# MadNLP/MadNLP.jl

Hardware: AMD Instinct MI355X
Metric: IP iterations/sec + ms per factorize!/solve!, condensed KKT n≈1e4 (higher is better)
Workload: dtype f64; 1 GPU; BASELINE config C3: case1354pegase-shaped sparse-condensed KKT, one instance; N=11192, m=16646, nnz(K)=68688; step = compress_J+compress_H+build_kkt+factorize (n_f=1) + inertia fetch + 2 solve_linear_system per instance; algorithm=BUNCHKAUFMAN (device: static-pivot LDL^T), outer_block=0, batch_per_gpu=1, batch_api=n/a (one instance), parallelism=1 GPU(s) x 1 independent instance(s)

## Files before the change

### include/madnlp_hip.h

```cpp
#ifndef MADNLP_HIP_H
#define MADNLP_HIP_H

#include <stdint.h>

#ifdef __cplusplus
extern "C" {
#endif

#define MNK_VERSION 100

enum { MNK_HOST = 0, MNK_DEVICE = 1 };

enum { MNK_BUNCHKAUFMAN = 1, MNK_LU = 2, MNK_QR = 3, MNK_CHOLESKY = 4, MNK_LDL = 5, MNK_EVD = 6 };

typedef struct mnk_ctx mnk_ctx;
typedef struct mnk_sc mnk_sc;
typedef struct mnk_dc mnk_dc;
typedef struct mnk_ls mnk_ls;

int mnk_version(void);
const char* mnk_last_error_string(void);
int mnk_ctx_create(int device, void* stream, mnk_ctx** out);
int mnk_ctx_destroy(mnk_ctx* ctx);
int mnk_ctx_synchronize(mnk_ctx* ctx);
// ... 156 lines not shown
                                       double* zl, double* zu);
int mnk_ipm_set_f_RR(mnk_ipm* ipm, double* f_R, const double* D_R, const double* x, const double* x_ref, double zeta);
int mnk_ipm_set_aug_rhs_RR(mnk_ipm* ipm, const double* f_R, const double* zl, const double* zu, const double* jacl,
                           const double* c, const double* y, const double* pp, const double* nn, const double* zp,
                           const double* zn, int64_t m, const double* x, const double* xl, const double* xu, double mu_R,
                           double rho, double* px, double* py, double* pzl, double* pzu);
int mnk_ipm_finish_aug_solve_RR(mnk_ipm* ipm, double* dpp, double* dnn, double* dzp, double* dzn, const double* l,
                                const double* dl, const double* pp, const double* nn, const double* zp, const double* zn,
                                int64_t m, double mu_R, double rho);
int mnk_ipm_reset_bound_dual_1(mnk_ipm* ipm, double* z, const double* x, int64_t n, double mu, double kappa_sigma);
int mnk_ipm_set_initial_bounds(mnk_ipm* ipm, double* xl, double* xu, int64_t n, double tol);
int mnk_ipm_set_initial_rhs(mnk_ipm* ipm, const double* f, const double* zl, const double* zu, double* px, double* py,
                            int64_t m, double* pzl, double* pzu);
int mnk_ipm_set_aug_rhs_ifr(mnk_ipm* ipm, const double* c, int64_t m, double* px, double* py, double* pzl, double* pzu);
int mnk_ipm_set_g_ifr(mnk_ipm* ipm, double* g, const double* f, const double* x, const double* xl, const double* xu,
                      const double* jacl, double mu);
int mnk_ipm_initialize_variables(mnk_ipm* ipm, double* x, const double* xl, const double* xu, int64_t n, double bound_push,
                                 double bound_fac);
int mnk_sc_set_aug_RR(mnk_sc* sc, const double* x, const double* xl, const double* xu, const double* zl, const double* zu,
                      const double* D_R, const double* pp, const double* zp, const double* nn, const double* zn, double zeta,
                      double primal_reg, double dual_reg);
int mnk_dc_set_aug_RR(mnk_dc* dc, const double* x, const double* xl, const double* xu, const double* zl, const double* zu,
                      const double* D_R, const double* pp, const double* zp, const double* nn, const double* zn, double zeta,
                      double primal_reg, double dual_reg);

int mnk_ipm_get_dot(mnk_ipm* ipm, const double* x, const double* y, int64_t n, double* out);
int mnk_ipm_get_sum(mnk_ipm* ipm, const double* v, int64_t n, double* out);
int mnk_ipm_get_norm2(mnk_ipm* ipm, const double* v, int64_t n, double* out);
int mnk_ipm_vec_copy(mnk_ipm* ipm, double* dst, const double* src, int64_t n);
int mnk_ipm_vec_fill(mnk_ipm* ipm, double* v, int64_t n, double value);
int mnk_ipm_vec_axpby(mnk_ipm* ipm, double* out, double a, const double* x, double b, const double* y, int64_t n);
int mnk_ipm_vec_scatter_axpy(mnk_ipm* ipm, double* y, const int64_t* idx, double a, const double* x, int64_t n);
int mnk_ipm_vec_gather(mnk_ipm* ipm, double* out, double a, const double* x, const int64_t* idx, int64_t n);
int mnk_ipm_bound_dual_axpy(mnk_ipm* ipm, double* zl, double* zu, double a, const double* dzl, const double* dzu);
int mnk_ipm_bound_dual_fill(mnk_ipm* ipm, double* zl, double* zu, double v);
int mnk_ipm_gemv(mnk_ipm* ipm, int trans, int64_t m, int64_t n, double alpha, const double* A, int64_t lda, const double* x,
                 double beta, double* y);

typedef struct mnk_opf mnk_opf;
int mnk_opf_create(mnk_ctx* ctx, int64_t nbus, int64_t ngen, int64_t nbranch, const int32_t* fr, const int32_t* to,
                   const int32_t* gen_bus, const double* arc_coef, const double* bus_data, const double* gen_cost,
                   mnk_opf** out);
int mnk_opf_destroy(mnk_opf* opf);
int mnk_opf_sizes(mnk_opf* opf, int64_t* n, int64_t* m, int64_t* nnzj, int64_t* nnzh);
int mnk_opf_obj_terms(mnk_opf* opf, const double* x, double* terms );
int mnk_opf_grad(mnk_opf* opf, const double* x, double* g);
int mnk_opf_cons(mnk_opf* opf, const double* x, double* c);
int mnk_opf_jac_coord(mnk_opf* opf, const double* x, double* jac);
int mnk_opf_hess_coord(mnk_opf* opf, const double* x, const double* y, double obj_weight, double* hess);

typedef struct mnk_schur mnk_schur;
int mnk_schur_create(mnk_ctx* ctx, int64_t ns_local, int64_t blk, int64_t nd, int algo, mnk_schur** out);
int mnk_schur_destroy(mnk_schur* h);
int mnk_schur_set_block(mnk_schur* h, int64_t k, const double* A_kk, int64_t lda, const double* C_dk, int64_t ldc,
                        int loc);
int mnk_schur_build_local(mnk_schur* h, const double* S0, int64_t lds0, int loc_s0, double* S_out, int64_t lds_out);
int mnk_schur_factorize_s(mnk_schur* h, const double* S, int64_t lds, int loc, int* info);
int mnk_schur_inertia_s(mnk_schur* h, int64_t* num_pos, int64_t* num_zero, int64_t* num_neg);
int mnk_schur_scenario_inertia(mnk_schur* h, int64_t k, int64_t* num_pos, int64_t* num_zero, int64_t* num_neg);
int mnk_schur_forward(mnk_schur* h, double* rhs_k, double* contrib_d);
int mnk_schur_solve_s(mnk_schur* h, double* rhs_d);
int mnk_schur_backward(mnk_schur* h, double* rhs_k, const double* x_d);
void* mnk_schur_s_buffer(mnk_schur* h);
int mnk_schur_set_structure(mnk_schur* h, int64_t n, int64_t m, int64_t nv, int64_t nc, int64_t nnzh, const int32_t* hess_I,
                            const int32_t* hess_J, int64_t nnzj, const int32_t* jac_I, const int32_t* jac_J, int64_t n_ineq,
                            const int64_t* ind_ineq, int64_t n_eq, const int64_t* ind_eq, int index_base, int64_t ns_global,
                            const int64_t* local_scen, int own_design);
int mnk_schur_assemble(mnk_schur* h, const double* hess, const double* jac, const double* pr_diag, const double* du_diag, int loc);
void* mnk_schur_s0_buffer(mnk_schur* h);
int mnk_schur_get_block(mnk_schur* h, int64_t k, double* A_kk, double* C_dk, double* S0);
int mnk_schur_solve(mnk_schur* h, double* rhs_k, double* rhs_d, int loc);

int mnk_ls_debug_solve_trace(mnk_ls* ls, unsigned long long* out, int64_t n);

int mnk_ls_debug_dag_state(mnk_ls* ls, int* flags, int64_t nflags, int* chain, int64_t nchain, int* have);

int mnk_debug_grid_at_launch(int cu_first, int num_cu, int first, int per_cu);
int mnk_debug_shader_clock(mnk_ctx* ctx, double* mhz);

int mnk_debug_dag_tasks(int ntile, int chunk, int band_tiles, int js2, int taper0, int* out, int cap, int* first_phase);
int mnk_debug_dag_merged_tasks(int ntile, int chunk, int band_tiles, int js2, int taper0, int fill, int ninst, int period,
                               int* out, int cap);

int mnk_debug_update(mnk_ctx* ctx, int variant, int64_t M, int64_t K, const double* A, int64_t lda,
                     double* C, double* C2, int64_t ldc, int reps, double* ms);

#ifdef __cplusplus
}
#endif
#endif
```

### madnlp.jl_amd/_lib.py

```python
from __future__ import annotations

import ctypes as C
import os
import subprocess

_HERE = os.path.dirname(os.path.abspath(__file__))
CSRC = os.path.join(_HERE, "csrc")
LIBDIR = os.path.join(_HERE, "lib")
LIBPATH = os.path.join(LIBDIR, "libmadnlp_hip.so")
_LIB_OVERRIDE = os.environ.get("MNK_LIBPATH")
SOURCES = ["gemm_f64.hip", "dag.hip", "factor.hip", "solve.hip", "ls.hip", "sparse_kkt.hip", "dense_kkt.hip", "bk.hip", "schur.hip", "ipm_vec.hip", "opf_eval.hip", "qr.hip"]
HEADERS = ["common.h", "ls.h", "kkt_vec.h", "gemm_tile.h", "leaf64.h", "gemm_macro.h", os.path.join("..", "..", "include", "madnlp_hip.h")]

MNK_HOST, MNK_DEVICE = 0, 1
MNK_BUNCHKAUFMAN, MNK_LU, MNK_QR, MNK_CHOLESKY, MNK_LDL, MNK_EVD = 1, 2, 3, 4, 5, 6
MNK_SC_JT, MNK_SC_HESS, MNK_SC_AUG, MNK_SC_DIAGBUF = 0, 1, 2, 3


def _stale() -> bool:
    if not os.path.exists(LIBPATH):
        return True
    t = os.path.getmtime(LIBPATH)
    deps = [os.path.join(CSRC, s) for s in SOURCES + HEADERS]
    return any(os.path.exists(d) and os.path.getmtime(d) > t for d in deps)
# ... 103 lines not shown
    "mnk_ipm_get_rel_search_norm": (C.c_int, [_vp, _vp, _vp, C.POINTER(C.c_double)]),
    "mnk_ipm_get_sd_sc": (C.c_int, [_vp, _vp, C.c_int64, _vp, _vp, C.c_double, C.POINTER(C.c_double)]),
    "mnk_ipm_get_norms": (C.c_int, [_vp, _vp, C.c_int64, C.POINTER(C.c_double)]),
    "mnk_ipm_set_perturbation_sets": (C.c_int, [_vp, C.c_int64, _vp, C.c_int64, _vp, C.c_int]),
    "mnk_ipm_set_aug_rhs": (C.c_int, [_vp, _vp, _vp, _vp, _vp, _vp, C.c_int64, _vp, _vp, _vp, C.c_double, _vp, _vp, _vp, _vp]),
    "mnk_ipm_dual_inf_perturbation": (C.c_int, [_vp, _vp, C.c_double, C.c_double]),
    "mnk_ipm_adjust_boundary": (C.c_int, [_vp, _vp, _vp, _vp, C.c_double]),
    "mnk_ipm_reset_bound_dual": (C.c_int, [_vp, _vp, _vp, _vp, _vp, _vp, C.c_double, C.c_double]),
    "mnk_ipm_get_obj_val_R": (C.c_int, [_vp, _vp, _vp, C.c_int64, _vp, _vp, _vp, C.c_double, C.c_double, C.POINTER(C.c_double)]),
    "mnk_ipm_get_theta_R": (C.c_int, [_vp, _vp, _vp, _vp, C.c_int64, C.POINTER(C.c_double)]),
    "mnk_ipm_get_inf_pr_R": (C.c_int, [_vp, _vp, _vp, _vp, C.c_int64, C.POINTER(C.c_double)]),
    "mnk_ipm_get_inf_du_R": (C.c_int, [_vp, _vp, _vp, _vp, _vp, _vp, _vp, _vp, C.c_int64, C.c_double, C.c_double, C.POINTER(C.c_double)]),
    "mnk_ipm_get_inf_compl_R": (C.c_int, [_vp, _vp, _vp, _vp, _vp, _vp, _vp, _vp, _vp, _vp, C.c_int64, C.c_double, C.c_double, C.POINTER(C.c_double)]),
    "mnk_ipm_get_alpha_max_R": (C.c_int, [_vp, _vp, _vp, _vp, _vp, _vp, _vp, _vp, _vp, C.c_int64, C.c_double, C.POINTER(C.c_double)]),
    "mnk_ipm_get_alpha_z_R": (C.c_int, [_vp, _vp, _vp, _vp, _vp, _vp, _vp, _vp, _vp, C.c_int64, C.c_double, C.POINTER(C.c_double)]),
    "mnk_ipm_get_varphi_R": (C.c_int, [_vp, C.c_double, _vp, _vp, _vp, _vp, _vp, C.c_int64, C.c_double, C.POINTER(C.c_double)]),
    "mnk_ipm_get_F": (C.c_int, [_vp, _vp, C.c_int64, _vp, _vp, _vp, _vp, _vp, _vp, _vp, C.c_double, C.POINTER(C.c_double)]),
    "mnk_ipm_get_varphi_d_R": (C.c_int, [_vp, _vp, _vp, _vp, _vp, _vp, _vp, _vp, _vp, _vp, C.c_int64, C.c_double, C.c_double, C.POINTER(C.c_double)]),
    "mnk_ipm_populate_RR_nn": (C.c_int, [_vp, _vp, _vp, C.c_int64, C.c_double, C.c_double]),
    "mnk_ipm_initialize_robust_restorer": (C.c_int, [_vp, _vp, _vp, C.c_int64, C.c_double, C.c_double, _vp, _vp, _vp, _vp, _vp, _vp, _vp, _vp]),
    "mnk_ipm_set_f_RR": (C.c_int, [_vp, _vp, _vp, _vp, _vp, C.c_double]),
    "mnk_ipm_set_aug_rhs_RR": (C.c_int, [_vp, _vp, _vp, _vp, _vp, _vp, _vp, _vp, _vp, _vp, _vp, C.c_int64, _vp, _vp, _vp, C.c_double, C.c_double, _vp, _vp, _vp, _vp]),
    "mnk_ipm_finish_aug_solve_RR": (C.c_int, [_vp, _vp, _vp, _vp, _vp, _vp, _vp, _vp, _vp, _vp, _vp, C.c_int64, C.c_double, C.c_double]),
    "mnk_ipm_reset_bound_dual_1": (C.c_int, [_vp, _vp, _vp, C.c_int64, C.c_double, C.c_double]),
    "mnk_ipm_set_initial_bounds": (C.c_int, [_vp, _vp, _vp, C.c_int64, C.c_double]),
    "mnk_ipm_set_initial_rhs": (C.c_int, [_vp, _vp, _vp, _vp, _vp, _vp, C.c_int64, _vp, _vp]),
    "mnk_ipm_set_aug_rhs_ifr": (C.c_int, [_vp, _vp, C.c_int64, _vp, _vp, _vp, _vp]),
    "mnk_ipm_set_g_ifr": (C.c_int, [_vp, _vp, _vp, _vp, _vp, _vp, _vp, C.c_double]),
    "mnk_ipm_initialize_variables": (C.c_int, [_vp, _vp, _vp, _vp, C.c_int64, C.c_double, C.c_double]),
    "mnk_ipm_get_dot": (C.c_int, [_vp, _vp, _vp, C.c_int64, C.POINTER(C.c_double)]),
    "mnk_ipm_get_sum": (C.c_int, [_vp, _vp, C.c_int64, C.POINTER(C.c_double)]),
    "mnk_ipm_get_norm2": (C.c_int, [_vp, _vp, C.c_int64, C.POINTER(C.c_double)]),
    "mnk_ipm_vec_copy": (C.c_int, [_vp, _vp, _vp, C.c_int64]),
    "mnk_ipm_vec_fill": (C.c_int, [_vp, _vp, C.c_int64, C.c_double]),
    "mnk_ipm_vec_axpby": (C.c_int, [_vp, _vp, C.c_double, _vp, C.c_double, _vp, C.c_int64]),
    "mnk_ipm_vec_scatter_axpy": (C.c_int, [_vp, _vp, _vp, C.c_double, _vp, C.c_int64]),
    "mnk_ipm_vec_gather": (C.c_int, [_vp, _vp, C.c_double, _vp, _vp, C.c_int64]),
    "mnk_ipm_bound_dual_axpy": (C.c_int, [_vp, _vp, _vp, C.c_double, _vp, _vp]),
    "mnk_ipm_bound_dual_fill": (C.c_int, [_vp, _vp, _vp, C.c_double]),
    "mnk_ipm_gemv": (C.c_int, [_vp, C.c_int, C.c_int64, C.c_int64, C.c_double, _vp, C.c_int64, _vp, C.c_double, _vp]),
    "mnk_opf_create": (C.c_int, [_vp, C.c_int64, C.c_int64, C.c_int64, _vp, _vp, _vp, _vp, _vp, _vp, C.POINTER(_vp)]),
    "mnk_opf_destroy": (C.c_int, [_vp]),
    "mnk_opf_sizes": (C.c_int, [_vp, _i64p, _i64p, _i64p, _i64p]),
    "mnk_opf_obj_terms": (C.c_int, [_vp, _vp, _vp]),
    "mnk_opf_grad": (C.c_int, [_vp, _vp, _vp]),
    "mnk_opf_cons": (C.c_int, [_vp, _vp, _vp]),
    "mnk_opf_jac_coord": (C.c_int, [_vp, _vp, _vp]),
    "mnk_opf_hess_coord": (C.c_int, [_vp, _vp, _vp, C.c_double, _vp]),
    "mnk_sc_set_aug_RR": (C.c_int, [_vp, _vp, _vp, _vp, _vp, _vp, _vp, _vp, _vp, _vp, _vp, C.c_double, C.c_double, C.c_double]),
    "mnk_dc_set_aug_RR": (C.c_int, [_vp, _vp, _vp, _vp, _vp, _vp, _vp, _vp, _vp, _vp, _vp, C.c_double, C.c_double, C.c_double]),
    "mnk_ls_bk_info": (C.c_int, [_vp, C.POINTER(C.c_int), C.POINTER(C.c_int), _vp, _vp]),
    "mnk_ls_get_stat": (C.c_int, [_vp, C.c_char_p, C.POINTER(C.c_double)]),
    "mnk_sc_set_bounds": (C.c_int, [_vp, C.c_int64, _vp, C.c_int64, _vp, C.c_int]),
    "mnk_sc_set_barrier_terms": (C.c_int, [_vp, _vp, _vp, _vp, _vp, _vp, C.c_int]),
    "mnk_sc_solve_kkt": (C.c_int, [_vp, _vp, _vp, C.c_int]),
    "mnk_sc_mul": (C.c_int, [_vp, _vp, _vp, C.c_double, C.c_double, C.c_int]),
    "mnk_dc_set_bounds": (C.c_int, [_vp, C.c_int64, _vp, C.c_int64, _vp, C.c_int]),
    "mnk_dc_set_barrier_terms": (C.c_int, [_vp, _vp, _vp, _vp, _vp, _vp, C.c_int]),
    "mnk_dc_solve_kkt": (C.c_int, [_vp, _vp, _vp, C.c_int]),
    "mnk_dc_mul": (C.c_int, [_vp, _vp, _vp, C.c_double, C.c_double, C.c_int]),
    "mnk_schur_create": (C.c_int, [_vp, C.c_int64, C.c_int64, C.c_int64, C.c_int, C.POINTER(_vp)]),
    "mnk_schur_destroy": (C.c_int, [_vp]),
    "mnk_schur_set_block": (C.c_int, [_vp, C.c_int64, _vp, C.c_int64, _vp, C.c_int64, C.c_int]),
    "mnk_schur_build_local": (C.c_int, [_vp, _vp, C.c_int64, C.c_int, _vp, C.c_int64]),
    "mnk_schur_factorize_s": (C.c_int, [_vp, _vp, C.c_int64, C.c_int, C.POINTER(C.c_int)]),
    "mnk_schur_inertia_s": (C.c_int, [_vp, _i64p, _i64p, _i64p]),
    "mnk_schur_scenario_inertia": (C.c_int, [_vp, C.c_int64, _i64p, _i64p, _i64p]),
    "mnk_schur_forward": (C.c_int, [_vp, _vp, _vp]),
    "mnk_schur_solve_s": (C.c_int, [_vp, _vp]),
    "mnk_schur_backward": (C.c_int, [_vp, _vp, _vp]),
    "mnk_schur_s_buffer": (C.c_void_p, [_vp]),
    "mnk_schur_set_structure": (C.c_int, [_vp, C.c_int64, C.c_int64, C.c_int64, C.c_int64, C.c_int64, _vp, _vp, C.c_int64, _vp, _vp,
                                          C.c_int64, _vp, C.c_int64, _vp, C.c_int, C.c_int64, _vp, C.c_int]),
    "mnk_schur_assemble": (C.c_int, [_vp, _vp, _vp, _vp, _vp, C.c_int]),
    "mnk_schur_s0_buffer": (_vp, [_vp]),
    "mnk_schur_get_block": (C.c_int, [_vp, C.c_int64, _vp, _vp, _vp]),
    "mnk_schur_solve": (C.c_int, [_vp, _vp, _vp, C.c_int]),
    "mnk_ls_debug_solve_trace": (C.c_int, [_vp, _vp, C.c_int64]),
    "mnk_ls_debug_dag_state": (C.c_int, [_vp, _vp, C.c_int64, _vp, C.c_int64, _vp]),
    "mnk_debug_grid_at_launch": (C.c_int, [C.c_int, C.c_int, C.c_int, C.c_int]),
    "mnk_debug_shader_clock": (C.c_int, [_vp, _vp]),
    "mnk_debug_dag_tasks": (C.c_int, [C.c_int, C.c_int, C.c_int, C.c_int, C.c_int, _vp, C.c_int, _vp]),
    "mnk_debug_dag_merged_tasks": (C.c_int, [C.c_int] * 8 + [_vp, C.c_int]),
    "mnk_factorize_batch_begin": (C.c_int, []),
    "mnk_factorize_batch_end": (C.c_int, []),
    "mnk_solve_batch_begin": (C.c_int, []),
    "mnk_solve_batch_end": (C.c_int, []),
    "mnk_release_idle_streams": (C.c_int, [C.c_int]),
    "mnk_sc_step_batch": (C.c_int, [C.c_int, _vp, _vp, _vp, _vp, _vp, _vp, C.c_int]),
    "mnk_ls_inertia_batch": (C.c_int, [C.c_int, _vp, _i64p, _i64p, _i64p]),
    "mnk_ls_solve_batch": (C.c_int, [C.c_int, _vp, _vp, C.c_int]),
    "mnk_debug_update": (C.c_int, [_vp, C.c_int, C.c_int64, C.c_int64, _vp, C.c_int64, _vp, _vp, C.c_int64, C.c_int,
                                   C.POINTER(C.c_double)]),
    "mnk_gemm_nt": (C.c_int, [_vp, C.c_int, C.c_int64, C.c_int64, C.c_int64, _vp, C.c_int64, _vp,
                              C.c_int64, _vp, C.c_int64]),
}


def lib():
    global _lib
    if _lib is not None:
        return _lib
    if not os.path.exists(LIBPATH):
        raise ImportError(
            f"{LIBPATH} is missing: run `python -c 'import __graft_entry__ as g; g.build()'` "
            "(hipcc --offload-arch=gfx950).  There is no CPU fallback for the KKT hot path.")
    try:
        import torch
    except Exception:
        pass
    l = C.CDLL(_LIB_OVERRIDE if _LIB_OVERRIDE and os.path.exists(_LIB_OVERRIDE) else LIBPATH)
    for name, (res, args) in SIGNATURES.items():
        f = getattr(l, name)
        f.restype = res
        f.argtypes = args
    _lib = l
    return l


class HipError(RuntimeError):
    pass


def check(rc: int, what: str = ""):
    if rc != 0:
        msg = lib().mnk_last_error_string()
        raise HipError(f"{what} failed (rc={rc}): {msg.decode() if msg else ''}")
```

### madnlp.jl_amd/csrc/dag.hip

```cpp
#include <algorithm>
#include <atomic>
#include <cfloat>
#include <climits>
#include <vector>

#include "gemm_tile.h"
#include "ls.h"

namespace mnk {

#ifndef MNK_DAG_DIAG_SUB
#define MNK_DAG_DIAG_SUB 1
#endif
struct DagInst {
    double* F;
    int64_t ld;
    double* V;
    const double* dinv;
    const double* dblk;
    const double* inv16;
    int* front;
    int* af;
    int* tprog;
    int* info;
    unsigned long long* vmax;
    double* zfill;
    int64_t N;
};

typedef const DagInst __attribute__((address_space(4))) * DagInstP;

struct DagArgs {
    const DagInst* insts;
    const int4* tasks;
    int ntasks;
    int ntile;
    int* qctr;
    long spin_limit;
    unsigned long long* trace;
    unsigned long long* wgstat;
    int fake_share;
};

#ifndef MNK_DIAG_BULK_DBG
#define MNK_DIAG_BULK_DBG 0
#endif
constexpr int DAG_BANDACC = 1, DAG_FINAL = 2, DAG_FIRST = 4, DAG_FILL = 8;

template <class IP>
__device__ __forceinline__ int dag_wait_front(IP a, long spin_limit, int s0, int s1, int s2, int s3, int c, int kend, int* s_val, int* d8 = nullptr) {
    if (threadIdx.x < 64) {
        const int lane = threadIdx.x;
        const int idx = lane == 0 ? s0 : (lane == 1 ? s1 : (lane == 2 ? s2 : s3));
        long spins = 0;
        int r;
        for (;;) {
            int f = lane < 4 ? __hip_atomic_load(a->front + idx, __ATOMIC_RELAXED, __HIP_MEMORY_SCOPE_AGENT) : INT_MAX;
#if MNK_DIAG_BULK_DBG
            const int f_raw = f;
#endif
            f = min(f, __shfl_xor(f, 1));
            f = min(f, __shfl_xor(f, 2));
            r = __builtin_amdgcn_readfirstlane(f);
            if (r > c) break;
            __builtin_amdgcn_s_sleep(4);
            if ((++spins & 255) == 0) {
#if MNK_DIAG_BULK_DBG
                if (d8 != nullptr && (spins & 0x3ffff) == 0) {
                    if (lane < 4) d8[8 + lane] = f_raw;
                    if (lane == 0) { d8[1] = 2; d8[2] = s0 | (s2 << 16); d8[3] = c; d8[4] = r; d8[5] = (int)(spins >> 18); }
                }
#endif
                if (__hip_atomic_load(a->info, __ATOMIC_RELAXED, __HIP_MEMORY_SCOPE_AGENT) != 0) {
#if MNK_DIAG_BULK_DBG
                    if (d8 != nullptr && lane == 0) { const unsigned long long now = wall_clock64(); d8[1] |= 16; d8[14] = (int)(unsigned)now; d8[15] = (int)(unsigned)(now >> 32); }
#endif
                    r = -1;
                    break;
                }
                if (spins > spin_limit) {
                    if (lane == 0 && atomicCAS(a->info, 0, -7) == 0) a->info[1] = 1;
                    r = -1;
                    break;
                }
            }
        }
        if (r > kend) r = kend;
        __builtin_amdgcn_fence(__ATOMIC_ACQUIRE, "agent");
        if (lane == 0) *s_val = r;
    }
    __syncthreads();
    const int r = *s_val;
    __syncthreads();
    return r;
}

template <class IP>
__device__ __forceinline__ bool dag_wait_words(IP a, long spin_limit, const int* w0, int t0, const int* w1, int t1, int* s_val, int* d8 = nullptr) {
    if (threadIdx.x < 64) {
        const int lane = threadIdx.x;
        long spins = 0;
        int ok = 1;
        for (;;) {
            const int v = lane < 2 ? __hip_atomic_load(lane == 0 ? w0 : w1, __ATOMIC_RELAXED, __HIP_MEMORY_SCOPE_AGENT) : INT_MAX;
            if (__all(v >= (lane == 0 ? t0 : (lane == 1 ? t1 : INT_MIN)))) break;
            __builtin_amdgcn_s_sleep(2);
            if ((++spins & 255) == 0) {
#if MNK_DIAG_BULK_DBG
                if (d8 != nullptr && (spins & 0x3ffff) == 0 && lane == 0) { d8[1] = 3; d8[2] = 0; d8[3] = t0; d8[4] = v; d8[5] = (int)(spins >> 18); }
#endif
// ... 82 lines not shown
                x0 = __builtin_amdgcn_mfma_f64_16x16x4f64(iv[sx], t0[sx], x0, 0, 0, 0);
                x1 = __builtin_amdgcn_mfma_f64_16x16x4f64(iv[sx], t1[sx], x1, 0, 0, 0);
            }
            X[h4 + cb][0] = x0;
            X[h4 + cb][1] = x1;
#pragma unroll
            for (int r = 0; r < 4; ++r) {
                if (LDL) vm = fmax(vm, fmax(fabs(x0[r]), fabs(x1[r])));
                const int64_t cc = (int64_t)(coff + 16 * cb + 4 * r) * ld;
                const double di = LDL ? Sd[16 * cb + 4 * r] : 1.0;
                Fs[cc] = LDL ? x0[r] * di : x0[r];
                Fs[cc + 16] = LDL ? x1[r] * di : x1[r];
                if (LDL) {
                    Vs[cc] = x0[r];
                    Vs[cc + 16] = x1[r];
                }
            }
            __builtin_amdgcn_sched_barrier(0);
        }
    };
    fill_diag(ja);
    __syncthreads();
    stamp(0);
    trsm(std::integral_constant<int, 0>(), 0);
    __syncthreads();
    stamp(1);
    {
        const double* __restrict__ Lba = F + (int64_t)64 * (ja + 1) + (int64_t)64 * ja * ld;
        for (int slot = tid; slot < 1024; slot += 256) {
            const int q = slot >> 6, i = slot & 15, k4 = (slot >> 4) & 3;
            const double* src = Lba + (16 * (q >> 2) + i) + (int64_t)(16 * (q & 3) + k4) * ld;
            v4f64 v;
#pragma unroll
            for (int sx = 0; sx < 4; ++sx) v[sx] = -src[(int64_t)(4 * sx) * ld];
            S[slot] = v;
        }
    }
    __syncthreads();
    stamp(2);
#pragma unroll
    for (int cb2 = 0; cb2 < 4; ++cb2)
#pragma unroll
        for (int ib = 0; ib < 4; ++ib) {
            const v4f64 aop = S[(cb2 * 4 + ib) * 64 + lane];
#pragma unroll
            for (int sx = 0; sx < 4; ++sx) {
                X[4 + cb2][0] = __builtin_amdgcn_mfma_f64_16x16x4f64(aop[sx], X[ib][0][sx], X[4 + cb2][0], 0, 0, 0);
                X[4 + cb2][1] = __builtin_amdgcn_mfma_f64_16x16x4f64(aop[sx], X[ib][1][sx], X[4 + cb2][1], 0, 0, 0);
            }
            if (ib == 3) __builtin_amdgcn_sched_barrier(0);
        }
    __syncthreads();
    stamp(3);
    fill_diag(ja + 1);
    __syncthreads();
    stamp(4);
    trsm(std::integral_constant<int, 1>(), 64);
    stamp(5);
    if (LDL && a->vmax != nullptr) {
        if (!(vm <= DBL_MAX)) vm = __longlong_as_double(0x7ff0000000000000LL);
        for (int off = 32; off > 0; off >>= 1) vm = fmax(vm, __shfl_xor(vm, off));
        if (lane == 0 && vm > 0.0) {
            const unsigned long long bits = (unsigned long long)__double_as_longlong(vm);
            if (bits > __hip_atomic_load(a->vmax, __ATOMIC_RELAXED, __HIP_MEMORY_SCOPE_AGENT)) atomicMax(a->vmax, bits);
        }
    }
}

__global__ void dag_gate_kernel(const int* __restrict__ word, int target, int* __restrict__ info, long spin_limit) {
    long spins = 0;
    while (__hip_atomic_load(word, __ATOMIC_RELAXED, __HIP_MEMORY_SCOPE_AGENT) < target) {
        __builtin_amdgcn_s_sleep(8);
        if ((++spins & 255) == 0) {
            if (__hip_atomic_load(info, __ATOMIC_RELAXED, __HIP_MEMORY_SCOPE_AGENT) != 0) break;
            if (spins > spin_limit) {
                if (atomicCAS(info, 0, -7) == 0) info[1] = 3;
                break;
            }
        }
    }
}

__global__ __launch_bounds__(256) void dag_reset_kernel(int* __restrict__ flags, int64_t n, int* __restrict__ info, DagInst rec,
                                                        DagInst* __restrict__ rec_dst, const SmallSysRec* __restrict__ recs = nullptr) {
    if (recs != nullptr) {
        const SmallSysRec r = recs[blockIdx.y];
        flags = r.flags; n = r.nflags; info = r.info;
    }
    if (blockIdx.x == 0 && threadIdx.x == 0 && rec_dst != nullptr) *rec_dst = rec;
    int4* f4 = reinterpret_cast<int4*>(flags);
    const int64_t n4 = n / 4, stride = (int64_t)gridDim.x * blockDim.x;
    for (int64_t i = (int64_t)blockIdx.x * blockDim.x + threadIdx.x; i < n4; i += stride) f4[i] = make_int4(0, 0, 0, 0);
    if (blockIdx.x == 0) {
        if (threadIdx.x < (unsigned)(n - 4 * n4)) flags[4 * n4 + threadIdx.x] = 0;
        if (threadIdx.x == 0) { info[0] = 0; info[1] = 0; }
    }
}

template <class IP>
__device__ __forceinline__ void dag_fill_tile(IP in, int I, int J, int tid) {
    double* Z = in->zfill;
    const int64_t ld = in->ld;
    const int r2 = (tid & 63) * 2, cg = tid >> 6;
#pragma unroll 4
    for (int c = cg; c < 128; c += 4) {
        const int64_t col = (int64_t)128 * J + c, row = (int64_t)128 * I + r2;
        double2 v = make_double2(0.0, 0.0);
        if (I == J && col >= in->N) {
            if (row == col) v.x = 1.0;
            if (row + 1 == col) v.y = 1.0;
        }
        *reinterpret_cast<double2*>(Z + row + col * ld) = v;
    }
}

template <bool LDL>
__global__ __launch_bounds__(256, 3) void dag_bulk_kernel(DagArgs a) {
    extern __shared__ __attribute__((aligned(16))) char smem_raw[];
    __shared__ int s_val;
    __shared__ unsigned long long s_stat[4];
    if (threadIdx.x < 4) s_stat[threadIdx.x] = 0;
    __syncthreads();
    for (;;) {
        int tid = threadIdx.x;
        asm volatile("" : "+v"(tid));
        if (tid == 0) s_val = atomicAdd(a.qctr, 1);
        __syncthreads();
        const int t = s_val;
        __syncthreads();
        if (t >= a.ntasks) {
            if (a.wgstat != nullptr && tid == 0) {
                unsigned long long* w = a.wgstat + (int64_t)blockIdx.x * 8;
                w[0] = s_stat[0]; w[1] = wall_clock64(); w[2] = s_stat[1]; w[3] = s_stat[2]; w[4] = s_stat[3];
            }
            return;
        }
        if (a.wgstat != nullptr && tid == 0) { if (s_stat[0] == 0) s_stat[0] = wall_clock64(); ++s_stat[2]; }
        const int4 tk = a.tasks[t];
        const int flags = __builtin_amdgcn_readfirstlane(tk.x) & 255, q = __builtin_amdgcn_readfirstlane(tk.x) >> 8;
        const int I = __builtin_amdgcn_readfirstlane(tk.y) & 0xffff, inst = __builtin_amdgcn_readfirstlane(tk.y) >> 16;
        const int J = __builtin_amdgcn_readfirstlane(tk.z);
        const int kbeg = __builtin_amdgcn_readfirstlane(tk.w) & 0xffff, kend = __builtin_amdgcn_readfirstlane(tk.w) >> 16;
        const int64_t row0 = (int64_t)128 * I, col0 = (int64_t)128 * J;
        unsigned long long* tr = a.trace != nullptr && tid == 0 ? a.trace + (int64_t)t * 8 : nullptr;
        if (tr) { tr[0] = wall_clock64(); tr[6] = 0; tr[7] = 0; }
        auto do_task = [&](auto in) __attribute__((always_inline)) {
        if (flags & DAG_FILL) {
            if (in->zfill != nullptr) dag_fill_tile(in, I, J, tid);
            return;
        }

        if (tid == 0) s_val = __hip_atomic_load(in->info, __ATOMIC_RELAXED, __HIP_MEMORY_SCOPE_AGENT) != 0 ? 1 : 0;
        __syncthreads();
        const bool dead = s_val != 0;
        __syncthreads();
        auto run_task = [&]() __attribute__((always_inline)) -> bool {
        if (dead) return false;
        int limit = 0;
        auto gate = [&](int kt) -> bool {
            if (kt < limit) return true;
            const unsigned long long w0 = tr ? wall_clock64() : 0;
            const int r = dag_wait_front(in, a.spin_limit, 2 * I, 2 * I + 1, 2 * J, 2 * J + 1, kbeg + (kt >> 4), kend, &s_val);
            if (tr) { const unsigned long long w1 = wall_clock64(); tr[2] = w1; tr[6] += 1; tr[7] += w1 - w0; s_stat[1] += w1 - w0; }
            if (r < 0) return false;
            limit = (__builtin_amdgcn_readfirstlane(r) - kbeg) * 16;
            return true;
        };
        const double* Ak = in->F + (a.fake_share > 0 ? (int64_t)128 * (kend + I % a.fake_share) : row0) + (int64_t)128 * kbeg * in->ld;
        const double* Bk = (LDL ? in->V : in->F) + (a.fake_share > 0 ? (int64_t)128 * (kend + J % a.fake_share) : col0) + (int64_t)128 * kbeg * in->ld;
        auto wait_chunk_order = [&]() -> bool {
            if (flags & DAG_FIRST) return true;
            const int* word = in->tprog + (int64_t)I * a.ntile + J;
            const unsigned long long w0 = tr ? wall_clock64() : 0;
            if (!dag_wait_words(in, a.spin_limit, word, q, word, q, &s_val)) return false;
            if (tr) s_stat[1] += wall_clock64() - w0;
            return true;
        };
        if ((flags & DAG_FINAL) && !(flags & DAG_BANDACC)) {
            __builtin_amdgcn_s_setprio(3);
            if (!wait_chunk_order()) return false;
            v4f64 X[8][2];
            {
                const int lane = tid & 63, w = tid >> 6;
                const double* Cs = in->F + (row0 + 32 * w + (lane & 15)) + (col0 + (lane >> 4)) * in->ld;
#pragma unroll
                for (int cb = 0; cb < 8; ++cb)
#pragma unroll
                    for (int r = 0; r < 4; ++r) {
                        const double* cp = Cs + (int64_t)(16 * cb + 4 * r) * in->ld;
                        X[cb][0][r] = cp[0];
                        X[cb][1][r] = cp[16];
                    }
            }
            if (kend > kbeg && !gate(0)) return false;
            (void)gemm_nt_mainloop3<2, 8, true>(X, Ak, in->ld, Bk, in->ld, (kend - kbeg) * 16, smem_raw, tid);
#pragma unroll
            for (int i = 0; i < 8; ++i) { asm volatile("" : "+v"(X[i][0])); asm volatile("" : "+v"(X[i][1])); }
            if (tr) tr[1] = tr[3] = wall_clock64();
            if (dag_wait_front(in, a.spin_limit, 2 * J, 2 * J + 1, 2 * J, 2 * J + 1, J, J + 1, &s_val) < 0) return false;
            if (tr) { tr[4] = wall_clock64(); s_stat[1] += tr[4] - tr[3]; }
            dag_finalize_tile<LDL>(in, row0, col0, 2 * J, smem_raw, tid, X, tr);
            if (tr) s_stat[3] += wall_clock64() - tr[4];
        } else if (!(MNK_DAG_DIAG_SUB && I == J && kend > kbeg)) {
            v4f64 acc[4][4];
#pragma unroll
            for (int i = 0; i < 4; ++i)
#pragma unroll
                for (int j = 0; j < 4; ++j) acc[i][j] = v4f64{0.0, 0.0, 0.0, 0.0};
            if (flags & DAG_FINAL) __builtin_amdgcn_s_setprio(3);
            if (!gemm_nt_mainloop<2, 2, 4, 0, 8>(acc, Ak, in->ld, Bk, in->ld, (kend - kbeg) * 16, smem_raw, tid, gate)) return false;
            if (tr) tr[1] = wall_clock64();
            if (!wait_chunk_order()) return false;
            if (kend > kbeg)
                gemm_nt_epilogue<2, 2, 4, 2, false, true>(acc, row0, col0, (int64_t)1 << 40, (int64_t)1 << 40, in->F, in->ld, nullptr, nullptr, 0, tid);
            if (tr) tr[3] = wall_clock64();
        } else {
            v4f64 acc[4][4];
#pragma unroll
            for (int i = 0; i < 4; ++i)
#pragma unroll
                for (int j = 0; j < 4; ++j) acc[i][j] = v4f64{0.0, 0.0, 0.0, 0.0};
            __builtin_amdgcn_s_setprio(3);
            if (!wait_chunk_order()) return false;
            gemm_nt_load_neg_lower<2, 2, 4>(acc, row0, col0, in->F, in->ld, tid);
            if (!gemm_nt_mainloop<2, 2, 4, 0, 8>(acc, Ak, in->ld, Bk, in->ld, (kend - kbeg) * 16, smem_raw, tid, gate)) return false;
            if (tr) tr[1] = wall_clock64();
            gemm_nt_store_neg_lower<2, 2, 4>(acc, row0, col0, in->F, in->ld, tid);
            if (tr) tr[3] = wall_clock64();
        }
        return true;
        };
        const bool done = run_task();
        asm volatile("s_waitcnt vmcnt(0)" ::: "memory");
        __syncthreads();
        if (done && tid == 0) {
            __builtin_amdgcn_fence(__ATOMIC_RELEASE, "agent");
            asm volatile("s_waitcnt vmcnt(0)" ::: "memory");
            if (!(flags & DAG_FINAL)) {
                __hip_atomic_store(in->tprog + (int64_t)I * a.ntile + J, q + 1, __ATOMIC_RELAXED, __HIP_MEMORY_SCOPE_AGENT);
            } else if (!(flags & DAG_BANDACC)) {
                __hip_atomic_store(in->front + 2 * I, J + 1, __ATOMIC_RELAXED, __HIP_MEMORY_SCOPE_AGENT);
                __hip_atomic_store(in->front + 2 * I + 1, J + 1, __ATOMIC_RELAXED, __HIP_MEMORY_SCOPE_AGENT);
            } else {
                __hip_atomic_store(in->af + (int64_t)I * a.ntile + J, 1, __ATOMIC_RELAXED, __HIP_MEMORY_SCOPE_AGENT);
            }
            if (tr) tr[5] = wall_clock64();
        }
        __builtin_amdgcn_s_setprio(0);
        __syncthreads();
        };
        do_task((DagInstP)(uintptr_t)(a.insts + inst));
    }
}

struct DagArgs1 {
    double* F;
    int64_t ld;
    double* V;
    const double* dinv;
    const double* dblk;
    const double* inv16;
    const int4* tasks;
    int ntasks;
    int* front;
    int* af;
    int* tprog;
    int ntile;
    int* qctr;
    int* info;
    long spin_limit;
    unsigned long long* trace;
    unsigned long long* wgstat;
    unsigned long long* vmax;
    int fake_share;
    double* zfill;
    int64_t N;
#if MNK_DIAG_BULK_DBG
    int* bdbg;
#endif
};

#if MNK_DIAG_BULK_DBG
#define MNK_BDBG(a) ((a).bdbg != nullptr ? (a).bdbg + 16 * blockIdx.x : nullptr)
int* g_diag_bdbg = nullptr;
#else
#define MNK_BDBG(a) nullptr
#endif

template <bool LDL>
__global__ __launch_bounds__(256, 3) void dag_bulk_kernel1(DagArgs1 a) {
    extern __shared__ __attribute__((aligned(16))) char smem_raw[];
    __shared__ int s_val;
    __shared__ unsigned long long s_stat[4];
    if (threadIdx.x < 4) s_stat[threadIdx.x] = 0;
    __syncthreads();
    for (;;) {
        int tid = threadIdx.x;
        asm volatile("" : "+v"(tid));
        if (tid == 0)
            s_val = __hip_atomic_load(a.info, __ATOMIC_RELAXED, __HIP_MEMORY_SCOPE_AGENT) != 0 ? INT_MAX : atomicAdd(a.qctr, 1);
        __syncthreads();
        const int t = s_val;
        __syncthreads();
        if (t >= a.ntasks) {
            if (a.wgstat != nullptr && tid == 0) {
                unsigned long long* w = a.wgstat + (int64_t)blockIdx.x * 8;
                w[0] = s_stat[0]; w[1] = wall_clock64(); w[2] = s_stat[1]; w[3] = s_stat[2]; w[4] = s_stat[3];
            }
            return;
        }
        if (a.wgstat != nullptr && tid == 0) { if (s_stat[0] == 0) s_stat[0] = wall_clock64(); ++s_stat[2]; }
#if MNK_DIAG_BULK_DBG
        if (a.bdbg != nullptr && tid == 0) {
            int* d8 = a.bdbg + 16 * blockIdx.x;
            d8[0] = t; d8[1] = 1; d8[6] += 1;
            d8[7] = (int)((__builtin_amdgcn_s_getreg(63492) & 0xffffu) | ((__builtin_amdgcn_s_getreg(63508) & 15u) << 16));
            const unsigned long long now = wall_clock64();
            d8[12] = (int)(unsigned)now; d8[13] = (int)(unsigned)(now >> 32);
        }
#endif
        const int4 tk = a.tasks[t];
        const int flags = __builtin_amdgcn_readfirstlane(tk.x) & 255, q = __builtin_amdgcn_readfirstlane(tk.x) >> 8;
        const int I = __builtin_amdgcn_readfirstlane(tk.y), J = __builtin_amdgcn_readfirstlane(tk.z);
        const int kbeg = __builtin_amdgcn_readfirstlane(tk.w) & 0xffff, kend = __builtin_amdgcn_readfirstlane(tk.w) >> 16;
        const int64_t row0 = (int64_t)128 * I, col0 = (int64_t)128 * J;
        unsigned long long* tr = a.trace != nullptr && tid == 0 ? a.trace + (int64_t)t * 8 : nullptr;
        if (tr) { tr[0] = wall_clock64(); tr[6] = 0; tr[7] = 0; }
        if (flags & DAG_FILL) {
            if (a.zfill != nullptr) dag_fill_tile(&a, I, J, tid);
            continue;
        }

        int limit = 0;
        auto gate = [&](int kt) -> bool {
            if (kt < limit) return true;
            const unsigned long long w0 = tr ? wall_clock64() : 0;
            const int r = dag_wait_front(&a, a.spin_limit, 2 * I, 2 * I + 1, 2 * J, 2 * J + 1, kbeg + (kt >> 4), kend, &s_val, MNK_BDBG(a));
            if (tr) { const unsigned long long w1 = wall_clock64(); tr[2] = w1; tr[6] += 1; tr[7] += w1 - w0; s_stat[1] += w1 - w0; }
            if (r < 0) return false;
            limit = (__builtin_amdgcn_readfirstlane(r) - kbeg) * 16;
            return true;
        };
        const double* Ak = a.F + (a.fake_share > 0 ? (int64_t)128 * (kend + I % a.fake_share) : row0) + (int64_t)128 * kbeg * a.ld;
        const double* Bk = (LDL ? a.V : a.F) + (a.fake_share > 0 ? (int64_t)128 * (kend + J % a.fake_share) : col0) + (int64_t)128 * kbeg * a.ld;
        auto wait_chunk_order = [&]() -> bool {
            if (flags & DAG_FIRST) return true;
            const int* word = a.tprog + (int64_t)I * a.ntile + J;
            const unsigned long long w0 = tr ? wall_clock64() : 0;
            if (!dag_wait_words(&a, a.spin_limit, word, q, word, q, &s_val, MNK_BDBG(a))) return false;
            if (tr) s_stat[1] += wall_clock64() - w0;
            return true;
        };
        if ((flags & DAG_FINAL) && !(flags & DAG_BANDACC)) {
            __builtin_amdgcn_s_setprio(3);
            if (!wait_chunk_order()) return;
            v4f64 X[8][2];
            {
                const int lane = tid & 63, w = tid >> 6;
                const double* Cs = a.F + (row0 + 32 * w + (lane & 15)) + (col0 + (lane >> 4)) * a.ld;
#pragma unroll
                for (int cb = 0; cb < 8; ++cb)
#pragma unroll
                    for (int r = 0; r < 4; ++r) {
                        const double* cp = Cs + (int64_t)(16 * cb + 4 * r) * a.ld;
                        X[cb][0][r] = cp[0];
                        X[cb][1][r] = cp[16];
                    }
            }
            if (kend > kbeg && !gate(0)) return;
            (void)gemm_nt_mainloop3<2, 8, true>(X, Ak, a.ld, Bk, a.ld, (kend - kbeg) * 16, smem_raw, tid);
#pragma unroll
            for (int i = 0; i < 8; ++i) { asm volatile("" : "+v"(X[i][0])); asm volatile("" : "+v"(X[i][1])); }
            if (tr) tr[1] = tr[3] = wall_clock64();
            if (dag_wait_front(&a, a.spin_limit, 2 * J, 2 * J + 1, 2 * J, 2 * J + 1, J, J + 1, &s_val, MNK_BDBG(a)) < 0) return;
            if (tr) { tr[4] = wall_clock64(); s_stat[1] += tr[4] - tr[3]; }
            dag_finalize_tile<LDL>(&a, row0, col0, 2 * J, smem_raw, tid, X, tr);
            if (tr) s_stat[3] += wall_clock64() - tr[4];
        } else if (!(MNK_DAG_DIAG_SUB && I == J && kend > kbeg)) {
            v4f64 acc[4][4];
#pragma unroll
            for (int i = 0; i < 4; ++i)
#pragma unroll
                for (int j = 0; j < 4; ++j) acc[i][j] = v4f64{0.0, 0.0, 0.0, 0.0};
            if (flags & DAG_FINAL) __builtin_amdgcn_s_setprio(3);
            if (!gemm_nt_mainloop<2, 2, 4, 0, 8>(acc, Ak, a.ld, Bk, a.ld, (kend - kbeg) * 16, smem_raw, tid, gate)) return;
            if (tr) tr[1] = wall_clock64();
            if (!wait_chunk_order()) return;
            if (kend > kbeg)
                gemm_nt_epilogue<2, 2, 4, 2, false, true>(acc, row0, col0, (int64_t)1 << 40, (int64_t)1 << 40, a.F, a.ld, nullptr, nullptr, 0, tid);
            if (tr) tr[3] = wall_clock64();
        } else {
            v4f64 acc[4][4];
#pragma unroll
            for (int i = 0; i < 4; ++i)
#pragma unroll
                for (int j = 0; j < 4; ++j) acc[i][j] = v4f64{0.0, 0.0, 0.0, 0.0};
            __builtin_amdgcn_s_setprio(3);
            if (!wait_chunk_order()) return;
            gemm_nt_load_neg_lower<2, 2, 4>(acc, row0, col0, a.F, a.ld, tid);
            if (!gemm_nt_mainloop<2, 2, 4, 0, 8>(acc, Ak, a.ld, Bk, a.ld, (kend - kbeg) * 16, smem_raw, tid, gate)) return;
            if (tr) tr[1] = wall_clock64();
            gemm_nt_store_neg_lower<2, 2, 4>(acc, row0, col0, a.F, a.ld, tid);
            if (tr) tr[3] = wall_clock64();
        }
        asm volatile("s_waitcnt vmcnt(0)" ::: "memory");
        __syncthreads();
        if (tid == 0) {
            __builtin_amdgcn_fence(__ATOMIC_RELEASE, "agent");
            asm volatile("s_waitcnt vmcnt(0)" ::: "memory");
            if (!(flags & DAG_FINAL)) {
                __hip_atomic_store(a.tprog + (int64_t)I * a.ntile + J, q + 1, __ATOMIC_RELAXED, __HIP_MEMORY_SCOPE_AGENT);
            } else if (!(flags & DAG_BANDACC)) {
                __hip_atomic_store(a.front + 2 * I, J + 1, __ATOMIC_RELAXED, __HIP_MEMORY_SCOPE_AGENT);
                __hip_atomic_store(a.front + 2 * I + 1, J + 1, __ATOMIC_RELAXED, __HIP_MEMORY_SCOPE_AGENT);
            } else {
                __hip_atomic_store(a.af + (int64_t)I * a.ntile + J, 1, __ATOMIC_RELAXED, __HIP_MEMORY_SCOPE_AGENT);
            }
            if (tr) tr[5] = wall_clock64();
#if MNK_DIAG_BULK_DBG
            if (a.bdbg != nullptr) {
                int* d8 = a.bdbg + 16 * blockIdx.x;
                const unsigned long long now = wall_clock64();
                d8[1] = 4; d8[14] = (int)(unsigned)now; d8[15] = (int)(unsigned)(now >> 32);
            }
#endif
        }
        __builtin_amdgcn_s_setprio(0);
        __syncthreads();
    }
}

int dag_build_tasks(int ntile, int chunk, int band_tiles, int js2, std::vector<int>& out, int taper0, std::vector<int>* ready) {
    struct T { int ready, cls, J, I, flags, q, kbeg, kend; };
    std::vector<T> ts;
    auto add_tile = [&](int I, int J, int K, bool band) {
        const int body = band ? K : std::max(0, K - 1);
        std::vector<int> cuts{body};
        int e = body;
        for (int len = taper0; len < chunk && e > 0; len *= 2) { e = std::max(0, e - len); cuts.push_back(e); }
        const int first = 1 + (I * 5 + J * 3) % chunk;
        while (e > first) { e = std::max(first, e - chunk); cuts.push_back(e); }
        if (e > 0) cuts.push_back(0);
        int q = 0;
        for (int c = (int)cuts.size() - 1; c > 0; --c, ++q) {
            const int kb = cuts[c], ke = cuts[c - 1];
            const bool last = band && ke == K;
            ts.push_back({ke, band ? 0 : 2, J, I, (band ? DAG_BANDACC : 0) | (last ? DAG_FINAL : 0) | (q == 0 ? DAG_FIRST : 0), q, kb, ke});
        }
        if (!band) ts.push_back({K, 1, J, I, DAG_FINAL | (q == 0 ? DAG_FIRST : 0), q, body, K});
    };
    for (int Jt = 0; Jt < ntile; ++Jt) {
        const int Js = Jt / 2;
        const int bt = Js >= js2 ? ntile : band_tiles;
        for (int I = 2 * Js + bt; I < ntile; ++I) add_tile(I, Jt, Jt, false);
        if (2 * Js - 2 > 0)
            for (int I = std::max(2 * Js, Jt); I < 2 * Js + bt && I < ntile; ++I) add_tile(I, Jt, 2 * Js - 2, true);
    }
    std::stable_sort(ts.begin(), ts.end(), [](const T& x, const T& y) {
        if (x.ready != y.ready) return x.ready < y.ready;
        if (x.cls != y.cls) return x.cls < y.cls;
        if (x.J != y.J) return x.J < y.J;
        return x.I < y.I;
    });
    out.clear();
    out.reserve(ts.size() * 4);
    if (ready != nullptr) { ready->clear(); ready->reserve(ts.size()); }
    int n1 = 0;
    for (const T& t : ts) {
        if (t.ready <= 2 * js2) ++n1;
        if (ready != nullptr) ready->push_back(t.ready);
        out.push_back(t.flags | (t.q << 8));
        out.push_back(t.I);
        out.push_back(t.J);
        out.push_back(t.kbeg | (t.kend << 16));
    }
    return n1;
}

int dag_add_fill_tasks(int ntile, std::vector<int>& tasks, std::vector<int>& ready, int n1) {
    const int nt = (int)(tasks.size() / 4), nfill = ntile * (ntile + 1) / 2;
    const int span = n1 > 0 ? n1 : nt;
    if (span <= 0) return n1;
    std::vector<int> out, rdy;
    out.reserve(tasks.size() + 4 * (size_t)nfill);
    rdy.reserve(ready.size() + nfill);
    int fi = 0, fj = 0, done = 0;
    auto emit_fill = [&](int r) {
        out.push_back(DAG_FILL); out.push_back(fi); out.push_back(fj); out.push_back(0);
        rdy.push_back(r);
        if (++fi >= ntile) { ++fj; fi = fj; }
        ++done;
    };
    for (int t = 0; t < nt; ++t) {
        for (int k = 0; k < 4; ++k) out.push_back(tasks[4 * t + k]);
        rdy.push_back(ready[t]);
        if (t < span)
            while (done < (int)((int64_t)(t + 1) * nfill / span)) emit_fill(ready[t]);
    }
    tasks.swap(out);
    ready.swap(rdy);
    return n1 > 0 ? n1 + nfill : 0;
}

void dag_merge_tasks(const std::vector<int>& tasks, const std::vector<int>& ready, int ninst, int period, std::vector<int>& out) {
    const int nt = (int)ready.size();
    out.clear();
    out.reserve((size_t)ninst * nt * 4);
    std::vector<int> pos(ninst, 0);
    for (;;) {
        int best = -1;
        long bkey = 0;
        for (int i = 0; i < ninst; ++i) {
            if (pos[i] >= nt) continue;
            const long key = (long)i * period + ready[pos[i]];
            if (best < 0 || key < bkey) { best = i; bkey = key; }
        }
        if (best < 0) break;
        const int t = pos[best]++;
        out.push_back(tasks[4 * t]);
        out.push_back(tasks[4 * t + 1] | (best << 16));
        out.push_back(tasks[4 * t + 2]);
        out.push_back(tasks[4 * t + 3]);
    }
}

template <bool LDL>
static int launch_bulk_t(hipStream_t s, const DagArgs& a, int nwg) {
    const size_t smem = TILE3_LDS_BYTES;
    auto kern = dag_bulk_kernel<LDL>;
    static std::atomic<uint64_t> attr_devs{0};
    int dev = 0;
    MNK_HIP(hipGetDevice(&dev));
    if (!(attr_devs.load(std::memory_order_relaxed) >> (dev & 63) & 1)) {
        MNK_HIP(hipFuncSetAttribute((const void*)kern, hipFuncAttributeMaxDynamicSharedMemorySize, (int)smem));
        attr_devs.fetch_or(1ull << (dev & 63), std::memory_order_relaxed);
    }
    hipLaunchKernelGGL(kern, dim3(nwg), dim3(256), smem, s, a);
    MNK_HIP(hipGetLastError());
    return 0;
}

template <bool LDL>
static int launch_bulk1_t(hipStream_t s, const DagArgs1& a, int nwg) {
    const size_t smem = TILE3_LDS_BYTES;
    auto kern = dag_bulk_kernel1<LDL>;
    static std::atomic<uint64_t> attr_devs{0};
    int dev = 0;
    MNK_HIP(hipGetDevice(&dev));
    if (!(attr_devs.load(std::memory_order_relaxed) >> (dev & 63) & 1)) {
        MNK_HIP(hipFuncSetAttribute((const void*)kern, hipFuncAttributeMaxDynamicSharedMemorySize, (int)smem));
        attr_devs.fetch_or(1ull << (dev & 63), std::memory_order_relaxed);
    }
    hipLaunchKernelGGL(kern, dim3(nwg), dim3(256), smem, s, a);
    MNK_HIP(hipGetLastError());
    return 0;
}

static int launch_dag_bulk(hipStream_t s, bool ldl, const DagInst& one, const DagInst* insts, const int* tasks, int ntasks, int ntile,
                           int* qctr, long spin_limit, int nwg, unsigned long long* trace, unsigned long long* wgstat) {
    if (ntasks <= 0) return 0;
    static const int fake = getenv("MNK_DAG_FAKE_SHARE") ? atoi(getenv("MNK_DAG_FAKE_SHARE")) : 0;
    if (insts == nullptr) {
        DagArgs1 a{one.F, one.ld, one.V, one.dinv, one.dblk, one.inv16, reinterpret_cast<const int4*>(tasks), ntasks, one.front, one.af,
                   one.tprog, ntile, qctr, one.info, spin_limit, trace, wgstat, one.vmax, fake, one.zfill, one.N};
#if MNK_DIAG_BULK_DBG
        a.bdbg = g_diag_bdbg;
#endif
        return ldl ? launch_bulk1_t<true>(s, a, nwg) : launch_bulk1_t<false>(s, a, nwg);
    }
    DagArgs a{insts, reinterpret_cast<const int4*>(tasks), ntasks, ntile, qctr, spin_limit, trace, wgstat, fake};
    return ldl ? launch_bulk_t<true>(s, a, nwg) : launch_bulk_t<false>(s, a, nwg);
}

}

using namespace mnk;

int mnk_dag_warmup(hipStream_t* streams, int n, int nwg) {
    static mnk::DevBuf<int> ctr;
    if (!ctr.p) {
        if (ctr.alloc(4)) return -2;
        MNK_HIP(hipMemset(ctr.p, 0, 4 * sizeof(int)));
    }
    for (int i = 0; i < n; ++i) {
        if (streams[i] == nullptr) continue;
        mnk::DagArgs1 a1{};
        a1.qctr = ctr.p;
        a1.info = ctr.p + 1;
        mnk::DagArgs a{};
        a.qctr = ctr.p;
        int rc = mnk::launch_bulk1_t<true>(streams[i], a1, nwg);
        if (!rc) rc = mnk::launch_bulk1_t<false>(streams[i], a1, nwg);
        if (!rc) rc = mnk::launch_bulk_t<true>(streams[i], a, nwg);
        if (!rc) rc = mnk::launch_bulk_t<false>(streams[i], a, nwg);
        if (rc) return rc;
    }
    for (int i = 0; i < n; ++i)
        if (streams[i] != nullptr) MNK_HIP(mnk::stream_wait(streams[i]));
    return 0;
}

long mnk_ls_dag_spin_limit(const mnk_ls* ls) {
    if (ls->dag_spin_limit > 0) return ls->dag_spin_limit;
    const double n = (double)ls->Np;
    const double t_est = n * n * n / 3.0 / 50e12;
    const double polls = 10.0 * t_est / 0.17e-6;
    const double floor_polls = mnk_live_contexts(ls->ctx->device) > 1 ? 5880000.0 : 588000.0;
    return (long)std::min(16777216.0, std::max(floor_polls, polls));
}

static mnk::DagInst dag_instance(mnk_ls* ls) {
    const int ntile = (int)(ls->Np / 128), nblk = (int)(ls->Np / NBI);
    int* front = ls->dag_flags.p + 2;
    int* af = front + nblk;
    int* tprog = af + (size_t)ntile * ntile;
    double* zfill = (ls->dag_fill && ls->dag_has_fill && ls->spare_pending && ls->fact_spare.p && !ls->spare_zeroed) ? ls->fact_spare.p : nullptr;
    return mnk::DagInst{ls->fact.p, ls->ld, ls->algo == MNK_LDL ? ls->vfull.p : nullptr, ls->dinv.p, ls->dblk.p, ls->inv16.p,
                        front, af, tprog, ls->info_dev.p, mnk_ls_growth_word(ls), zfill, ls->N};
}

int mnk_ls_dag_prepare(mnk_ls* ls) {
    mnk_ctx* ctx = ls->ctx;
    hipStream_t s = ctx->stream;
    const int64_t Np = ls->Np, ld = ls->ld;
    const bool ldl = ls->algo == MNK_LDL;
    const int ntile = (int)(Np / 128), nblk = (int)(Np / NBI), nsc = (int)((Np + 255) / 256);
    const size_t nflags = (size_t)2 + nblk + 2 * (size_t)ntile * ntile;
    auto give_up = [&]() {
        (void)hipGetLastError();
        ls->dag_tasks.release();
        ls->dag_flags.release();
        ls->vfull.release();
        return 1;
    };
    if (!ls->dag_tasks.p) {
        const int64_t deep_rows = std::min<int64_t>((int64_t)ctx->dag_cus2 * NBI, ls->dag_deep_rows);
        ls->dag_js2 = (ctx->dag_cus2 > 0 && Np <= deep_rows) ? 0 : nsc;
        if (ls->dag_js2_override >= 0) ls->dag_js2 = std::min(nsc, ls->dag_js2_override);
        std::vector<int>& h = ls->dag_host_tasks;
        ls->dag_ntasks1 = mnk::dag_build_tasks(ntile, ls->dag_chunk, ls->dag_band / 2, ls->dag_js2, h, ls->dag_taper0, &ls->dag_host_ready);
        ls->dag_has_fill = ls->dag_fill && ls->prefill && Np <= ls->prefill_max_rows;
        if (ls->dag_has_fill && h.empty()) ls->dag_has_fill = false;
        if (ls->dag_has_fill) ls->dag_ntasks1 = mnk::dag_add_fill_tasks(ntile, h, ls->dag_host_ready, ls->dag_ntasks1);
        ls->dag_ntasks = (int)(h.size() / 4);
        if (ls->dag_tasks.alloc(h.size() + 4)) return give_up();
        {
            mnk::H2DGuard h2d;
            if (!h.empty() && hipMemcpyAsync(ls->dag_tasks.p, h.data(), h.size() * sizeof(int), hipMemcpyHostToDevice, s) != hipSuccess) return give_up();
            if (mnk::stream_wait(s) != hipSuccess) return give_up();
        }
        if (ls->dag_flags.alloc(nflags)) return give_up();
    }
    if (ldl && !ls->vfull.p && ls->vfull.alloc((size_t)ld * Np + SLACK)) {
        (void)hipGetLastError();
        bool ok = false;
        if (ls->fact_spare.p && !ls->spare_zeroed) {
            ls->fact_spare.release();
            ls->prefill = 0;
            ls->spare_pending = false;
            ok = ls->vfull.alloc((size_t)ld * Np + SLACK) == 0;
        }
        if (!ok) return give_up();
    }
    if (ls->dag_trace_on) {
        const size_t ntr = (size_t)ls->dag_ntasks * 8 + 4096 * 8 + 1024 * 8;
        if (ls->dag_trace.n < ntr && ls->dag_trace.alloc(ntr)) return give_up();
    }
    return 0;
}

int mnk_ls_run_factorization_dag(mnk_ls* ls) {
    mnk_ctx* ctx = ls->ctx;
    hipStream_t s = ctx->stream;
    const int64_t Np = ls->Np;
    const bool ldl = ls->algo == MNK_LDL;
    const int ntile = (int)(Np / 128), nblk = (int)(Np / NBI), nsc = (int)((Np + 255) / 256);
    const size_t nflags = (size_t)2 + nblk + 2 * (size_t)ntile * ntile;
    MNK_REQUIRE(ls->dag_tasks.p && ls->dag_flags.p && (!ldl || ls->vfull.p), "task-DAG schedule: mnk_ls_dag_prepare was not called");
    const mnk::DagInst inst = dag_instance(ls);
    ls->dag_filled = inst.zfill != nullptr;
    hipLaunchKernelGGL(mnk::dag_reset_kernel, dim3((unsigned)std::min<size_t>((nflags + 1023) / 1024, 64)), dim3(256), 0, s,
                       ls->dag_flags.p, (int64_t)nflags, ls->info_dev.p, inst, (mnk::DagInst*)nullptr);
    int* qctr = ls->dag_flags.p;
    int* front = inst.front;
    const long spin_limit = mnk_ls_dag_spin_limit(ls);
    unsigned long long* trace = nullptr;
    if (ls->dag_trace_on && ls->dag_trace.p) {
        const size_t ntr = (size_t)ls->dag_ntasks * 8 + 4096 * 8 + 1024 * 8;
        MNK_HIP(hipMemsetAsync(ls->dag_trace.p, 0, ntr * sizeof(unsigned long long), s));
        trace = ls->dag_trace.p;
    }
    const int js2 = ls->dag_js2;
    auto phase = [&](hipStream_t sp, hipStream_t su, int chain_cus, int task0, int ntask, int* counter, int js_begin, int js_end,
                     unsigned strips) -> int {
        const bool small = js_begin == 0 && js_end == nsc && js2 == 0 && ls->dag_chain_inline;
        if (small) sp = s;
        MNK_HIP(hipEventRecord(ctx->ev_a, s));
        if (!small) MNK_HIP(hipStreamWaitEvent(sp, ctx->ev_a, 0));
        MNK_HIP(hipStreamWaitEvent(su, ctx->ev_a, 0));
        mnk::PpDag dag{front, inst.af, ntile, 0, 0, -1, spin_limit, trace ? trace + (size_t)ls->dag_ntasks * 8 + (size_t)js_begin * 8 * 16 : nullptr,
                  mnk_ls_growth_word(ls), ls->dag_debug ? ls->dag_dbg.p : nullptr};
        int rc = mnk_launch_pchain(ls, sp, dag, js_begin, js_end, strips);
        if (rc) return rc;
#if MNK_DIAG_BULK_DBG
        mnk::g_diag_bdbg = ls->dag_debug && ls->dag_dbg.p ? ls->dag_dbg.p + 8 * 128 : nullptr;
#endif
        rc = mnk::launch_dag_bulk(su, ldl, inst, nullptr, ls->dag_tasks.p + 4 * (size_t)task0, ntask, ntile, counter, spin_limit,
                                  std::min(ntask, mnk_ctx_bulk_wgs(ctx, chain_cus, 3)), trace ? trace + 8 * (size_t)task0 : nullptr,
                                  trace ? trace + (size_t)ls->dag_ntasks * 8 + 4096 * 8 + (task0 > 0 ? 512 * 8 : 0) : nullptr);
        if (rc) return rc;
        if (js_begin == 0 && js_end > 0) {
            const int64_t safe = std::min<int64_t>(js_end, std::max<int64_t>(0, (ntile - ls->dag_band / 2 - 1) / 2)) & ~(int64_t)1;
            if (strips == (unsigned)ls->dag_band && safe > 0) {
                rc = mnk_ls_invert_blocks(ls, su, 0, safe);
                if (rc) return rc;
                ls->inv_done = safe;
            }
        }
        if (small) {
            rc = mnk_ls_invert_blocks(ls, s, 0, nsc);
            if (rc) return rc;
            ls->inv_done = nsc;
        } else if (js_begin == 0 && js_end == nsc && js2 == 0) {
            hipLaunchKernelGGL(mnk::dag_gate_kernel, dim3(1), dim3(1), 0, su, front + (nblk - 1), ntile, ls->info_dev.p, spin_limit);
            rc = mnk_ls_invert_blocks(ls, su, 0, nsc);
            if (rc) return rc;
            ls->inv_done = nsc;
        }
        if (!small) MNK_HIP(hipEventRecord(ctx->ev_a, sp));
        MNK_HIP(hipEventRecord(ctx->ev_b, su));
        if (!small) MNK_HIP(hipStreamWaitEvent(s, ctx->ev_a, 0));
        MNK_HIP(hipStreamWaitEvent(s, ctx->ev_b, 0));
        return 0;
    };
    if (js2 > 0) {
        int rc = phase(ctx->sp_dag, ctx->su_dag, ctx->dag_cus, 0, ls->dag_ntasks1, qctr, 0, std::min(js2, nsc),
                       (unsigned)std::min<int64_t>(ls->dag_band, Np / NBI));
        if (rc) return rc;
    }
    if (js2 < nsc) {
        const int64_t rows2 = Np - 256 * (int64_t)js2;
        MNK_REQUIRE(ctx->sp_dag2 != nullptr, "task-DAG schedule: the deep-band streams are missing");
        int rc = phase(ctx->sp_dag2, ctx->su_dag2, ctx->dag_cus2, ls->dag_ntasks1, ls->dag_ntasks - ls->dag_ntasks1,
                       qctr + 1, js2, nsc, (unsigned)(rows2 / NBI));
        if (rc) return rc;
    }
    return 0;
}

namespace {
struct BatchState {
    int depth = 0;
    bool active = false;
    std::vector<mnk_ls*> pend;
};
thread_local BatchState t_batch;

struct BatchBuffers {
    mnk::DevBuf<int> tasks;
    mnk::DevBuf<int> qctr;
    mnk::DevBuf<char> insts, pcsys, aux;
    char* stage = nullptr;
    size_t stage_bytes = 0;
    hipEvent_t stage_ev = nullptr;
    int ntile = 0, ninst = 0, period = 0, chunk = 0, taper0 = 0, band = 0, ntasks = 0;
    bool fill = false;
    hipEvent_t ev[4] = {nullptr, nullptr, nullptr, nullptr};
};
BatchBuffers g_batch[64];
}

bool mnk_batch_active() { return t_batch.active; }

bool mnk_batch_defer(mnk_ls* ls) {
    if (!t_batch.active) return false;
    const int nsc = (int)((ls->Np + 255) / 256);
    if (ls->algo_now != 5 || (ls->dag_js2 != nsc && ls->dag_js2 != 0) || ls->dag_trace_on || ls->ctx->partitioned) return false;
    if (mnk_ctx_ensure_batch_streams(ls->ctx) != 0) (void)hipGetLastError();
    if (!ls->ctx->sp_dagB) return false;
    if (!ls->ev_defer && hipEventCreateWithFlags(&ls->ev_defer, hipEventDisableTiming) != hipSuccess) { (void)hipGetLastError(); return false; }
    if (hipEventRecord(ls->ev_defer, ls->ctx->stream) != hipSuccess) { (void)hipGetLastError(); return false; }
    ls->deferred = true;
    t_batch.pend.push_back(ls);
    return true;
}

static void batch_mark_done(mnk_ls* ls) {
    ls->factorized = true;
    ls->info_valid = false;
    ls->bk_active = false;
    ls->deferred = false;
}

static int batch_run_group(std::vector<mnk_ls*>& g) {
    mnk_ls* l0 = g[0];
    mnk_ctx* c0 = l0->ctx;
    hipStream_t h = c0->stream;
    MNK_HIP(hipSetDevice(c0->device));
    const int64_t Np = l0->Np;
    const bool ldl = l0->algo == MNK_LDL;
    const int ntile = (int)(Np / 128), nsc = (int)((Np + 255) / 256), ninst = (int)g.size();
    const size_t nflags = (size_t)2 + (size_t)(Np / NBI) + 2 * (size_t)ntile * ntile;
    for (mnk_ls* ls : g)
        if (ls->ctx->stream != h) MNK_HIP(hipStreamWaitEvent(h, ls->ev_defer, 0));
    int rc = mnk_persist_begin(c0, h);
    if (rc) return rc;
    auto body = [&]() -> int {
        BatchBuffers& B = g_batch[c0->device & 63];
        const int period = std::max((ntile + 1) / 2, l0->batch_period > 0 ? l0->batch_period : 0);
        if (B.ntile != ntile || B.ninst != ninst || B.period != period || B.chunk != l0->dag_chunk || B.taper0 != l0->dag_taper0 ||
            B.band != l0->dag_band || B.fill != l0->dag_has_fill || !B.tasks.p) {
            std::vector<int> merged;
            mnk::dag_merge_tasks(l0->dag_host_tasks, l0->dag_host_ready, ninst, period, merged);
            if (B.tasks.alloc(merged.size() + 4)) return -2;
            { mnk::H2DGuard h2d; MNK_HIP(hipMemcpy(B.tasks.p, merged.data(), merged.size() * sizeof(int), hipMemcpyHostToDevice)); }
            if (!B.qctr.p && B.qctr.alloc(4)) return -2;
            if (B.insts.alloc(sizeof(mnk::DagInst) * (size_t)ninst)) return -2;
            for (hipEvent_t& e : B.ev)
                if (!e) MNK_HIP(hipEventCreateWithFlags(&e, hipEventDisableTiming));
            B.ntile = ntile; B.ninst = ninst; B.period = period; B.chunk = l0->dag_chunk; B.taper0 = l0->dag_taper0;
            B.band = l0->dag_band; B.fill = l0->dag_has_fill; B.ntasks = (int)(merged.size() / 4);
        }
        std::vector<mnk::DagInst> hin;
        mnk::DagInst* insts_dev = reinterpret_cast<mnk::DagInst*>(B.insts.p);
        for (mnk_ls* ls : g) {
            hin.push_back(dag_instance(ls));
            ls->dag_filled = hin.back().zfill != nullptr;
            hipLaunchKernelGGL(mnk::dag_reset_kernel, dim3((unsigned)std::min<size_t>((nflags + 1023) / 1024, 64)), dim3(256), 0, h,
                               ls->dag_flags.p, (int64_t)nflags, ls->info_dev.p, hin.back(), insts_dev + (hin.size() - 1));
        }
        MNK_HIP(hipMemsetAsync(B.qctr.p, 0, 4 * sizeof(int), h));
        hipStream_t sp[2] = {c0->sp_dag, c0->sp_dagB}, su = c0->su_dagB;
        MNK_HIP(hipEventRecord(B.ev[0], h));
        MNK_HIP(hipStreamWaitEvent(sp[0], B.ev[0], 0));
        MNK_HIP(hipStreamWaitEvent(sp[1], B.ev[0], 0));
        MNK_HIP(hipStreamWaitEvent(su, B.ev[0], 0));
        const unsigned strips = (unsigned)std::min<int64_t>(l0->dag_band, Np / NBI);
        const int bulk_wgs = mnk_ctx_bulk_wgs(c0, 2 * c0->dag_cus, 3);
        auto launch_chain = [&](int i) -> int {
            mnk_ls* ls = g[i];
            mnk::PpDag dag{hin[i].front, hin[i].af, ntile, 0, 0, -1, mnk_ls_dag_spin_limit(ls), nullptr, mnk_ls_growth_word(ls)};
            return mnk_launch_pchain(ls, sp[i & 1], dag, 0, nsc, strips);
        };
        auto launch_tail = [&](int i) -> int {
            mnk_ls* ls = g[i];
            int r = mnk_ls_invert_blocks(ls, sp[i & 1], 0, nsc);
            if (r) return r;
            ls->inv_done = nsc;
            return mnk_ls_launch_finish_info(ls, sp[i & 1]);
        };
        for (int i = 0; i < std::min(2, ninst); ++i) {
            int r = launch_chain(i);
            if (r) return r;
        }
        int r = mnk::launch_dag_bulk(su, ldl, hin[0], insts_dev, B.tasks.p, B.ntasks, ntile, B.qctr.p,
                                     mnk_ls_dag_spin_limit(l0), std::min(B.ntasks, bulk_wgs), nullptr, nullptr);
        if (r) return r;
        for (int i = 0; i < ninst; ++i) {
            r = launch_tail(i);
            if (r) return r;
            if (i + 2 < ninst) {
                r = launch_chain(i + 2);
                if (r) return r;
            }
        }
        MNK_HIP(hipEventRecord(B.ev[1], sp[0]));
        MNK_HIP(hipEventRecord(B.ev[2], sp[1]));
        MNK_HIP(hipEventRecord(B.ev[3], su));
        for (int e = 1; e < 4; ++e) MNK_HIP(hipStreamWaitEvent(h, B.ev[e], 0));
        return 0;
    };
    rc = body();
    rc = mnk_persist_end(c0, h, rc);
    if (rc) return rc;
    MNK_HIP(hipEventRecord(l0->ev_defer, h));
    for (mnk_ls* ls : g) {
        if (ls->ctx->stream != h) MNK_HIP(hipStreamWaitEvent(ls->ctx->stream, l0->ev_defer, 0));
        batch_mark_done(ls);
        int r = mnk_ls_prefill_spare(ls);
        if (r) return r;
    }
    return 0;
}

static int batch_run_group_small(std::vector<mnk_ls*>& g) {
    mnk_ls* l0 = g[0];
    mnk_ctx* c0 = l0->ctx;
    hipStream_t h = c0->stream;
    MNK_HIP(hipSetDevice(c0->device));
    const int64_t Np = l0->Np;
    const bool ldl = l0->algo == MNK_LDL;
    const int ntile = (int)(Np / 128), nsc = (int)((Np + 255) / 256), strips = (int)(Np / NBI);
    const size_t nflags = (size_t)2 + (size_t)(Np / NBI) + 2 * (size_t)ntile * ntile;
    const int ntasks1 = l0->dag_ntasks;
    const int bulk_min = ntasks1 > 0 ? std::max(32, c0->num_cu / 4) : 0;
    auto chain_cus_for = [&](int k) { return std::min(c0->num_cu, (k * strips + 63) / 64 * 64); };
    int kmax = std::min(32, (c0->num_cu - bulk_min) / strips);
    while (kmax > 1 && chain_cus_for(kmax) > c0->num_cu - bulk_min) --kmax;
    if (kmax < 2) {
        for (mnk_ls* ls : g) {
            ls->deferred = false;
            int rc = mnk_ls_run_factorization_now(ls);
            if (rc) return rc;
        }
        return 0;
    }
    for (mnk_ls* ls : g)
        if (ls->ctx->stream != h) MNK_HIP(hipStreamWaitEvent(h, ls->ev_defer, 0));
    BatchBuffers& B = g_batch[c0->device & 63];
    for (size_t r0 = 0; r0 < g.size(); r0 += (size_t)kmax) {
        const int k = (int)std::min<size_t>(kmax, g.size() - r0);
        hipStream_t sp = nullptr, su = nullptr;
        int rc = mnk_masked_stream_pair(c0, chain_cus_for(k), &sp, &su);
        if (rc) return rc;
        if (ntasks1 > 0 && su == nullptr) { set_error("factorize batch: no CUs left for the bulk kernel"); return -1; }
        rc = mnk_persist_begin(c0, h);
        if (rc) return rc;
        auto body = [&]() -> int {
            if (ntasks1 > 0 && (B.ntile != ntile || B.ninst != k || B.period != 0 || B.chunk != l0->dag_chunk || B.taper0 != l0->dag_taper0 ||
                                B.band != l0->dag_band || B.fill != l0->dag_has_fill || !B.tasks.p)) {
                std::vector<int> merged;
                mnk::dag_merge_tasks(l0->dag_host_tasks, l0->dag_host_ready, k, 0, merged);
                if (B.tasks.alloc(merged.size() + 4)) return -2;
                { mnk::H2DGuard h2d; MNK_HIP(hipMemcpy(B.tasks.p, merged.data(), merged.size() * sizeof(int), hipMemcpyHostToDevice)); }
                B.ntile = ntile; B.ninst = k; B.period = 0; B.chunk = l0->dag_chunk; B.taper0 = l0->dag_taper0;
                B.band = l0->dag_band; B.fill = l0->dag_has_fill; B.ntasks = (int)(merged.size() / 4);
            }
            if (!B.qctr.p && B.qctr.alloc(4)) return -2;
            if (B.insts.n < sizeof(mnk::DagInst) * (size_t)k && B.insts.alloc(sizeof(mnk::DagInst) * (size_t)std::max(k, 32))) return -2;
            if (B.pcsys.n < mnk_pchain_sys_bytes() * (size_t)k && B.pcsys.alloc(mnk_pchain_sys_bytes() * (size_t)std::max(k, 32))) return -2;
            for (hipEvent_t& e : B.ev)
                if (!e) MNK_HIP(hipEventCreateWithFlags(&e, hipEventDisableTiming));
            std::vector<mnk::DagInst> hin;
            std::vector<int*> fronts;
            std::vector<const int*> afs;
            mnk::DagInst* insts_dev = reinterpret_cast<mnk::DagInst*>(B.insts.p);
            const size_t pc_bytes = mnk_pchain_sys_bytes();
            const size_t need = (size_t)k * (sizeof(mnk::DagInst) + pc_bytes + sizeof(mnk::SmallSysRec));
            if (B.aux.n < sizeof(mnk::SmallSysRec) * (size_t)k && B.aux.alloc(sizeof(mnk::SmallSysRec) * (size_t)std::max(k, 32))) return -2;
            if (B.stage_ev == nullptr) MNK_HIP(hipEventCreateWithFlags(&B.stage_ev, hipEventDisableTiming));
            else MNK_HIP(hipEventSynchronize(B.stage_ev));
            if (B.stage_bytes < need) {
                mnk::LaunchLock lock;
                if (B.stage) { mnk::quiesce_persistent(); (void)hipHostFree(B.stage); B.stage = nullptr; }
                const size_t cap = (size_t)std::max(k, 32) * (sizeof(mnk::DagInst) + pc_bytes + sizeof(mnk::SmallSysRec));
                MNK_HIP(hipHostMalloc((void**)&B.stage, cap, hipHostMallocDefault));
                B.stage_bytes = cap;
            }
            mnk::DagInst* st_inst = reinterpret_cast<mnk::DagInst*>(B.stage);
            char* st_pc = B.stage + (size_t)k * sizeof(mnk::DagInst);
            mnk::SmallSysRec* st_aux = reinterpret_cast<mnk::SmallSysRec*>(st_pc + (size_t)k * pc_bytes);
            const bool batch_aux = l0->linv_mfma && !l0->solve512;
            for (int i = 0; i < k; ++i) {
                mnk_ls* ls = g[r0 + i];
                hin.push_back(dag_instance(ls));
                ls->dag_filled = hin.back().zfill != nullptr;
                fronts.push_back(hin.back().front);
                afs.push_back(hin.back().af);
                st_inst[i] = hin.back();
                mnk_pchain_fill_sys(ls, st_pc + (size_t)i * pc_bytes, hin.back().front, hin.back().af);
                mnk_ls_fill_small_rec(ls, st_aux + i);
            }
            MNK_HIP(hipMemcpyAsync(B.insts.p, st_inst, (size_t)k * sizeof(mnk::DagInst), hipMemcpyHostToDevice, h));
            MNK_HIP(hipMemcpyAsync(B.pcsys.p, st_pc, (size_t)k * pc_bytes, hipMemcpyHostToDevice, h));
            MNK_HIP(hipMemcpyAsync(B.aux.p, st_aux, (size_t)k * sizeof(mnk::SmallSysRec), hipMemcpyHostToDevice, h));
            MNK_HIP(hipEventRecord(B.stage_ev, h));
            const mnk::SmallSysRec* aux_dev = reinterpret_cast<const mnk::SmallSysRec*>(B.aux.p);
            hipLaunchKernelGGL(mnk::dag_reset_kernel, dim3((unsigned)std::min<size_t>((nflags + 1023) / 1024, 64), (unsigned)k), dim3(256), 0, h,
                               (int*)nullptr, (int64_t)0, (int*)nullptr, hin[0], (mnk::DagInst*)nullptr, aux_dev);
            MNK_HIP(hipMemsetAsync(B.qctr.p, 0, 4 * sizeof(int), h));
            MNK_HIP(hipEventRecord(B.ev[0], h));
            MNK_HIP(hipStreamWaitEvent(sp, B.ev[0], 0));
            if (su != nullptr) MNK_HIP(hipStreamWaitEvent(su, B.ev[0], 0));
            int r = mnk_launch_pchain_multi(g.data() + r0, k, sp, nullptr, B.pcsys.p, fronts.data(), afs.data());
            if (r) return r;
            if (ntasks1 > 0) {
                const int bulk_wgs = mnk_ctx_bulk_wgs(c0, chain_cus_for(k), 3);
                r = mnk::launch_dag_bulk(su, ldl, hin[0], insts_dev, B.tasks.p, B.ntasks, ntile, B.qctr.p, mnk_ls_dag_spin_limit(l0),
                                         std::min(B.ntasks, bulk_wgs), nullptr, nullptr);
                if (r) return r;
                MNK_HIP(hipEventRecord(B.ev[2], su));
                MNK_HIP(hipStreamWaitEvent(h, B.ev[2], 0));
            }
            MNK_HIP(hipEventRecord(B.ev[1], sp));
            MNK_HIP(hipStreamWaitEvent(h, B.ev[1], 0));
            if (su != nullptr) MNK_HIP(hipStreamWaitEvent(su, B.ev[1], 0));
            if (su != nullptr) MNK_HIP(hipStreamWaitEvent(sp, B.ev[2], 0));
            if (batch_aux) {
                r = mnk_ls_invert_blocks_batch(h, ldl, aux_dev, k, Np);
                if (r) return r;
                r = mnk_ls_finish_info_batch(h, aux_dev, k, ldl ? (l0->N >= 4096 ? 1024 : 256) : 64);
                if (r) return r;
                for (int i = 0; i < k; ++i) {
                    mnk_ls* ls = g[r0 + i];
                    ls->inv_done = nsc;
                    if (!ls->ev_info) MNK_HIP(hipEventCreateWithFlags(&ls->ev_info, hipEventDisableTiming));
                    MNK_HIP(hipEventRecord(ls->ev_info, h));
                    ls->ev_info_recorded = true;
                }
                return 0;
            }
            hipStream_t inv_s[3] = {h, sp, su != nullptr ? su : sp};
            for (int i = 0; i < k; ++i) {
                mnk_ls* ls = g[r0 + i];
                hipStream_t si = inv_s[i % 3];
                r = mnk_ls_invert_blocks(ls, si, 0, nsc);
                if (r) return r;
                ls->inv_done = nsc;
                r = mnk_ls_launch_finish_info(ls, si);
                if (r) return r;
            }
            MNK_HIP(hipEventRecord(B.ev[1], sp));
            MNK_HIP(hipStreamWaitEvent(h, B.ev[1], 0));
            if (su != nullptr) {
                MNK_HIP(hipEventRecord(B.ev[2], su));
                MNK_HIP(hipStreamWaitEvent(h, B.ev[2], 0));
            }
            return 0;
        };
        rc = body();
        rc = mnk_persist_end(c0, h, rc);
        if (rc) return rc;
    }
    MNK_HIP(hipEventRecord(l0->ev_defer, h));
    for (mnk_ls* ls : g) {
        if (ls->ctx->stream != h) MNK_HIP(hipStreamWaitEvent(ls->ctx->stream, l0->ev_defer, 0));
        batch_mark_done(ls);
        int r = mnk_ls_prefill_spare(ls);
        if (r) return r;
    }
    return 0;
}

static int batch_flush() {
    std::vector<mnk_ls*> pend;
    pend.swap(t_batch.pend);
    int rc_all = 0;
    while (!pend.empty()) {
        mnk_ls* l0 = pend.front();
// ... 81 lines not shown
```

### madnlp.jl_amd/csrc/factor.hip

```cpp
#include <atomic>
#include <type_traits>
#include <atomic>
#include <cfloat>
#include <chrono>
#include <cmath>
#include <cstdlib>

#include "ls.h"
#include "leaf64.h"

namespace mnk {

template <bool LDL, int NS>
__device__ __forceinline__ void trsm64_mfma_body(double* __restrict__ F, int64_t ld, int64_t j0, int64_t Np,
                                                 const double* __restrict__ Dblk, const double* __restrict__ inv16,
                                                 const double* __restrict__ dinv, double* __restrict__ W, int64_t ldw,
                                                 int64_t wcol, const int* __restrict__ info,
                                                 unsigned long long* __restrict__ vmax) {
    if (*info != 0) return;
    const int lane = threadIdx.x & 63, wave = threadIdx.x >> 6;
    const int l15 = lane & 15, l4 = lane >> 4;
    const int64_t r0 = j0 + 64 + ((int64_t)blockIdx.x * 4 + wave) * (16 * NS);
    if (r0 >= Np) return;
    double Ln[6][4];
// ... 1086 lines not shown
            MNK_HIP(hipFuncSetAttribute((const void*)pchain_kernel<true>, hipFuncAttributeMaxDynamicSharedMemorySize, PC_LDS_BYTES));
            MNK_HIP(hipFuncSetAttribute((const void*)pchain_kernel<false>, hipFuncAttributeMaxDynamicSharedMemorySize, PC_LDS_BYTES));
            attr_devs.fetch_or(1ull << (dev & 63), std::memory_order_relaxed);
        }
    }
    const bool ldl = ls->algo == MNK_LDL;
    const int epoch16 = ls->epoch * 16;
    double* V = ldl ? ls->vfull.p : nullptr;
    if (ldl)
        hipLaunchKernelGGL(pchain_kernel<true>, dim3(strips), dim3(256), PC_LDS_BYTES, sp, ls->fact.p, ls->ld, ls->Np, ls->dblk.p,
                           ls->inv16.p, ls->dvec.p, ls->dinv.p, V, ls->info_dev.p, ls->pivot_tol, ls->flag_p.p, epoch16,
                           ls->debug_pp_missing, dag, js_begin, js_end);
    else
        hipLaunchKernelGGL(pchain_kernel<false>, dim3(strips), dim3(256), PC_LDS_BYTES, sp, ls->fact.p, ls->ld, ls->Np, ls->dblk.p,
                           ls->inv16.p, ls->dvec.p, ls->dinv.p, V, ls->info_dev.p, ls->pivot_tol, ls->flag_p.p, epoch16,
                           ls->debug_pp_missing, dag, js_begin, js_end);
    MNK_HIP(hipGetLastError());
    return 0;
}

static int run_factorization_body(mnk_ls* ls);

size_t mnk_pchain_sys_bytes() { return sizeof(mnk::PcSys); }
void mnk_pchain_fill_sys(mnk_ls* ls, void* rec_host, int* front, const int* af) {
    const bool ldl = ls->algo == MNK_LDL;
    *static_cast<mnk::PcSys*>(rec_host) = mnk::PcSys{ls->fact.p, ls->ld, ls->Np, ls->dblk.p, ls->inv16.p, ls->dvec.p, ls->dinv.p,
                                                       ldl ? ls->vfull.p : nullptr, ls->info_dev.p, ls->pivot_tol, ls->flag_p.p,
                                                       ls->epoch * 16, front, af, (int)(ls->Np / 128), mnk_ls_dag_spin_limit(ls),
                                                       mnk_ls_growth_word(ls)};
}

int mnk_launch_pchain_multi(mnk_ls* const* v, int n, hipStream_t sp, hipStream_t fill_stream, void* table, int* const* front,
                            const int* const* af) {
    {
        static std::atomic<uint64_t> attr_devs{0};
        int dev = 0;
        MNK_HIP(hipGetDevice(&dev));
        if (!(attr_devs.load(std::memory_order_relaxed) >> (dev & 63) & 1)) {
            MNK_HIP(hipFuncSetAttribute((const void*)pchain_multi_kernel<true>, hipFuncAttributeMaxDynamicSharedMemorySize, PC_LDS_BYTES));
            MNK_HIP(hipFuncSetAttribute((const void*)pchain_multi_kernel<false>, hipFuncAttributeMaxDynamicSharedMemorySize, PC_LDS_BYTES));
            attr_devs.fetch_or(1ull << (dev & 63), std::memory_order_relaxed);
        }
    }
    mnk::PcSys* dst = static_cast<mnk::PcSys*>(table);
    const bool ldl = v[0]->algo == MNK_LDL;
    const int strips = (int)(v[0]->Np / NBI);
    for (int i = 0; i < n && fill_stream != nullptr; ++i) {
        mnk_ls* ls = v[i];
        mnk::PcSys rec{ls->fact.p, ls->ld, ls->Np, ls->dblk.p, ls->inv16.p, ls->dvec.p, ls->dinv.p, ldl ? ls->vfull.p : nullptr,
                       ls->info_dev.p, ls->pivot_tol, ls->flag_p.p, ls->epoch * 16, front[i], af[i], (int)(ls->Np / 128),
                       mnk_ls_dag_spin_limit(ls), mnk_ls_growth_word(ls)};
        hipLaunchKernelGGL(pc_set_sys_kernel, dim3(1), dim3(1), 0, fill_stream, rec, dst + i);
    }
    MNK_HIP(hipGetLastError());
    if (ldl)
        hipLaunchKernelGGL(pchain_multi_kernel<true>, dim3((unsigned)(n * strips)), dim3(256), PC_LDS_BYTES, sp, dst, strips);
    else
        hipLaunchKernelGGL(pchain_multi_kernel<false>, dim3((unsigned)(n * strips)), dim3(256), PC_LDS_BYTES, sp, dst, strips);
    MNK_HIP(hipGetLastError());
    return 0;
}

int mnk_ls_run_factorization(mnk_ls* ls) {
    if (ls->algo == MNK_QR) return mnk_qr_factor(ls);
    mnk_ctx* ctx = ls->ctx;
    hipStream_t s = ctx->stream;
    const int64_t Np = ls->Np;
    if (ls->panel_algo >= 4 && !ls->flag_p.p) {
        if (ls->flag_p.alloc(Np / NBI + 1)) return -2;
        MNK_HIP(hipMemsetAsync(ls->flag_p.p, 0, (Np / NBI + 1) * sizeof(int), s));
    }
    ++ls->epoch;
    ls->inv_done = 0;
    ls->factor_invalid = false;
    ls->t_fact_launch_ms = mnk_host_ms();
    {
        const int want = (ls->early_reject && ls->accept_only_pd && ls->algo == MNK_LDL && ls->src_persistent) ? 1 : 0;
        if (want != ls->reject_on_device) {
            MNK_HIP(hipMemsetAsync(ls->info_dev.p + 2, want, sizeof(int), s));
            ls->reject_on_device = want;
        }
    }
    ls->algo_now = ls->panel_algo;
    const int64_t min_rows = mnk_batch_active() ? std::min<int64_t>(ls->dag_min_rows, 256) : ls->dag_min_rows;
    if (ls->algo_now == 5 && (ctx->dag_cus < ls->dag_band || !ls->lookahead || Np < min_rows || Np > ls->dag_max_rows)) ls->algo_now = 4;
    if (ls->algo_now == 5 && ctx->sp_dag == nullptr && mnk_ctx_ensure_dag(ctx) != 0) { (void)hipGetLastError(); ls->algo_now = 4; }
    if (ls->algo_now == 5 && ctx->sp_dag == nullptr) ls->algo_now = 4;
    ++ls->fact_count;
    if (ls->pp_blocked && ls->fact_count >= ls->pp_retry_at) ls->pp_blocked = false;
    if (ls->algo_now >= 4 && ls->pp_blocked) ls->algo_now = 1;
    if (ls->algo_now == 5 && mnk_ls_dag_prepare(ls) != 0) ls->algo_now = 4;
    if (ls->algo_now == 5 && ls->dag_js2 < (Np + 255) / 256) {
        if (mnk_ctx_ensure_dag2(ctx) != 0) (void)hipGetLastError();
        if (ctx->sp_dag2 == nullptr) ls->algo_now = 4;
    }
    if (ls->algo_now == 5 && mnk_batch_defer(ls)) return 0;
    return mnk_ls_run_factorization_now(ls);
}

int mnk_ls_run_factorization_now(mnk_ls* ls) {
    mnk_ctx* ctx = ls->ctx;
    hipStream_t s = ctx->stream;
    const bool persistent = ls->algo_now >= 4;
    if (persistent) {
        int rc0 = mnk_persist_begin(ctx, s);
        if (rc0) return rc0;
    }
    const int rc_run = run_factorization_body(ls);
    return persistent ? mnk_persist_end(ctx, s, rc_run) : rc_run;
}

static int run_factorization_body(mnk_ls* ls) {
    mnk_ctx* ctx = ls->ctx;
    hipStream_t s = ctx->stream;
    const int64_t Np = ls->Np, ld = ls->ld;
    const bool ldl = ls->algo == MNK_LDL;
    double* F = ls->fact.p;
    const int64_t NBO = mnk_ls_effective_nbo(ls);
    if (ls->algo_now != 5) MNK_HIP(hipMemsetAsync(ls->info_dev.p, 0, 2 * sizeof(int), s));
    std::vector<int64_t> bnd{0};
    for (int64_t pos = 0; pos < Np;) {
        const bool tail = ls->lookahead && NBO < Np && ls->tail_rows > 0 && Np - pos <= ls->tail_rows && ls->tail_nbo < NBO;
        pos = std::min<int64_t>(pos + (tail ? ls->tail_nbo : NBO), Np);
        bnd.push_back(pos);
    }
    const int64_t npanel = (int64_t)bnd.size() - 1;
    const bool la = ls->lookahead && npanel > 1;

    if (ls->algo_now == 5) {
        int rc = mnk_ls_run_factorization_dag(ls);
        if (rc) return rc;
    } else if (!la) {
        for (int64_t ko = 0; ko < Np; ko += NBO) {
            const int64_t kend = std::min<int64_t>(ko + NBO, Np);
            int rc = factor_outer_panel(ls, s, ko, kend, ls->wbuf[0].p);
            if (rc) return rc;
            const int64_t Mt = Np - kend;
            if (Mt > 0) {
                const double* Wsrc = ldl ? ls->wbuf[0].p + kend : F + kend + ko * ld;
                rc = launch_gemm_nt(s, 2, Mt, Mt, kend - ko, Wsrc, ldl ? ls->ldw : ld, F + kend + ko * ld, ld,
                                    F + kend + kend * ld, ld, nullptr, nullptr, 0, ls->info_dev.p);
                if (rc) return rc;
            }
        }
    } else {
        { int rc_s = mnk_ctx_ensure_panel_streams(ctx); if (rc_s) return rc_s; }
        hipStream_t sp = ctx->sp, su = ctx->su;
        if ((int64_t)ctx->ev_panel.size() < npanel + 1) {
            const size_t old = ctx->ev_panel.size();
            ctx->ev_panel.resize(npanel + 1);
            ctx->ev_next.resize(npanel + 1);
            ctx->ev_next2.resize(npanel + 1);
            ctx->ev_bdone.resize(npanel + 1);
            for (size_t e = old; e < ctx->ev_panel.size(); ++e) {
                MNK_HIP(hipEventCreateWithFlags(&ctx->ev_panel[e], hipEventDisableTiming));
                MNK_HIP(hipEventCreateWithFlags(&ctx->ev_next[e], hipEventDisableTiming));
                MNK_HIP(hipEventCreateWithFlags(&ctx->ev_next2[e], hipEventDisableTiming));
                MNK_HIP(hipEventCreateWithFlags(&ctx->ev_bdone[e], hipEventDisableTiming));
            }
        }
        const int pcus = ctx->panel_cus;
        const int ucus = pcus > 0 ? ctx->num_cu - pcus : ctx->num_cu;
        const bool share = ls->share != 0;
        if (share) {
            if (ls->tile_ctr.n < 8 * ((size_t)npanel + 1)) {
                int rc0 = ls->tile_ctr.alloc(8 * ((size_t)npanel + 1));
// ... 307 lines not shown
```

### madnlp.jl_amd/csrc/ls.h

```cpp
#pragma once
#include <algorithm>
#include <functional>
#include <memory>
#include <string>
#include <vector>

#include "common.h"

struct mnk_sc {
    mnk_ctx* ctx = nullptr;
    int64_t n = 0, m = 0, nnzj = 0, nnzh = 0;
    int64_t nnz_jt = 0, nnz_hess = 0, nnz_aug = 0, len_jptr = 0;
    std::vector<int32_t> jt_colptr, jt_rowval, h_colptr, h_rowval, aug_colptr, aug_rowval;
    std::vector<int64_t> jt_map, h_map;
    std::vector<int32_t> d_dst, d_src, hp_dst, hp_src, j_dst, j_c, j_k, j_l;
    mnk::DevBuf<int32_t> jt_seg_ptr, jt_seg_src, h_seg_ptr, h_seg_src;
    mnk::DevBuf<int32_t> aug_hptr, aug_hsrc;
    mnk::DevBuf<int32_t> aug_dsrc;
    mnk::DevBuf<int32_t> aug_jptr, aug_jc, aug_jk, aug_jl;
    mnk::DevBuf<int32_t> aug_row, aug_col;
    mnk::DevBuf<int32_t> d_jt_colptr, d_jt_rowval, d_jt_colidx, d_h_colptr, d_h_rowval, d_h_colidx;
    mnk::DevBuf<double> jac_coo, hess_coo, jt_nz, h_nz, aug_nz, diag_buffer, pr_diag, du_diag;
    void* extra = nullptr;
    std::shared_ptr<int> alive = std::make_shared<int>(0);
};

struct mnk_dc {
    mnk_ctx* ctx = nullptr;
    int condensed = 1;
    bool mirror_pending = false;
    int64_t n = 0, m = 0, ns = 0, n_eq = 0, order = 0;
    std::vector<int64_t> ind_ineq, ind_eq;
    mnk::DevBuf<int64_t> d_ind_ineq, d_ind_eq;
    mnk::DevBuf<double> hess, jac, aug, pr_diag, du_diag, diag_buffer;
    mnk::DevBuf<double> jis;
    int64_t ld_jis = 0, kpad = 0, npad = 0;
    void* extra = nullptr;
    std::shared_ptr<int> alive = std::make_shared<int>(0);
};

struct mnk_ls {
    mnk_ctx* ctx = nullptr;
    int64_t N = 0, Np = 0, ld = 0, ldw = 0, nbo = 512;
    bool nbo_auto = true;
    int algo = MNK_LDL;
    double pivot_tol = 0.0;
    int lookahead = 1;
    int share = 1;
    int small_tiles = 400;
    int split_a = 2;
    int64_t single_rows = 2560;
    int64_t tail_rows = 4096;
    int64_t tail_nbo = 256;
    int small_tiles_mid = 1000;
    mnk::DevBuf<int> tile_ctr;
    mnk::DevBuf<double> fact, wbuf[2], linv, dblk, inv16, linv256, linv256t, dvec, dinv, xwork;
    mnk::DevBuf<double> fact_spare;
    hipEvent_t ev_spare = nullptr, ev_free = nullptr;
    bool spare_zeroed = false, spare_pending = false;
    int prefill = 1;
    int64_t prefill_max_rows = 24576;
    int epoch = 0;
    mnk::DevBuf<int> flag_p;
    int panel0_whole = 1;
    int algo_now = 1;
    bool pp_blocked = false;
    int64_t fact_count = 0, pp_retry_at = 0, pp_backoff = 16;
    int pp_fallbacks = 0;
    int last_timeout_site = 0;
    double stall_ms_total = 0.0;
    double t_fact_launch_ms = 0.0;
    int64_t pp_fuse_rows = 4096;
    int64_t own_cols = 128;
    mnk::DevBuf<int> dag_tasks;
    int dag_ntasks = 0, dag_ntasks1 = 0, dag_js2 = 0;
    std::vector<int> dag_host_tasks, dag_host_ready;
    int dag_fill = 1;
    bool dag_has_fill = false;
    bool dag_filled = false;
    int batch_period = 0;
    hipEvent_t ev_info = nullptr;
    bool ev_info_recorded = false;
    hipEvent_t ev_defer = nullptr;
    bool deferred = false;
    mnk::DevBuf<int> dag_flags;
    mnk::DevBuf<double> vfull;
    mnk::DevBuf<unsigned long long> dag_trace;
    bool dag_trace_on = false;
    int64_t inv_done = 0;
    int dag_band = 16;
    int dag_taper0 = 2;
    long dag_spin_limit = 0;
    int dag_chunk = 64;
    int64_t dag_min_rows = 1280;
    int64_t dag_deep_rows = 5376;
    int64_t dag_max_rows = 30720;
    int panel_algo = 5;
    int persistent_solve = 1;
    int solve512 = 0;
    int64_t solve512_min_rows = 4096;
    int dag_chain_inline = 1;
    std::vector<std::string> env_keys;
    int dag_js2_override = -1;
    int linv_mfma = 1;
    mnk::DevBuf<double> linv512, linv512t, linv512tmp;
    int pub_next = 0;
    bool pub_clean[2] = {false, false};
    int* solve_abort = nullptr;
    long ps_spin_limit = 6000000;
    int debug_pp_missing = -1;
    int debug_ps_missing = -1;
    mnk::DevBuf<unsigned long long> solve_trace;
    mnk::DevBuf<int> info_dev;
    mnk::DevBuf<unsigned long long> inertia_dev;
    unsigned long long* pin = nullptr;
    unsigned long long* pin_dev = nullptr;
    bool bk_requested = false;
    int bk_fallback = 1;
    int early_reject = 0;
    int reject_on_device = -1;
    bool src_persistent = false;
    bool factor_invalid = false;
    int64_t early_rejects = 0, early_reject_col = -1, early_reject_redone = 0;
    int probe = 1;
    mnk_ls* probe_ls = nullptr;
    int64_t probe_order = 0;
    int64_t probe_hint_col = -1;
    int probe_since_hint = 1 << 20;
    bool probe_last_rejected = false;
    int64_t probe_hits = 0, probe_misses = 0;
    int accept_only_pd = 0;
    double bk_growth_tol = 64.0, bk_growth_tol_qd = 1e8;
    double last_growth = 0.0;
    int64_t last_sign_changes = 0;
    mnk::DevBuf<unsigned long long> amax_dev;
    bool bk_active = false;
    int bk_count = 0;
    std::function<int()> retransfer;
    mnk::DevBuf<int> bk_perm, bk_ptype;
    mnk::DevBuf<double> bk_doff, bk_dcoup, bk_work;
    mnk::DevBuf<char> bk_state;
    mnk::DevBuf<double> bk_wv, bk_tmp;
    mnk::DevBuf<unsigned long long> bk_msg;
    mnk::DevBuf<int> bk_aux;
    int bk_panel_wgs = 0;
    int bk_max_wgs = 0;
    long bk_spin_limit = 1L << 21;
    int debug_bk_missing = -1;
    bool bk_multi_last = false, bk_mw_blocked = false;
    int bk_mw_fallbacks = 0;
    bool factorized = false, info_valid = false;
    int dag_debug = 0;
    mnk::DevBuf<int> dag_dbg;
    std::vector<int> dbg_flags, dbg_chain;
    bool spare_by_dag = false;
    int info = 0;
    int64_t npos = 0, nzero = 0, nneg = 0;
    mnk::DevBuf<double> qr_v, qr_t, qr_w, qr_p;
};

int64_t mnk_ls_effective_nbo(const mnk_ls* ls);
int mnk_qr_alloc(mnk_ls* ls);
int mnk_qr_factor(mnk_ls* ls);
int mnk_qr_solve(mnk_ls* ls, double* x, int64_t nrhs, int64_t ldx, int loc);
int mnk_ls_run_factorization(mnk_ls* ls);
int mnk_ls_run_factorization_now(mnk_ls* ls);
int mnk_ls_launch_finish_info(mnk_ls* ls, hipStream_t s);
bool mnk_solve_defer(mnk_ls* ls, double* xuser);
int mnk_solve_sync_deferred(mnk_ls* ls);
int mnk_solve_batch_flush_pending(void);
int mnk_ls_factorize_dense_dev_async(mnk_ls* ls, const double* Adev, int64_t lda);
double mnk_host_ms();
void mnk_add_process_stall_ms(double ms);
double mnk_process_stall_ms();
bool mnk_ls_pending_elsewhere(const mnk_ls* ls);
bool mnk_batch_active();
size_t mnk_pchain_sys_bytes();
int mnk_launch_pchain_multi(mnk_ls* const* v, int n, hipStream_t sp, hipStream_t fill_stream, void* table, int* const* front,
// ... 35 lines not shown
```

### madnlp.jl_amd/csrc/ls.hip

```cpp
#include <cstdarg>
#include <cstdlib>
#include <atomic>
#include <map>
#include <mutex>

#include <cfloat>
#include "ls.h"

namespace mnk {

static thread_local std::string g_err;
void set_error(const char* fmt, ...) {
    char buf[1024];
    va_list ap;
    va_start(ap, fmt);
    vsnprintf(buf, sizeof(buf), fmt, ap);
    va_end(ap);
    g_err = buf;
}

__global__ __launch_bounds__(256) void fill_lower_kernel(double* __restrict__ F, int64_t ld, int64_t N, int64_t Np) {
    const int64_t col = blockIdx.x;
    const int64_t first = (col / PAD) * PAD;
    const int64_t r = first + ((int64_t)blockIdx.y * 256 + threadIdx.x) * 2;
    if (r >= Np) return;
    double2 v = make_double2(0.0, 0.0);
    if (col >= N) {
        if (r == col) v.x = 1.0;
        if (r + 1 == col) v.y = 1.0;
    }
    *reinterpret_cast<double2*>(F + r + col * ld) = v;
}

__device__ __forceinline__ void wave_absmax_to(unsigned long long* word, double v) {
    double a = fabs(v);
    if (!(a <= DBL_MAX)) a = __longlong_as_double(0x7ff0000000000000LL);
    for (int off = 32; off > 0; off >>= 1) a = fmax(a, __shfl_xor(a, off));
    if ((threadIdx.x & 63) == 0 && a > 0.0) {
        const unsigned long long bits = (unsigned long long)__double_as_longlong(a);
        if (bits > __hip_atomic_load(word, __ATOMIC_RELAXED, __HIP_MEMORY_SCOPE_AGENT)) atomicMax(word, bits);
    }
}

__global__ void scatter_csc_kernel(double* __restrict__ F, int64_t ld, const int32_t* __restrict__ row,
                                   const int32_t* __restrict__ col, const double* __restrict__ nz, int64_t nnz,
                                   unsigned long long* __restrict__ amax, int32_t lim = INT32_MAX) {
    const int64_t k = blockIdx.x * (int64_t)blockDim.x + threadIdx.x;
    double v = 0.0;
    if (k < nnz && row[k] < lim && col[k] < lim) {
        v = nz[k];
        F[row[k] + (int64_t)col[k] * ld] = v;
    }
    if (amax != nullptr) wave_absmax_to(amax + AMAX_SLOT0 + AMAX_STRIDE * (blockIdx.x & (AMAX_SLOTS - 1)), v);
}

__global__ __launch_bounds__(256) void copy_lower_kernel(double* __restrict__ F, int64_t ld,
                                                         const double* __restrict__ A, int64_t lda, int64_t N,
                                                         int64_t Np, unsigned long long* __restrict__ amax) {
    const int64_t col = blockIdx.x;
    const int64_t first = (col / PAD) * PAD;
    const int64_t r0 = first + (int64_t)blockIdx.y * 1024 + threadIdx.x;
    if (r0 - threadIdx.x >= Np) return;
    double v[4], vl = 0.0;
#pragma unroll
    for (int i = 0; i < 4; ++i) {
        const int64_t r = r0 + 256 * i;
        v[i] = 0.0;
        if (r < Np) {
            if (col < N && r < N) {
                v[i] = A[r + col * lda];
                if (r >= col) vl = fmax(vl, fabs(v[i]));
                if (r >= col && !(fabs(v[i]) <= DBL_MAX)) vl = __longlong_as_double(0x7ff0000000000000LL);
            } else if (r == col) {
                v[i] = 1.0;
            }
        }
    }
#pragma unroll
    for (int i = 0; i < 4; ++i) {
        const int64_t r = r0 + 256 * i;
        if (r < Np) F[r + col * ld] = v[i];
    }
    if (amax != nullptr) {
        __shared__ double wmax[4];
        for (int off = 32; off > 0; off >>= 1) vl = fmax(vl, __shfl_xor(vl, off));
        if ((threadIdx.x & 63) == 0) wmax[threadIdx.x >> 6] = vl;
        __syncthreads();
        if (threadIdx.x < 64)
            wave_absmax_to(amax + AMAX_SLOT0 + AMAX_STRIDE * ((blockIdx.x + 5 * blockIdx.y) & (AMAX_SLOTS - 1)),
                           fmax(fmax(wmax[0], wmax[1]), fmax(wmax[2], wmax[3])));
    }
}

}

using namespace mnk;

static std::mutex g_ctx_mutex;
static std::atomic<int> g_live_ctx[64];
static std::vector<mnk_ctx*> g_ctx_list[64];

int mnk_live_contexts(int device) { return g_live_ctx[device & 63].load(std::memory_order_relaxed); }

std::recursive_mutex& mnk::launch_mutex() {
    static std::recursive_mutex m;
    return m;
}

namespace {
struct PersistSlot {
    hipEvent_t last = nullptr;
    bool recorded = false;
};
PersistSlot g_persist[64];
PersistSlot& persist_slot_of(mnk_ctx* ctx) {
    if (!ctx->partitioned) return g_persist[ctx->device & 63];
    if (ctx->persist_slot == nullptr) ctx->persist_slot = new PersistSlot();
    return *static_cast<PersistSlot*>(ctx->persist_slot);
}
}

void mnk::quiesce_persistent() {
    int cur = 0;
    const bool have_cur = hipGetDevice(&cur) == hipSuccess;
    for (int d = 0; d < 64; ++d) {
        PersistSlot& ps = g_persist[d];
        if (ps.last == nullptr || !ps.recorded) continue;
        (void)hipSetDevice(d);
        (void)hipEventSynchronize(ps.last);
    }
    if (have_cur) (void)hipSetDevice(cur);
    (void)hipGetLastError();
}

// ... 419 lines not shown
            }
        }
    }
    ls->Np = round_up(N, PAD);
    ls->ld = ls->Np;
    ls->ldw = ls->Np;
    int rc = 0;
    rc |= ls->fact.alloc((size_t)ls->ld * ls->Np + SLACK);
    rc |= ls->linv.alloc((size_t)(ls->Np / NBI) * NBI * NBI);
    rc |= ls->dblk.alloc((size_t)(ls->Np / NBI) * NBI * NBI);
    rc |= ls->inv16.alloc((size_t)(ls->Np / NBI) * 1024);
    rc |= ls->linv256.alloc((size_t)((ls->Np + 255) / 256) * 65536);
    rc |= ls->linv256t.alloc((size_t)((ls->Np + 255) / 256) * 65536);
    rc |= ls->dvec.alloc(ls->Np);
    rc |= ls->dinv.alloc(ls->Np);
    rc |= ls->xwork.alloc(10 * ls->Np);
    if (hipHostMalloc((void**)&ls->solve_abort, sizeof(int), hipHostMallocDefault) != hipSuccess) {
        (void)hipGetLastError();
        ls->solve_abort = nullptr;
        rc |= -2;
    } else {
        *ls->solve_abort = 0;
    }
    if (hipHostMalloc((void**)&ls->pin, 8 * sizeof(unsigned long long), hipHostMallocMapped) != hipSuccess ||
        hipHostGetDevicePointer((void**)&ls->pin_dev, ls->pin, 0) != hipSuccess) {
        (void)hipGetLastError();
        rc |= -2;
    }
    rc |= ls->info_dev.alloc(4);
    rc |= ls->inertia_dev.alloc(3);
    if (algo == MNK_QR) {
        rc |= mnk_qr_alloc(ls);
        ls->prefill = 0;
    }
    if (rc) { delete ls; return -2; }
    MNK_HIP(hipMemsetAsync(ls->fact.p, 0, ((size_t)ls->ld * ls->Np + SLACK) * sizeof(double), ctx->stream));
    mnk_ctx_child_added(ctx);
    *out = ls;
    return 0;
}

int mnk_ls_destroy(mnk_ls* ls) {
    if (!ls) return 0;
    (void)hipSetDevice(ls->ctx->device);
    if (mnk_ls_pending_elsewhere(ls)) {
        set_error("mnk_ls_destroy: a factorize! call of this solver is pending in a batch that another thread opened "
                  "(that thread's mnk_factorize_batch_end must come first); the solver was NOT destroyed");
        return -1;
    }
    (void)mnk_ls_sync_deferred(ls);
    (void)mnk::stream_wait(ls->ctx->stream);
    if (ls->probe_ls) { (void)mnk_ls_destroy(ls->probe_ls); ls->probe_ls = nullptr; }
    mnk::LaunchLock lock;
    mnk::quiesce_persistent();
    if (ls->solve_abort) (void)hipHostFree(ls->solve_abort);
    if (ls->pin) (void)hipHostFree(ls->pin);
    if (ls->ctx->s_fill) (void)mnk::stream_wait(ls->ctx->s_fill);
    if (ls->ev_spare) (void)hipEventDestroy(ls->ev_spare);
    if (ls->ev_free) (void)hipEventDestroy(ls->ev_free);
    if (ls->ev_defer) (void)hipEventDestroy(ls->ev_defer);
    if (ls->ev_info) (void)hipEventDestroy(ls->ev_info);
    mnk_ctx* ctx = ls->ctx;
    delete ls;
    mnk_ctx_child_gone(ctx);
    return 0;
}

int mnk_ls_set_option(mnk_ls* ls, const char* key, double value) {
    MNK_REQUIRE(ls && key, "mnk_ls_set_option: NULL argument");
    { int rc_d = mnk_ls_sync_deferred(ls); if (rc_d) return rc_d; }
    for (const std::string& k : ls->env_keys)
        if (k == key) {
            static std::mutex warn_mutex;
            static std::vector<std::string> warned;
            std::lock_guard<std::mutex> lock(warn_mutex);
            if (std::find(warned.begin(), warned.end(), k) == warned.end()) {
                warned.push_back(k);
                fprintf(stderr, "madnlp_hip: set_option('%s', %g) ignored: the option is pinned by MNK_OPTIONS / MNK_PANEL_ALGO / "
                                "MNK_PERSISTENT_SOLVE for this process (query: get_stat(\"pinned:%s\"))\n", key, value, key);
            }
            return 0;
        }
    if (!strcmp(key, "pivot_tol")) { ls->pivot_tol = value; return 0; }
    if (!strcmp(key, "split_a")) { ls->split_a = (int)value; return 0; }
    if (!strcmp(key, "tail_rows")) { ls->tail_rows = (int64_t)value; return 0; }
    if (!strcmp(key, "tail_nbo")) { ls->tail_nbo = (int64_t)value; return 0; }
    if (!strcmp(key, "own_cols")) { ls->own_cols = std::max<long>(64, (long)value / 64 * 64); return 0; }
    if (!strcmp(key, "panel0_whole")) { ls->panel0_whole = (int)value; return 0; }
    if (!strcmp(key, "dag_js2")) { ls->dag_js2_override = (int)value; return 0; }
    if (!strcmp(key, "outer_block")) {
        int64_t v = (int64_t)value;
        MNK_REQUIRE(v == 0 || (v >= NBI && v % NBI == 0), "outer_block must be 0 (by size) or a positive multiple of 64");
        ls->nbo_auto = v == 0;
        if (v > 0) ls->nbo = v;
        ls->wbuf[0].release();
        ls->wbuf[1].release();
        return 0;
    }
    if (!strcmp(key, "solve512")) { ls->solve512 = value != 0; return 0; }
    if (!strcmp(key, "solve512_min_rows")) { ls->solve512_min_rows = (int64_t)value; return 0; }
    if (!strcmp(key, "linv_mfma")) { ls->linv_mfma = value != 0.0; return 0; }
    if (!strcmp(key, "dag_chain_inline")) { ls->dag_chain_inline = value != 0.0; return 0; }
    if (!strcmp(key, "prefill")) { ls->prefill = value != 0; return 0; }
    if (!strcmp(key, "prefill_max_rows")) { ls->prefill_max_rows = (int64_t)value; return 0; }
    if (!strcmp(key, "single_rows")) {
        ls->single_rows = (int64_t)value;
        ls->wbuf[0].release();
        ls->wbuf[1].release();
        return 0;
    }
    if (!strcmp(key, "lookahead")) { ls->lookahead = value != 0.0; return 0; }
    if (!strcmp(key, "share")) { ls->share = (int)value; return 0; }
    if (!strcmp(key, "small_tiles")) { ls->small_tiles = (int)value; return 0; }
    if (!strcmp(key, "small_tiles_mid")) { ls->small_tiles_mid = (int)value; return 0; }
    if (!strcmp(key, "panel_algo")) {
        MNK_REQUIRE((int)value == 1 || (int)value == 4 || (int)value == 5, "panel_algo must be 1, 4 or 5");
        ls->panel_algo = (int)value;
        return 0;
    }
    if (!strcmp(key, "pp_fuse_rows")) { ls->pp_fuse_rows = (int64_t)value; return 0; }
    if (!strcmp(key, "dag_min_rows")) { ls->dag_min_rows = (int64_t)value; return 0; }
    if (!strcmp(key, "dag_taper0")) {
        MNK_REQUIRE(value >= 1.0 && value <= 16.0, "dag_taper0 must be in 1..16");
        ls->dag_taper0 = (int)value;
        ls->dag_tasks.release();
        return 0;
    }
    if (!strcmp(key, "dag_chunk")) {
        MNK_REQUIRE(value >= 1.0 && value <= 64.0, "dag_chunk must be in 1..64");
        ls->dag_chunk = (int)value;
        ls->dag_tasks.release();
        return 0;
    }
    if (!strcmp(key, "dag_band")) {
        MNK_REQUIRE(value >= 8.0 && value <= 64.0 && (int)value % 4 == 0 && (double)(int)value == value, "dag_band must be a multiple of 4 in 8..64");
        ls->dag_band = (int)value;
        ls->dag_tasks.release();
        return 0;
    }
    if (!strcmp(key, "dag_spin_limit")) {
        MNK_REQUIRE(value >= 1024.0, "dag_spin_limit must be at least 1024");
        ls->dag_spin_limit = (long)value;
        return 0;
    }
    if (!strcmp(key, "dag_fill")) { ls->dag_fill = value != 0.0; ls->dag_tasks.release(); return 0; }
    if (!strcmp(key, "batch_period")) { ls->batch_period = (int)value; return 0; }
    if (!strcmp(key, "dag_trace")) { ls->dag_trace_on = value != 0.0; return 0; }
    if (!strcmp(key, "dag_max_rows")) { ls->dag_max_rows = (int64_t)value; return 0; }
    if (!strcmp(key, "dag_deep_rows")) { ls->dag_deep_rows = (int64_t)value; ls->dag_tasks.release(); return 0; }
    if (!strcmp(key, "bk_fallback")) { ls->bk_fallback = (int)value; return 0; }
    if (!strcmp(key, "bk_panel_wgs")) {
        MNK_REQUIRE(value == 0.0 || value == 1.0, "bk_panel_wgs must be 0 or 1");
        ls->bk_panel_wgs = (int)value;
        return 0;
    }
    if (!strcmp(key, "accept_only_pd")) { ls->accept_only_pd = value != 0; return 0; }
    if (!strcmp(key, "probe")) { ls->probe = value != 0; return 0; }
    if (!strcmp(key, "early_reject")) { ls->early_reject = value != 0; return 0; }
    if (!strcmp(key, "dag_debug")) {
        ls->dag_debug = value != 0.0;
        if (ls->dag_debug && !ls->dag_dbg.p) {
            if (ls->dag_dbg.alloc(8 * 128 + 16 * 1024)) return -2;
            MNK_HIP(hipMemset(ls->dag_dbg.p, 0, (8 * 128 + 16 * 1024) * sizeof(int)));
        }
        return 0;
    }
// ... 27 lines not shown
    if (!strcmp(key, "debug_pp_missing")) { ls->debug_pp_missing = (int)value; return 0; }
    if (!strcmp(key, "debug_ps_missing")) { ls->debug_ps_missing = (int)value; return 0; }
    if (!strcmp(key, "solve_trace")) {
        if (value != 0.0) {
            int rc = ls->solve_trace.alloc((size_t)(ls->Np / 64) * 8);
            if (rc) return rc;
            MNK_HIP(hipMemset(ls->solve_trace.p, 0, (size_t)(ls->Np / 64) * 8 * sizeof(unsigned long long)));
        } else {
            ls->solve_trace.release();
        }
        return 0;
    }
    set_error("mnk_ls_set_option: unknown option '%s'", key);
    return -1;
}

static int ensure_wbuf(mnk_ls* ls) {
    if (ls->algo != MNK_LDL || ls->wbuf[0].p) return 0;
    const size_t cnt = (size_t)ls->ldw * std::min<int64_t>(mnk_ls_effective_nbo(ls), ls->Np) + SLACK;
    int rc = ls->wbuf[0].alloc(cnt);
    if (!rc && mnk_ls_effective_nbo(ls) < ls->Np) rc = ls->wbuf[1].alloc(cnt);
    return rc;
}

static unsigned long long* amax_word(mnk_ls* ls) {
    if (!(ls->bk_requested && ls->bk_fallback && ls->algo == MNK_LDL)) return nullptr;
    if (!ls->amax_dev.p && ls->amax_dev.alloc(AMAX_WORDS)) return nullptr;
    (void)hipMemsetAsync(ls->amax_dev.p, 0, AMAX_WORDS * sizeof(unsigned long long), ls->ctx->stream);
    return ls->amax_dev.p;
}

static int prepare_fill(mnk_ls* ls) {
    mnk_ctx* ctx = ls->ctx;
    hipStream_t s = ctx->stream;
    dim3 grid((unsigned)ls->Np, (unsigned)((ls->Np / 2 + 255) / 256));
    bool pre = ls->prefill && ls->Np <= ls->prefill_max_rows;
    if (pre && !ls->fact_spare.p) {
        if (ls->fact_spare.alloc(ls->fact.n) != 0) { (void)hipGetLastError(); ls->prefill = 0; pre = false; }
        if (pre && !ctx->s_fill && hipStreamCreateWithFlags(&ctx->s_fill, hipStreamNonBlocking) != hipSuccess) { ls->prefill = 0; pre = false; }
        if (pre && (hipEventCreateWithFlags(&ls->ev_spare, hipEventDisableTiming) != hipSuccess ||
                    hipEventCreateWithFlags(&ls->ev_free, hipEventDisableTiming) != hipSuccess)) { ls->prefill = 0; pre = false; }
        if (pre) MNK_HIP(hipMemsetAsync(ls->fact_spare.p, 0, ls->fact_spare.n * sizeof(double), s));
    }
    if (pre && ls->spare_zeroed && ls->spare_by_dag && !ls->info_valid) {
        ls->spare_zeroed = false;
        ls->spare_by_dag = false;
    }
    if (pre && ls->spare_zeroed) {
        std::swap(ls->fact.p, ls->fact_spare.p);
        MNK_HIP(hipStreamWaitEvent(s, ls->ev_spare, 0));
        ls->spare_zeroed = false;
    } else {
        hipLaunchKernelGGL(fill_lower_kernel, grid, dim3(256), 0, s, ls->fact.p, ls->ld, ls->N, ls->Np);
    }
    ls->spare_pending = pre;
    MNK_HIP(hipGetLastError());
    return 0;
}

}
int mnk_ls_prefill_spare(mnk_ls* ls) {
    if (!ls->spare_pending) return 0;
    ls->spare_pending = false;
    if (ls->dag_filled) {
        ls->dag_filled = false;
        MNK_HIP(hipEventRecord(ls->ev_spare, ls->ctx->stream));
        ls->spare_zeroed = true;
        ls->spare_by_dag = true;
        return 0;
    }
    ls->spare_by_dag = false;
    mnk_ctx* ctx = ls->ctx;
    dim3 grid((unsigned)ls->Np, (unsigned)((ls->Np / 2 + 255) / 256));
    MNK_HIP(hipEventRecord(ls->ev_free, ctx->stream));
    MNK_HIP(hipStreamWaitEvent(ctx->s_fill, ls->ev_free, 0));
    hipLaunchKernelGGL(fill_lower_kernel, grid, dim3(256), 0, ctx->s_fill, ls->fact_spare.p, ls->ld, ls->N, ls->Np);
    MNK_HIP(hipGetLastError());
    MNK_HIP(hipEventRecord(ls->ev_spare, ctx->s_fill));
    ls->spare_zeroed = true;
    return 0;
}
extern "C" {

static int transfer_sc(mnk_ls* ls, mnk_sc* sc) {
    int rc = prepare_fill(ls);
    if (rc) return rc;
    const int64_t nnz = sc->nnz_aug;
    hipLaunchKernelGGL(scatter_csc_kernel, dim3((unsigned)((nnz + 255) / 256)), dim3(256), 0, ls->ctx->stream,
                       ls->fact.p, ls->ld, sc->aug_row.p, sc->aug_col.p, sc->aug_nz.p, nnz, amax_word(ls),
                       ls->N < sc->n ? (int32_t)ls->N : INT32_MAX);
    MNK_HIP(hipGetLastError());
    return 0;
}

static int probe_leading_block(mnk_ls* ls, mnk_sc* sc, bool* rejected) {
    *rejected = false;
    if (!(ls->probe && ls->early_reject && ls->accept_only_pd && ls->algo == MNK_LDL && ls->N == sc->n && !mnk_batch_active())) return 0;
    if (ls->probe_last_rejected || ls->probe_hint_col < 0 || ls->probe_since_hint > 3) return 0;
    const int64_t m = (ls->probe_hint_col + 256) / 256 * 256;
    if (m < 512 || 2 * m > ls->N) return 0;
    if (ls->probe_ls == nullptr || ls->probe_order != m) {
        if (ls->probe_ls) { (void)mnk_ls_destroy(ls->probe_ls); ls->probe_ls = nullptr; }
        mnk_ls* child = nullptr;
        if (mnk_ls_create(ls->ctx, m, ls->algo, &child) != 0) { (void)hipGetLastError(); return 0; }
        child->probe = 0;
        child->accept_only_pd = 1;
        child->early_reject = 1;
        ls->probe_ls = child;
        ls->probe_order = m;
    }
    mnk_ls* c = ls->probe_ls;
    c->pivot_tol = ls->pivot_tol;
    int rc = mnk_ls_factorize_sc_async(c, sc);
    if (!rc) rc = mnk_ls_fetch_info(c);
    if (rc) return rc;
    if (c->npos == m && c->nzero == 0 && c->nneg == 0) { ++ls->probe_misses; return 0; }
    ++ls->probe_hits;
    ++ls->early_rejects;
    ls->early_reject_col = c->factor_invalid ? c->early_reject_col : m - 1;
    ls->info = 1;
    ls->npos = c->npos;
    ls->nzero = c->nzero;
    ls->nneg = ls->N - ls->npos - ls->nzero;
    ls->factor_invalid = true;
    ls->info_valid = true;
    ls->factorized = true;
    ls->bk_active = false;
    ls->probe_last_rejected = true;
    if (2 * ls->early_reject_col < ls->N) { ls->probe_hint_col = ls->early_reject_col; ls->probe_since_hint = 0; }
    *rejected = true;
    return 0;
}

int mnk_ls_factorize_sc_async(mnk_ls* ls, mnk_sc* sc) {
    MNK_REQUIRE(ls && sc && sc->ctx, "mnk_ls_factorize_sc: NULL argument or host-only handle");
    MNK_REQUIRE(sc->n >= ls->N, "mnk_ls_factorize_sc: the solver's order exceeds the KKT system's");
    MNK_HIP(hipSetDevice(ls->ctx->device));
    { int rc_d = mnk_ls_sync_deferred(ls); if (rc_d) return rc_d; }
    int rc = ensure_wbuf(ls);
    if (rc) return rc;
    bool probe_rejected = false;
    rc = probe_leading_block(ls, sc, &probe_rejected);
    if (rc) return rc;
    if (!probe_rejected) {
        rc = transfer_sc(ls, sc);
        if (rc) return rc;
    }
    ls->src_persistent = true;
    ls->retransfer = [ls, sc, w = std::weak_ptr<int>(sc->alive)]() {
        if (w.expired()) {
            set_error("factorize!: the KKT handle of the last factorize! call was destroyed before its inertia was fetched; the "
                      "matrix cannot be transferred again for the fall-back tier");
            return -5;
        }
        return transfer_sc(ls, sc);
    };
    if (probe_rejected) return 0;
    return mnk_ls_run_factorization(ls);
}

static int transfer_dense(mnk_ls* ls, const double* Adev, int64_t lda) {
    dim3 grid((unsigned)ls->Np, (unsigned)((ls->Np + 1023) / 1024));
    hipLaunchKernelGGL(copy_lower_kernel, grid, dim3(256), 0, ls->ctx->stream, ls->fact.p, ls->ld, Adev, lda,
                       ls->N, ls->Np, amax_word(ls));
    MNK_HIP(hipGetLastError());
    return 0;
}

static int factorize_dense_dev(mnk_ls* ls, const double* Adev, int64_t lda, bool src_persistent = false) {
    int rc = ensure_wbuf(ls);
    if (rc) return rc;
    rc = transfer_dense(ls, Adev, lda);
    if (rc) return rc;
    ls->src_persistent = src_persistent;
    ls->retransfer = [ls, Adev, lda]() { return transfer_dense(ls, Adev, lda); };
    return mnk_ls_run_factorization(ls);
}

}
int mnk_ls_factorize_dense_dev_async(mnk_ls* ls, const double* Adev, int64_t lda) {
    MNK_REQUIRE(ls && Adev && lda >= ls->N, "mnk_ls_factorize_dense_dev_async: bad argument");
    MNK_HIP(hipSetDevice(ls->ctx->device));
    { int rc_d = mnk_ls_sync_deferred(ls); if (rc_d) return rc_d; }
    return factorize_dense_dev(ls, Adev, lda);
}
extern "C" {

int mnk_ls_factorize_dc_async(mnk_ls* ls, mnk_dc* dc) {
    MNK_REQUIRE(ls && dc, "mnk_ls_factorize_dc: NULL argument");
    MNK_REQUIRE(dc->order == ls->N, "mnk_ls_factorize_dc: order mismatch");
    MNK_HIP(hipSetDevice(ls->ctx->device));
    { int rc_d = mnk_ls_sync_deferred(ls); if (rc_d) return rc_d; }
    int rc = factorize_dense_dev(ls, dc->aug.p, round_up(dc->order, PAD), true);
    ls->retransfer = [ls, dc, w = std::weak_ptr<int>(dc->alive)]() {
        if (w.expired()) {
            set_error("factorize!: the KKT handle of the last factorize! call was destroyed before its inertia was fetched; the "
                      "matrix cannot be transferred again for the fall-back tier");
            return -5;
        }
        return transfer_dense(ls, dc->aug.p, round_up(dc->order, PAD));
    };
    return rc;
}

static int finish_info(mnk_ls* ls, int* info) {
    int rc = mnk_ls_fetch_info(ls);
    if (rc) return rc;
    if (info) *info = ls->info;
    return 0;
}

int mnk_ls_factorize_sc(mnk_ls* ls, mnk_sc* sc, int* info) {
    int rc = mnk_ls_factorize_sc_async(ls, sc);
    return rc ? rc : finish_info(ls, info);
}

int mnk_ls_factorize_dc(mnk_ls* ls, mnk_dc* dc, int* info) {
    int rc = mnk_ls_factorize_dc_async(ls, dc);
    return rc ? rc : finish_info(ls, info);
}

int mnk_ls_factorize_dense(mnk_ls* ls, const double* A, int64_t lda, int loc, int* info) {
    MNK_REQUIRE(ls && A, "mnk_ls_factorize_dense: NULL argument");
    MNK_REQUIRE(lda >= ls->N, "mnk_ls_factorize_dense: lda < N");
    MNK_HIP(hipSetDevice(ls->ctx->device));
    { int rc_d = mnk_ls_sync_deferred(ls); if (rc_d) return rc_d; }
    int rc;
    if (loc == MNK_DEVICE) {
        rc = factorize_dense_dev(ls, A, lda);
    } else {
        DevBuf<double> tmp;
        rc = tmp.alloc((size_t)ls->N * ls->N);
        if (rc) return rc;
        MNK_HIP(mnk::h2d_copy_2d(tmp.p, ls->N * sizeof(double), A, lda * sizeof(double), ls->N * sizeof(double), ls->N,
                                 ls->ctx->stream));
        rc = factorize_dense_dev(ls, tmp.p, ls->N);
        MNK_HIP(mnk::stream_wait(ls->ctx->stream));
        if (!rc) rc = finish_info(ls, info);
        ls->retransfer = nullptr;
        return rc;
    }
    rc = rc ? rc : finish_info(ls, info);
    ls->retransfer = nullptr;
    return rc;
}

int mnk_ls_factorize_csc(mnk_ls* ls, const int32_t* colptr, const int32_t* rowval, const double* nzval,
                         int index_base, int* info) {
    MNK_REQUIRE(ls && colptr && rowval && nzval, "mnk_ls_factorize_csc: NULL argument");
    MNK_HIP(hipSetDevice(ls->ctx->device));
    { int rc_d = mnk_ls_sync_deferred(ls); if (rc_d) return rc_d; }
    const int64_t N = ls->N;
    const int64_t nnz = colptr[N] - index_base;
    std::vector<int32_t> row(nnz), col(nnz);
    for (int64_t c = 0; c < N; ++c)
        for (int64_t k = colptr[c] - index_base; k < colptr[c + 1] - index_base; ++k) {
            row[k] = rowval[k] - index_base;
            col[k] = (int32_t)c;
            MNK_REQUIRE(row[k] >= c && row[k] < N, "mnk_ls_factorize_csc: matrix must be lower triangular");
        }
    DevBuf<int32_t> drow, dcol;
    DevBuf<double> dnz;
    std::vector<double> nzv(nzval, nzval + nnz);
    int rc = drow.upload(row, ls->ctx->stream);
    rc |= dcol.upload(col, ls->ctx->stream);
    rc |= dnz.upload(nzv, ls->ctx->stream);
    if (rc) return -2;
    rc = ensure_wbuf(ls);
    if (rc) return rc;
    auto transfer = [ls, nnz, &drow, &dcol, &dnz]() -> int {
        int r = prepare_fill(ls);
        if (r) return r;
        if (nnz > 0)
            hipLaunchKernelGGL(scatter_csc_kernel, dim3((unsigned)((nnz + 255) / 256)), dim3(256), 0, ls->ctx->stream,
                               ls->fact.p, ls->ld, drow.p, dcol.p, dnz.p, nnz, amax_word(ls));
        MNK_HIP(hipGetLastError());
        return 0;
    };
    rc = transfer();
    if (rc) return rc;
    ls->src_persistent = false;
    ls->retransfer = transfer;
    rc = mnk_ls_run_factorization(ls);
    if (!rc) {
        MNK_HIP(mnk::stream_wait(ls->ctx->stream));
        rc = finish_info(ls, info);
    }
    ls->retransfer = nullptr;
    return rc;
}

int mnk_ls_inertia(mnk_ls* ls, int64_t* num_pos, int64_t* num_zero, int64_t* num_neg) {
    MNK_REQUIRE(ls, "mnk_ls_inertia: NULL argument");
    MNK_REQUIRE(ls->algo != MNK_QR, "mnk_ls_inertia: a QR factorization reveals no inertia (is_inertia is false for QR)");
    { int rc_d = mnk_ls_sync_deferred(ls); if (rc_d) return rc_d; }
    MNK_REQUIRE(ls->factorized, "mnk_ls_inertia: factorize first");
    MNK_HIP(hipSetDevice(ls->ctx->device));
    int rc = mnk_ls_fetch_info(ls);
    if (rc) return rc;
    if (num_pos) *num_pos = ls->npos;
    if (num_zero) *num_zero = ls->nzero;
    if (num_neg) *num_neg = ls->nneg;
    return 0;
}

int mnk_ls_check_solve(mnk_ls* ls) {
    MNK_REQUIRE(ls, "mnk_ls_check_solve: NULL argument");
    MNK_HIP(hipSetDevice(ls->ctx->device));
    { int rc_q = mnk_solve_sync_deferred(ls); if (rc_q) return rc_q; }
    MNK_HIP(mnk::stream_wait(ls->ctx->stream));
    if (mnk_ls_take_solve_abort(ls)) {
        set_error("mnk_ls_check_solve: a persistent solve on device-resident data gave up waiting for a peer workgroup "
                  "(device oversubscribed by another process?); its result is invalid -- solve again "
                  "(persistent_solve is now off for this solver)");
        return -3;
    }
    return 0;
}

static int ensure_complete_factor(mnk_ls* ls, const char* who) {
    if (ls->reject_on_device == 1) { int rc_i = mnk_ls_fetch_info(ls); if (rc_i) return rc_i; }
    if (!ls->factor_invalid) return 0;
    { static const bool peek = getenv("MNK_DBG_NO_REDO") != nullptr; if (peek) return 0; }
    if (!ls->retransfer) {
        set_error("%s: the last factorization was stopped at its first non-positive pivot (early_reject) and its source is gone: "
                  "there is no factor", who);
        return -1;
    }
    const int keep = ls->early_reject;
    ls->early_reject = 0;
    int rc = ls->retransfer();
    if (!rc) rc = mnk_ls_run_factorization(ls);
    if (!rc) rc = mnk_ls_fetch_info(ls);
    ls->early_reject = keep;
    ++ls->early_reject_redone;
    return rc;
}

int mnk_ls_solve(mnk_ls* ls, double* x, int64_t nrhs, int64_t ldx, int loc) {
    MNK_REQUIRE(ls && x, "mnk_ls_solve: NULL argument");
    { int rc_d = mnk_ls_sync_deferred_fact(ls); if (rc_d) return rc_d; }
    MNK_REQUIRE(ls->factorized, "mnk_ls_solve: factorize first");
    MNK_HIP(hipSetDevice(ls->ctx->device));
    { int rc_f = ensure_complete_factor(ls, "mnk_ls_solve"); if (rc_f) return rc_f; }
    MNK_REQUIRE(nrhs >= 1 && ldx >= ls->N, "mnk_ls_solve: bad nrhs/ldx");
    MNK_HIP(hipSetDevice(ls->ctx->device));
    if (ls->algo == MNK_QR) return mnk_qr_solve(ls, x, nrhs, ldx, loc);
    if (ls->solve_abort && *ls->solve_abort != 0) {
        *ls->solve_abort = 0;
        ls->persistent_solve = 0;
        ls->pub_clean[0] = ls->pub_clean[1] = false;
        set_error("mnk_ls_solve: an earlier persistent solve on device-resident data gave up waiting for a peer "
                  "workgroup (device oversubscribed by another process?); its result is invalid -- refactorize/solve "
                  "again (persistent_solve is now off for this solver)");
        return -3;
    }
    hipStream_t s = ls->ctx->stream;
    const int64_t N = ls->N, Np = ls->Np;
    double* w = ls->xwork.p;
    for (int64_t k = 0; k < nrhs; ++k) {
        double* xk = x + k * ldx;
        if (loc == MNK_DEVICE) {
            if (nrhs == 1 && mnk_solve_defer(ls, xk)) continue;
            int rc = mnk_solve_sync_deferred(ls);
            if (rc) return rc;
            rc = mnk_ls_run_solve(ls, w, xk);
            if (rc) return rc;
            continue;
        }
        { int rc_q = mnk_solve_sync_deferred(ls); if (rc_q) return rc_q; }
        MNK_HIP(hipMemsetAsync(w, 0, Np * sizeof(double), s));
        MNK_HIP(mnk::h2d_copy(w, xk, N * sizeof(double), s));
// ... 41 lines not shown
int mnk_ls_solve_batch(int n, mnk_ls* const* ls, double* const* x, int loc) {
    MNK_REQUIRE(n >= 0 && (n == 0 || (ls && x)), "mnk_ls_solve_batch: NULL argument");
    int rc = mnk_solve_batch_begin();
    if (rc) return rc;
    for (int i = 0; i < n && !rc; ++i) rc = mnk_ls_solve(ls[i], x[i], 1, ls[i]->N, loc);
    const int rc_end = mnk_solve_batch_end();
    return rc ? rc : rc_end;
}

int mnk_ls_debug_dag_state(mnk_ls* ls, int* flags, int64_t nflags, int* chain, int64_t nchain, int* have) {
    MNK_REQUIRE(ls && have, "mnk_ls_debug_dag_state: NULL argument");
    *have = ls->dbg_flags.empty() ? 0 : 1;
    if (flags) memcpy(flags, ls->dbg_flags.data(), sizeof(int) * (size_t)std::min<int64_t>(nflags, (int64_t)ls->dbg_flags.size()));
    if (chain) memcpy(chain, ls->dbg_chain.data(), sizeof(int) * (size_t)std::min<int64_t>(nchain, (int64_t)ls->dbg_chain.size()));
    return 0;
}

int mnk_ls_debug_solve_trace(mnk_ls* ls, unsigned long long* out, int64_t n) {
    if (ls && out && ls->dag_trace.p && ls->dag_trace_on) {
        MNK_HIP(hipSetDevice(ls->ctx->device));
        MNK_HIP(mnk::stream_wait(ls->ctx->stream));
        const int64_t cnt = std::min<int64_t>(n, (int64_t)ls->dag_trace.n);
        MNK_HIP(mnk::d2h_copy(out, ls->dag_trace.p, cnt * sizeof(unsigned long long), ls->ctx->stream));
        return 0;
    }
    MNK_REQUIRE(ls && out && ls->solve_trace.p, "mnk_ls_debug_solve_trace: tracing is off (option solve_trace)");
    MNK_HIP(hipSetDevice(ls->ctx->device));
    MNK_HIP(mnk::stream_wait(ls->ctx->stream));
    const int64_t cnt = std::min<int64_t>(n, (ls->Np / 64) * 8);
    MNK_HIP(mnk::d2h_copy(out, ls->solve_trace.p, cnt * sizeof(unsigned long long), ls->ctx->stream));
    return 0;
}

int mnk_ls_get_factor(mnk_ls* ls, double* L, double* D, int loc) {
    MNK_REQUIRE(ls && L, "mnk_ls_get_factor: NULL argument");
    { int rc_d = mnk_ls_sync_deferred(ls); if (rc_d) return rc_d; }
    MNK_REQUIRE(ls->factorized, "mnk_ls_get_factor: factorize first");
    { int rc_f = ensure_complete_factor(ls, "mnk_ls_get_factor"); if (rc_f) return rc_f; }
    MNK_HIP(hipSetDevice(ls->ctx->device));
    hipStream_t s = ls->ctx->stream;
    if (loc == MNK_DEVICE) {
        MNK_HIP(hipMemcpy2DAsync(L, ls->N * sizeof(double), ls->fact.p, ls->ld * sizeof(double), ls->N * sizeof(double), ls->N,
                                 hipMemcpyDeviceToDevice, s));
        if (D) MNK_HIP(hipMemcpyAsync(D, ls->dvec.p, ls->N * sizeof(double), hipMemcpyDeviceToDevice, s));
        MNK_HIP(mnk::stream_wait(s));
    } else {
        MNK_HIP(mnk::d2h_copy_2d(L, ls->N * sizeof(double), ls->fact.p, ls->ld * sizeof(double), ls->N * sizeof(double), ls->N, s));
        if (D) MNK_HIP(mnk::d2h_copy(D, ls->dvec.p, ls->N * sizeof(double), s));
    }
    return 0;
}

int mnk_ls_get_stat(mnk_ls* ls, const char* key, double* value) {
    MNK_REQUIRE(ls && key && value, "mnk_ls_get_stat: NULL argument");
    MNK_HIP(hipSetDevice(ls->ctx->device));
    { int rc_d = mnk_ls_sync_deferred(ls); if (rc_d) return rc_d; }
    if (ls->factorized) {
        int rc = mnk_ls_fetch_info(ls);
        if (rc) return rc;
    }
    if (!strncmp(key, "pinned:", 7)) {
        *value = std::find(ls->env_keys.begin(), ls->env_keys.end(), std::string(key + 7)) != ls->env_keys.end() ? 1.0 : 0.0;
        return 0;
    }
    if (!strcmp(key, "panel_algo")) { *value = ls->algo_now; return 0; }
    if (!strcmp(key, "pp_fallbacks")) { *value = ls->pp_fallbacks; return 0; }
    if (!strcmp(key, "timeout_site")) { *value = ls->last_timeout_site; return 0; }
    if (!strcmp(key, "probe_hits")) { *value = (double)ls->probe_hits; return 0; }
    if (!strcmp(key, "probe_misses")) { *value = (double)ls->probe_misses; return 0; }
    if (!strcmp(key, "early_rejects")) { *value = (double)ls->early_rejects; return 0; }
    if (!strcmp(key, "early_reject_redone")) { *value = (double)ls->early_reject_redone; return 0; }
    if (!strcmp(key, "early_reject_col")) { *value = (double)ls->early_reject_col; return 0; }
    if (!strcmp(key, "stall_ms_total")) { *value = ls->stall_ms_total; return 0; }
    if (!strcmp(key, "stall_ms_process")) { *value = mnk_process_stall_ms(); return 0; }
    if (!strcmp(key, "growth")) { *value = ls->last_growth; return 0; }
    if (!strcmp(key, "sign_changes")) { *value = (double)ls->last_sign_changes; return 0; }
    if (!strcmp(key, "bk_count")) { *value = ls->bk_count; return 0; }
    if (!strcmp(key, "bk_panel_multi")) { *value = ls->bk_multi_last ? 1.0 : 0.0; return 0; }
    if (!strcmp(key, "bk_mw_fallbacks")) { *value = ls->bk_mw_fallbacks; return 0; }
    if (!strcmp(key, "dag_bulk_wgs")) { *value = ls->ctx->dag_cus > 0 ? mnk_ctx_bulk_wgs(ls->ctx, ls->ctx->dag_cus, 3) : 0; return 0; }
    if (!strcmp(key, "dag_ntasks")) { *value = ls->dag_ntasks; return 0; }
    if (!strcmp(key, "dag_ntasks1")) { *value = ls->dag_ntasks1; return 0; }
    if (!strcmp(key, "dag_js2")) { *value = ls->dag_js2; return 0; }
    set_error("mnk_ls_get_stat: unknown key '%s'", key);
    return -1;
}

int mnk_ls_bk_info(mnk_ls* ls, int* active, int* count, int32_t* perm, double* doff) {
    MNK_REQUIRE(ls, "mnk_ls_bk_info: NULL argument");
    MNK_HIP(hipSetDevice(ls->ctx->device));
    { int rc_d = mnk_ls_sync_deferred(ls); if (rc_d) return rc_d; }
    if (ls->factorized) {
        int rc = mnk_ls_fetch_info(ls);
        if (rc) return rc;
    }
    if (active) *active = ls->bk_active ? 1 : 0;
    if (count) *count = ls->bk_count;
    if (ls->bk_active && (perm || doff)) {
        hipStream_t s = ls->ctx->stream;
        if (perm) MNK_HIP(mnk::d2h_copy(perm, ls->bk_perm.p, ls->N * sizeof(int32_t), s));
        if (doff) MNK_HIP(mnk::d2h_copy(doff, ls->bk_doff.p, ls->N * sizeof(double), s));
    }
    return 0;
}

int mnk_gemm_nt(mnk_ctx* ctx, int mode, int64_t M, int64_t N, int64_t K, const double* A, int64_t lda,
                const double* B, int64_t ldb, double* C, int64_t ldc) {
    MNK_REQUIRE(ctx && A && B && C, "mnk_gemm_nt: NULL argument");
    MNK_HIP(hipSetDevice(ctx->device));
    return launch_gemm_nt(ctx->stream, mode, M, N, K, A, lda, B, ldb, C, ldc, nullptr, nullptr, 0, nullptr);
}

__global__ void clock_probe_kernel(unsigned long long* out, int iters, double a, double b) {
    double x = (double)threadIdx.x;
    const unsigned long long t0 = wall_clock64();
    for (int i = 0; i < iters; ++i) {
#pragma unroll
        for (int j = 0; j < 16; ++j) x = __builtin_fma(x, a, b);
    }
    const unsigned long long t1 = wall_clock64();
    if (threadIdx.x == 0) out[0] = t1 - t0;
    if (x == 1.2345) out[1] = 1;
}

int mnk_debug_update(mnk_ctx* ctx, int variant, int64_t M, int64_t K, const double* A, int64_t lda, double* C,
                     double* C2, int64_t ldc, int reps, double* ms) {
    MNK_REQUIRE(ctx && A && C && ms, "mnk_debug_update: NULL argument");
    MNK_HIP(hipSetDevice(ctx->device));
    { int rc_s = mnk_ctx_ensure_panel_streams(ctx); if (rc_s) return rc_s; }
    hipStream_t s = ctx->stream, su = ctx->su, sp = ctx->sp;
    MNK_REQUIRE(su && sp, "mnk_debug_update: no look-ahead streams");
    DevBuf<int> ctr;
    int rc = ctr.alloc(8 * (size_t)reps);
    if (rc) return rc;
    MNK_HIP(hipMemsetAsync(ctr.p, 0, 8 * (size_t)reps * sizeof(int), s));
    hipEvent_t e0, e1;
    MNK_HIP(hipEventCreate(&e0));
    MNK_HIP(hipEventCreate(&e1));
    const int pcus = ctx->panel_cus, ucus = ctx->num_cu - pcus;
    MNK_HIP(hipEventRecord(e0, s));
    MNK_HIP(hipEventRecord(ctx->ev_a, s));
    MNK_HIP(hipStreamWaitEvent(su, ctx->ev_a, 0));
    MNK_HIP(hipStreamWaitEvent(sp, ctx->ev_a, 0));
    for (int r = 0; r < reps && !rc; ++r) {
        switch (variant) {
        case 0: rc = launch_gemm_nt(s, 2, M, M, K, A, lda, A, lda, C, ldc, nullptr, nullptr, 0, nullptr); break;
        case 1: rc = launch_gemm_nt_queue(s, M, M, K, A, lda, A, lda, C, ldc, ctr.p + 8 * r, ctx->num_cu, nullptr); break;
        case 2: rc = launch_gemm_nt(su, 2, M, M, K, A, lda, A, lda, C, ldc, nullptr, nullptr, 0, nullptr); break;
        case 3: rc = launch_gemm_nt_queue(su, M, M, K, A, lda, A, lda, C, ldc, ctr.p + 8 * r, ucus, nullptr); break;
        case 4:
            rc = launch_gemm_nt_queue(su, M, M, K, A, lda, A, lda, C, ldc, ctr.p + 8 * r, ucus, nullptr);
            if (!rc) rc = launch_gemm_nt_queue(sp, M, M, K, A, lda, A, lda, C, ldc, ctr.p + 8 * r, pcus, nullptr);
            break;
        case 20: break;
        case 21: rc = launch_gemm_nt(su, 2, M, M, K, A, lda, A, lda, C, ldc, nullptr, nullptr, 0, nullptr); break;
        case 9: rc = launch_gemm_nt_dbg(s, 1, M, M, K, A, lda, A, lda, C, ldc); break;
        case 10: rc = launch_gemm_nt_dbg(su, 1, M, M, K, A, lda, A, lda, C, ldc); break;
        case 11: rc = launch_gemm_nt_dbg(su, 2, M, M, K, A, lda, A, lda, C, ldc); break;
        case 12: rc = launch_gemm_nt_dbg(su, 3, M, M, K, A, lda, A, lda, C, ldc); break;
        case 13: rc = launch_gemm_nt_dbg(su, 5, M, M, K, A, lda, A, lda, C, ldc); break;
        case 14: rc = launch_gemm_nt_dbg(s, 5, M, M, K, A, lda, A, lda, C, ldc); break;
        case 15: rc = launch_gemm_nt_dbg(su, 6, M, M, K, A, lda, A, lda, C, ldc); break;
        case 16: rc = launch_gemm_nt_dbg(s, 6, M, M, K, A, lda, A, lda, C, ldc); break;
        case 6: case 7: case 8: {
            const int chunk = variant == 6 ? 2 * ctx->num_cu : variant == 7 ? 4 * ctx->num_cu : ctx->num_cu;
            const int nt = gemm_nt_lower_tiles(M, M);
// ... 36 lines not shown
```

### madnlp.jl_amd/csrc/sparse_kkt.hip

```cpp
#pragma clang fp contract(off)

#include <algorithm>
#include <numeric>

#include "ls.h"
#include "kkt_vec.h"

namespace mnk {

__global__ void segsum_kernel(double* __restrict__ dst, const double* __restrict__ src,
                              const int32_t* __restrict__ ptr, const int32_t* __restrict__ idx, int64_t nseg) {
    const int64_t s = blockIdx.x * (int64_t)blockDim.x + threadIdx.x;
    if (s >= nseg) return;
    double acc = 0.0;
    for (int32_t k = ptr[s]; k < ptr[s + 1]; ++k) acc += src[idx[k]];
    dst[s] = acc;
}

__global__ void condense_kernel(double* __restrict__ K, const double* __restrict__ Hnz,
                                const double* __restrict__ pr_diag, const double* __restrict__ du,
                                double* __restrict__ Dout, double* __restrict__ pr_keep, double* __restrict__ du_keep,
                                const double* __restrict__ Jt, const int32_t* __restrict__ hptr,
                                const int32_t* __restrict__ hsrc, const int32_t* __restrict__ dsrc,
                                const int32_t* __restrict__ jptr, const int32_t* __restrict__ jc,
// ... 140 lines not shown
    for (int64_t k = 0; k < nnzj; ++k) {
        jtI[k] = jac_J[k] - index_base;
        jtJ[k] = jac_I[k] - index_base;
        MNK_REQUIRE(jtI[k] >= 0 && jtI[k] < n && jtJ[k] >= 0 && jtJ[k] < m, "mnk_sc_create: Jacobian index out of range");
    }
    for (int64_t k = 0; k < nnzh; ++k) {
        int32_t i = hess_I[k] - index_base, j = hess_J[k] - index_base;
        MNK_REQUIRE(i >= 0 && i < n && j >= 0 && j < n, "mnk_sc_create: Hessian index out of range");
        if (j > i) std::swap(i, j);
        hI[k] = i;
        hJ[k] = j;
    }
    mnk_sc* sc = new mnk_sc();
    sc->ctx = ctx;
    sc->n = n; sc->m = m; sc->nnzj = nnzj; sc->nnzh = nnzh;
    CscPattern jt = coo_to_csc(n, m, jtI, jtJ);
    CscPattern hh = coo_to_csc(n, n, hI, hJ);
    sc->jt_colptr = jt.colptr; sc->jt_rowval = jt.rowval; sc->jt_map = jt.map;
    sc->h_colptr = hh.colptr; sc->h_rowval = hh.rowval; sc->h_map = hh.map;
    sc->nnz_jt = (int64_t)jt.rowval.size();
    sc->nnz_hess = (int64_t)hh.rowval.size();

    int64_t L = 0;
    for (int64_t c = 0; c < m; ++c) {
        const int64_t k = jt.colptr[c + 1] - jt.colptr[c];
        L += k * (k + 1) / 2;
    }
    const int64_t T = n + sc->nnz_hess + L;
    MNK_REQUIRE(T < (int64_t)2000000000, "mnk_sc_create: symbolic structure exceeds int32 range");
    std::vector<int64_t> key(T);
    std::vector<int8_t> kind(T);
    std::vector<int32_t> sa(T), sb(T), scc(T);
    int64_t t = 0;
    for (int64_t i = 0; i < n; ++i, ++t) { key[t] = i * n + i; kind[t] = -1; sa[t] = (int32_t)i; sb[t] = 0; scc[t] = 0; }
    {
        std::vector<int32_t> hcol = col_index(hh.colptr);
        for (int64_t k = 0; k < sc->nnz_hess; ++k, ++t) {
            key[t] = (int64_t)hcol[k] * n + hh.rowval[k]; kind[t] = 0; sa[t] = (int32_t)k; sb[t] = 0; scc[t] = 0;
        }
    }
    for (int64_t c = 0; c < m; ++c)
        for (int32_t j = jt.colptr[c]; j < jt.colptr[c + 1]; ++j)
            for (int32_t k = j; k < jt.colptr[c + 1]; ++k, ++t) {
                const int64_t c1 = jt.rowval[j], c2 = jt.rowval[k];
                key[t] = c1 * n + c2;
                kind[t] = 1; sa[t] = (int32_t)c; sb[t] = j; scc[t] = k;
            }
    std::vector<int64_t> ord(T);
    std::iota(ord.begin(), ord.end(), 0);
    std::stable_sort(ord.begin(), ord.end(), [&](int64_t a, int64_t b) { return key[a] < key[b]; });

    std::vector<int32_t> a_hptr, a_hsrc, a_dsrc, a_jptr, a_jc, a_jk, a_jl, a_row, a_col;
    sc->aug_colptr.assign(n + 1, 0);
    int64_t slot = -1, prev = -1;
    for (int64_t q = 0; q < T; ++q) {
        const int64_t e = ord[q];
        if (key[e] != prev) {
            prev = key[e];
            ++slot;
            const int32_t col = (int32_t)(key[e] / n), row = (int32_t)(key[e] % n);
            a_row.push_back(row); a_col.push_back(col);
            sc->aug_rowval.push_back(row);
            sc->aug_colptr[col + 1]++;
            a_hptr.push_back((int32_t)a_hsrc.size());
            a_jptr.push_back((int32_t)a_jc.size());
            a_dsrc.push_back(-1);
        }
        if (kind[e] == -1) {
            a_dsrc[slot] = sa[e];
            sc->d_dst.push_back((int32_t)slot); sc->d_src.push_back(sa[e]);
        } else if (kind[e] == 0) {
            a_hsrc.push_back(sa[e]);
            sc->hp_dst.push_back((int32_t)slot); sc->hp_src.push_back(sa[e]);
        } else {
            a_jc.push_back(sa[e]); a_jk.push_back(sb[e]); a_jl.push_back(scc[e]);
            sc->j_dst.push_back((int32_t)slot); sc->j_c.push_back(sa[e]); sc->j_k.push_back(sb[e]); sc->j_l.push_back(scc[e]);
        }
    }
    a_hptr.push_back((int32_t)a_hsrc.size());
    a_jptr.push_back((int32_t)a_jc.size());
    for (int64_t c = 0; c < n; ++c) sc->aug_colptr[c + 1] += sc->aug_colptr[c];
    sc->nnz_aug = slot + 1;
    sc->len_jptr = L;

    if (!ctx) { *out = sc; return 0; }
    hipStream_t s = ctx->stream;
    std::vector<int32_t> ptr, src;
    int rc = 0;
    group_by_slot(jt.map, sc->nnz_jt, ptr, src);
    rc |= sc->jt_seg_ptr.upload(ptr, s); rc |= sc->jt_seg_src.upload(src, s);
    group_by_slot(hh.map, sc->nnz_hess, ptr, src);
    rc |= sc->h_seg_ptr.upload(ptr, s); rc |= sc->h_seg_src.upload(src, s);
    rc |= sc->aug_hptr.upload(a_hptr, s); rc |= sc->aug_hsrc.upload(a_hsrc, s);
    rc |= sc->aug_dsrc.upload(a_dsrc, s);
    rc |= sc->aug_jptr.upload(a_jptr, s); rc |= sc->aug_jc.upload(a_jc, s);
    rc |= sc->aug_jk.upload(a_jk, s); rc |= sc->aug_jl.upload(a_jl, s);
    rc |= sc->aug_row.upload(a_row, s); rc |= sc->aug_col.upload(a_col, s);
    rc |= sc->d_jt_colptr.upload(sc->jt_colptr, s); rc |= sc->d_jt_rowval.upload(sc->jt_rowval, s);
    rc |= sc->d_h_colptr.upload(sc->h_colptr, s); rc |= sc->d_h_rowval.upload(sc->h_rowval, s);
    rc |= sc->jac_coo.alloc(nnzj); rc |= sc->hess_coo.alloc(nnzh);
    rc |= sc->jt_nz.alloc(sc->nnz_jt); rc |= sc->h_nz.alloc(sc->nnz_hess); rc |= sc->aug_nz.alloc(sc->nnz_aug);
    rc |= sc->diag_buffer.alloc(m); rc |= sc->pr_diag.alloc(n + m); rc |= sc->du_diag.alloc(m);

    mnk_sc_spmv_data* sp = new mnk_sc_spmv_data();
    {
        std::vector<int32_t> rp(n + 1, 0), ri(sc->nnz_jt), rperm(sc->nnz_jt);
        for (int32_t r : jt.rowval) rp[r + 1]++;
        for (int64_t i = 0; i < n; ++i) rp[i + 1] += rp[i];
        std::vector<int32_t> cur(rp.begin(), rp.end() - 1);
        for (int64_t c = 0; c < m; ++c)
            for (int32_t k = jt.colptr[c]; k < jt.colptr[c + 1]; ++k) {
                const int32_t p = cur[jt.rowval[k]]++;
                ri[p] = (int32_t)c; rperm[p] = k;
            }
        rc |= sp->jtr_ptr.upload(rp, s); rc |= sp->jtr_idx.upload(ri, s); rc |= sp->jtr_perm.upload(rperm, s);
    }
    {
        std::vector<int32_t> cnt(n + 1, 0);
        std::vector<int32_t> hcol = col_index(hh.colptr);
        for (int64_t k = 0; k < sc->nnz_hess; ++k) {
            cnt[hcol[k] + 1]++;
            if (hh.rowval[k] != hcol[k]) cnt[hh.rowval[k] + 1]++;
        }
        for (int64_t i = 0; i < n; ++i) cnt[i + 1] += cnt[i];
        std::vector<int32_t> idx(cnt[n]), perm(cnt[n]), cur(cnt.begin(), cnt.end() - 1);
        for (int64_t k = 0; k < sc->nnz_hess; ++k)
            if (hh.rowval[k] != hcol[k]) { const int32_t p = cur[hh.rowval[k]]++; idx[p] = hcol[k]; perm[p] = (int32_t)k; }
        for (int64_t k = 0; k < sc->nnz_hess; ++k) { const int32_t p = cur[hcol[k]]++; idx[p] = hh.rowval[k]; perm[p] = (int32_t)k; }
        rc |= sp->hs_ptr.upload(cnt, s); rc |= sp->hs_idx.upload(idx, s); rc |= sp->hs_perm.upload(perm, s);
    }
    if (rc) { delete sp; delete sc; return -2; }
    MNK_HIP(hipMemsetAsync(sc->jt_nz.p, 0, sc->jt_nz.n * sizeof(double), s));
    MNK_HIP(hipMemsetAsync(sc->h_nz.p, 0, sc->h_nz.n * sizeof(double), s));
    MNK_HIP(hipMemsetAsync(sc->aug_nz.p, 0, sc->aug_nz.n * sizeof(double), s));
    sc->extra = sp;
    mnk_ctx_child_added(ctx);
    *out = sc;
    return 0;
}

int mnk_sc_destroy(mnk_sc* sc) {
    if (!sc) return 0;
    if (sc->ctx) {
        (void)hipSetDevice(sc->ctx->device);
        (void)mnk::stream_wait(sc->ctx->stream);
    }
    delete spmv_of(sc);
    sc->extra = nullptr;
    mnk_ctx* ctx = sc->ctx;
    delete sc;
    mnk_ctx_child_gone(ctx);
    return 0;
}

int mnk_sc_sizes(mnk_sc* sc, int64_t* nnz_jt, int64_t* nnz_hess, int64_t* nnz_aug, int64_t* len_jptr) {
    MNK_REQUIRE(sc, "mnk_sc_sizes: NULL argument");
    if (nnz_jt) *nnz_jt = sc->nnz_jt;
    if (nnz_hess) *nnz_hess = sc->nnz_hess;
    if (nnz_aug) *nnz_aug = sc->nnz_aug;
    if (len_jptr) *len_jptr = sc->len_jptr;
    return 0;
}

int mnk_sc_get_structure(mnk_sc* sc, int which, int32_t* colptr, int32_t* rowval) {
    MNK_REQUIRE(sc && colptr && rowval, "mnk_sc_get_structure: NULL argument");
    const std::vector<int32_t>*cp, *rv;
    if (which == MNK_SC_JT) { cp = &sc->jt_colptr; rv = &sc->jt_rowval; }
    else if (which == MNK_SC_HESS) { cp = &sc->h_colptr; rv = &sc->h_rowval; }
    else if (which == MNK_SC_AUG) { cp = &sc->aug_colptr; rv = &sc->aug_rowval; }
    else { set_error("mnk_sc_get_structure: bad selector %d", which); return -1; }
    std::copy(cp->begin(), cp->end(), colptr);
    std::copy(rv->begin(), rv->end(), rowval);
    return 0;
}

int mnk_sc_get_map(mnk_sc* sc, int which, int64_t* map) {
    MNK_REQUIRE(sc && map, "mnk_sc_get_map: NULL argument");
    const std::vector<int64_t>* mp = which == MNK_SC_JT ? &sc->jt_map : which == MNK_SC_HESS ? &sc->h_map : nullptr;
    MNK_REQUIRE(mp != nullptr, "mnk_sc_get_map: bad selector");
    std::copy(mp->begin(), mp->end(), map);
    return 0;
}

int mnk_sc_get_ptrs(mnk_sc* sc, int32_t* d_dst, int32_t* d_src, int32_t* h_dst, int32_t* h_src, int32_t* j_dst,
                    int32_t* j_c, int32_t* j_k, int32_t* j_l) {
    MNK_REQUIRE(sc, "mnk_sc_get_ptrs: NULL argument");
    auto cp = [](const std::vector<int32_t>& v, int32_t* o) { if (o) std::copy(v.begin(), v.end(), o); };
    cp(sc->d_dst, d_dst); cp(sc->d_src, d_src); cp(sc->hp_dst, h_dst); cp(sc->hp_src, h_src);
    cp(sc->j_dst, j_dst); cp(sc->j_c, j_c); cp(sc->j_k, j_k); cp(sc->j_l, j_l);
    return 0;
}

static int stage_in(mnk_ctx* ctx, double* dev, const double* src, int64_t n, int loc, const double** use) {
    if (loc == MNK_DEVICE) { *use = src; return 0; }
    if (n > 0) {
        MNK_HIP(mnk::h2d_copy(dev, src, n * sizeof(double), ctx->stream));
    }
    *use = dev;
    return 0;
}

int mnk_sc_compress_jacobian(mnk_sc* sc, const double* jac_coo, int loc) {
    MNK_REQUIRE(sc && sc->ctx && (jac_coo || sc->nnzj == 0), "mnk_sc_compress_jacobian: NULL argument or host-only handle");
    MNK_HIP(hipSetDevice(sc->ctx->device));
    const double* src;
    int rc = stage_in(sc->ctx, sc->jac_coo.p, jac_coo, sc->nnzj, loc, &src);
    if (rc) return rc;
    if (sc->nnz_jt > 0)
        hipLaunchKernelGGL(segsum_kernel, dim3((unsigned)((sc->nnz_jt + 255) / 256)), dim3(256), 0, sc->ctx->stream,
                           sc->jt_nz.p, src, sc->jt_seg_ptr.p, sc->jt_seg_src.p, sc->nnz_jt);
    MNK_HIP(hipGetLastError());
    return 0;
}

int mnk_sc_compress_hessian(mnk_sc* sc, const double* hess_coo, int loc) {
    MNK_REQUIRE(sc && sc->ctx && (hess_coo || sc->nnzh == 0), "mnk_sc_compress_hessian: NULL argument or host-only handle");
    MNK_HIP(hipSetDevice(sc->ctx->device));
    const double* src;
    int rc = stage_in(sc->ctx, sc->hess_coo.p, hess_coo, sc->nnzh, loc, &src);
    if (rc) return rc;
    if (sc->nnz_hess > 0)
        hipLaunchKernelGGL(segsum_kernel, dim3((unsigned)((sc->nnz_hess + 255) / 256)), dim3(256), 0, sc->ctx->stream,
                           sc->h_nz.p, src, sc->h_seg_ptr.p, sc->h_seg_src.p, sc->nnz_hess);
    MNK_HIP(hipGetLastError());
    return 0;
}

int mnk_sc_build(mnk_sc* sc, const double* pr_diag, const double* du_diag, int loc) {
    MNK_REQUIRE(sc && sc->ctx, "mnk_sc_build: NULL argument or host-only handle");
    MNK_HIP(hipSetDevice(sc->ctx->device));
    hipStream_t s = sc->ctx->stream;
    if (pr_diag == nullptr && du_diag == nullptr) {
        mnk_sc_spmv_data* sp0 = spmv_of(sc);
        MNK_REQUIRE(sp0 != nullptr && sp0->have_diag, "mnk_sc_build: no diagonals given and mnk_sc_set_aug_diagonal was not called");
        pr_diag = sc->pr_diag.p;
        du_diag = sc->du_diag.p;
        loc = MNK_DEVICE;
    }
    MNK_REQUIRE(pr_diag && (du_diag || sc->m == 0), "mnk_sc_build: NULL argument");
    const double *pr, *du;
    int rc = stage_in(sc->ctx, sc->pr_diag.p, pr_diag, sc->n + sc->m, loc, &pr);
    rc |= stage_in(sc->ctx, sc->du_diag.p, du_diag, sc->m, loc, &du);
    if (rc) return rc;
    const bool keep = loc == MNK_DEVICE && pr != sc->pr_diag.p;
// ... 282 lines not shown
```

Baseline: 99.67 it/s.

## Skip leading zero k-steps in DAG LDL tiles using a sparsity envelope

Computes a per-128-tile envelope on the host from the sparse KKT pattern: the first nonzero column block for each row tile. The DAG factorization kernels use it to start each tile's update GEMM at the envelope instead of kbeg. Final tiles that lie entirely outside the envelope are zeroed or skipped, so no multiply work is spent on structurally zero leading blocks. A device gate word disables the skip whenever the scatter kernel sees a non-finite value. This adds host envelope computation, extra per-task reads and some control flow, and its correctness depends on fill never reaching outside the envelope.

```diff
diff --git a/include/madnlp_hip.h b/include/madnlp_hip.h
--- a/include/madnlp_hip.h
+++ b/include/madnlp_hip.h
@@ -262,6 +262,9 @@
 int mnk_debug_dag_merged_tasks(int ntile, int chunk, int band_tiles, int js2, int taper0, int fill, int ninst, int period,
                                int* out, int cap);
 
+int mnk_sc_debug_tile_env(mnk_sc* sc, int64_t order, int32_t* out, int cap);
+int mnk_debug_tile_env_csc(int64_t n, const int32_t* colptr, const int32_t* rowval, int index_base, int32_t* out, int cap);
+
 int mnk_debug_update(mnk_ctx* ctx, int variant, int64_t M, int64_t K, const double* A, int64_t lda,
                      double* C, double* C2, int64_t ldc, int reps, double* ms);
 
diff --git a/madnlp.jl_amd/_lib.py b/madnlp.jl_amd/_lib.py
--- a/madnlp.jl_amd/_lib.py
+++ b/madnlp.jl_amd/_lib.py
@@ -209,6 +209,8 @@
     "mnk_debug_shader_clock": (C.c_int, [_vp, _vp]),
     "mnk_debug_dag_tasks": (C.c_int, [C.c_int, C.c_int, C.c_int, C.c_int, C.c_int, _vp, C.c_int, _vp]),
     "mnk_debug_dag_merged_tasks": (C.c_int, [C.c_int] * 8 + [_vp, C.c_int]),
+    "mnk_sc_debug_tile_env": (C.c_int, [_vp, C.c_int64, _vp, C.c_int]),
+    "mnk_debug_tile_env_csc": (C.c_int, [C.c_int64, _vp, _vp, C.c_int, _vp, C.c_int]),
     "mnk_factorize_batch_begin": (C.c_int, []),
     "mnk_factorize_batch_end": (C.c_int, []),
     "mnk_solve_batch_begin": (C.c_int, []),
diff --git a/madnlp.jl_amd/csrc/dag.hip b/madnlp.jl_amd/csrc/dag.hip
--- a/madnlp.jl_amd/csrc/dag.hip
+++ b/madnlp.jl_amd/csrc/dag.hip
@@ -26,6 +26,8 @@
     unsigned long long* vmax;
     double* zfill;
     int64_t N;
+    const int* env;
+    const int* envgate;
 };
 
 typedef const DagInst __attribute__((address_space(4))) * DagInstP;
@@ -274,12 +276,14 @@
 }
 
 __global__ __launch_bounds__(256) void dag_reset_kernel(int* __restrict__ flags, int64_t n, int* __restrict__ info, DagInst rec,
-                                                        DagInst* __restrict__ rec_dst, const SmallSysRec* __restrict__ recs = nullptr) {
+                                                        DagInst* __restrict__ rec_dst, const SmallSysRec* __restrict__ recs = nullptr,
+                                                        int* __restrict__ envw = nullptr) {
     if (recs != nullptr) {
         const SmallSysRec r = recs[blockIdx.y];
         flags = r.flags; n = r.nflags; info = r.info;
     }
     if (blockIdx.x == 0 && threadIdx.x == 0 && rec_dst != nullptr) *rec_dst = rec;
+    if (blockIdx.x == 0 && threadIdx.x == 0 && envw != nullptr) { envw[1] = envw[0]; envw[0] = 0; }
     int4* f4 = reinterpret_cast<int4*>(flags);
     const int64_t n4 = n / 4, stride = (int64_t)gridDim.x * blockDim.x;
     for (int64_t i = (int64_t)blockIdx.x * blockDim.x + threadIdx.x; i < n4; i += stride) f4[i] = make_int4(0, 0, 0, 0);
@@ -304,6 +308,12 @@
         }
         *reinterpret_cast<double2*>(Z + row + col * ld) = v;
     }
+}
+
+__device__ __forceinline__ void dag_zero_tile(double* Z, int64_t ld, int64_t row0, int64_t col0, int tid) {
+    const int r2 = (tid & 63) * 2, cg = tid >> 6;
+#pragma unroll 4
+    for (int c = cg; c < 128; c += 4) *reinterpret_cast<double2*>(Z + row0 + r2 + (col0 + c) * ld) = make_double2(0.0, 0.0);
 }
 
 template <bool LDL>
@@ -348,18 +358,27 @@
         __syncthreads();
         auto run_task = [&]() __attribute__((always_inline)) -> bool {
         if (dead) return false;
+        int eI = 0, k0 = kbeg;
+        if (in->env != nullptr && __builtin_amdgcn_readfirstlane(*in->envgate) == 0) {
+            eI = __builtin_amdgcn_readfirstlane(in->env[I]);
+            k0 = min(kend, max(kbeg, max(eI, __builtin_amdgcn_readfirstlane(in->env[J]))));
+        }
         int limit = 0;
+        auto gate_at = [&](int kc) -> int {
+            const unsigned long long w0 = tr ? wall_clock64() : 0;
+            const int r = dag_wait_front(in, a.spin_limit, 2 * I, 2 * I + 1, 2 * J, 2 * J + 1, kc, kend, &s_val);
+            if (tr) { const unsigned long long w1 = wall_clock64(); tr[2] = w1; tr[6] += 1; tr[7] += w1 - w0; s_stat[1] += w1 - w0; }
+            return r;
+        };
         auto gate = [&](int kt) -> bool {
             if (kt < limit) return true;
-            const unsigned long long w0 = tr ? wall_clock64() : 0;
-            const int r = dag_wait_front(in, a.spin_limit, 2 * I, 2 * I + 1, 2 * J, 2 * J + 1, kbeg + (kt >> 4), kend, &s_val);
-            if (tr) { const unsigned long long w1 = wall_clock64(); tr[2] = w1; tr[6] += 1; tr[7] += w1 - w0; s_stat[1] += w1 - w0; }
+            const int r = gate_at(k0 + (kt >> 4));
             if (r < 0) return false;
-            limit = (__builtin_amdgcn_readfirstlane(r) - kbeg) * 16;
+            limit = (__builtin_amdgcn_readfirstlane(r) - k0) * 16;
             return true;
         };
-        const double* Ak = in->F + (a.fake_share > 0 ? (int64_t)128 * (kend + I % a.fake_share) : row0) + (int64_t)128 * kbeg * in->ld;
-        const double* Bk = (LDL ? in->V : in->F) + (a.fake_share > 0 ? (int64_t)128 * (kend + J % a.fake_share) : col0) + (int64_t)128 * kbeg * in->ld;
+        const double* Ak = in->F + (a.fake_share > 0 ? (int64_t)128 * (kend + I % a.fake_share) : row0) + (int64_t)128 * k0 * in->ld;
+        const double* Bk = (LDL ? in->V : in->F) + (a.fake_share > 0 ? (int64_t)128 * (kend + J % a.fake_share) : col0) + (int64_t)128 * k0 * in->ld;
         auto wait_chunk_order = [&]() -> bool {
             if (flags & DAG_FIRST) return true;
             const int* word = in->tprog + (int64_t)I * a.ntile + J;
@@ -371,6 +390,11 @@
         if ((flags & DAG_FINAL) && !(flags & DAG_BANDACC)) {
             __builtin_amdgcn_s_setprio(3);
             if (!wait_chunk_order()) return false;
+            if (J < eI) {
+                if (kend > kbeg && gate_at(kbeg) < 0) return false;
+                if (LDL) dag_zero_tile(in->V, in->ld, row0, col0, tid);
+                return true;
+            }
             v4f64 X[8][2];
             {
                 const int lane = tid & 63, w = tid >> 6;
@@ -384,8 +408,8 @@
                         X[cb][1][r] = cp[16];
                     }
             }
-            if (kend > kbeg && !gate(0)) return false;
-            (void)gemm_nt_mainloop3<2, 8, true>(X, Ak, in->ld, Bk, in->ld, (kend - kbeg) * 16, smem_raw, tid);
+            if (kend > kbeg && gate_at(kbeg) < 0) return false;
+            if (kend > k0) (void)gemm_nt_mainloop3<2, 8, true>(X, Ak, in->ld, Bk, in->ld, (kend - k0) * 16, smem_raw, tid);
 #pragma unroll
             for (int i = 0; i < 8; ++i) { asm volatile("" : "+v"(X[i][0])); asm volatile("" : "+v"(X[i][1])); }
             if (tr) tr[1] = tr[3] = wall_clock64();
@@ -393,17 +417,17 @@
             if (tr) { tr[4] = wall_clock64(); s_stat[1] += tr[4] - tr[3]; }
             dag_finalize_tile<LDL>(in, row0, col0, 2 * J, smem_raw, tid, X, tr);
             if (tr) s_stat[3] += wall_clock64() - tr[4];
-        } else if (!(MNK_DAG_DIAG_SUB && I == J && kend > kbeg)) {
+        } else if (!(MNK_DAG_DIAG_SUB && I == J && kend > k0)) {
             v4f64 acc[4][4];
 #pragma unroll
             for (int i = 0; i < 4; ++i)
 #pragma unroll
                 for (int j = 0; j < 4; ++j) acc[i][j] = v4f64{0.0, 0.0, 0.0, 0.0};
             if (flags & DAG_FINAL) __builtin_amdgcn_s_setprio(3);
-            if (!gemm_nt_mainloop<2, 2, 4, 0, 8>(acc, Ak, in->ld, Bk, in->ld, (kend - kbeg) * 16, smem_raw, tid, gate)) return false;
+            if (!gemm_nt_mainloop<2, 2, 4, 0, 8>(acc, Ak, in->ld, Bk, in->ld, (kend - k0) * 16, smem_raw, tid, gate)) return false;
             if (tr) tr[1] = wall_clock64();
             if (!wait_chunk_order()) return false;
-            if (kend > kbeg)
+            if (kend > k0)
                 gemm_nt_epilogue<2, 2, 4, 2, false, true>(acc, row0, col0, (int64_t)1 << 40, (int64_t)1 << 40, in->F, in->ld, nullptr, nullptr, 0, tid);
             if (tr) tr[3] = wall_clock64();
         } else {
@@ -415,7 +439,7 @@
             __builtin_amdgcn_s_setprio(3);
             if (!wait_chunk_order()) return false;
             gemm_nt_load_neg_lower<2, 2, 4>(acc, row0, col0, in->F, in->ld, tid);
-            if (!gemm_nt_mainloop<2, 2, 4, 0, 8>(acc, Ak, in->ld, Bk, in->ld, (kend - kbeg) * 16, smem_raw, tid, gate)) return false;
+            if (!gemm_nt_mainloop<2, 2, 4, 0, 8>(acc, Ak, in->ld, Bk, in->ld, (kend - k0) * 16, smem_raw, tid, gate)) return false;
             if (tr) tr[1] = wall_clock64();
             gemm_nt_store_neg_lower<2, 2, 4>(acc, row0, col0, in->F, in->ld, tid);
             if (tr) tr[3] = wall_clock64();
@@ -467,6 +491,8 @@
     int fake_share;
     double* zfill;
     int64_t N;
+    const int* env;
+    const int* envgate;
 #if MNK_DIAG_BULK_DBG
     int* bdbg;
 #endif
@@ -485,6 +511,7 @@
     __shared__ int s_val;
     __shared__ unsigned long long s_stat[4];
     if (threadIdx.x < 4) s_stat[threadIdx.x] = 0;
+    const int* __restrict__ env = a.env != nullptr && __builtin_amdgcn_readfirstlane(*a.envgate) == 0 ? a.env : nullptr;
     __syncthreads();
     for (;;) {
         int tid = threadIdx.x;
@@ -523,18 +550,27 @@
             continue;
         }
 
+        int eI = 0, k0 = kbeg;
+        if (env != nullptr) {
+            eI = __builtin_amdgcn_readfirstlane(env[I]);
+            k0 = min(kend, max(kbeg, max(eI, __builtin_amdgcn_readfirstlane(env[J]))));
+        }
         int limit = 0;
+        auto gate_at = [&](int kc) -> int {
+            const unsigned long long w0 = tr ? wall_clock64() : 0;
+            const int r = dag_wait_front(&a, a.spin_limit, 2 * I, 2 * I + 1, 2 * J, 2 * J + 1, kc, kend, &s_val, MNK_BDBG(a));
+            if (tr) { const unsigned long long w1 = wall_clock64(); tr[2] = w1; tr[6] += 1; tr[7] += w1 - w0; s_stat[1] += w1 - w0; }
+            return r;
+        };
         auto gate = [&](int kt) -> bool {
             if (kt < limit) return true;
-            const unsigned long long w0 = tr ? wall_clock64() : 0;
-            const int r = dag_wait_front(&a, a.spin_limit, 2 * I, 2 * I + 1, 2 * J, 2 * J + 1, kbeg + (kt >> 4), kend, &s_val, MNK_BDBG(a));
-            if (tr) { const unsigned long long w1 = wall_clock64(); tr[2] = w1; tr[6] += 1; tr[7] += w1 - w0; s_stat[1] += w1 - w0; }
+            const int r = gate_at(k0 + (kt >> 4));
             if (r < 0) return false;
-            limit = (__builtin_amdgcn_readfirstlane(r) - kbeg) * 16;
+            limit = (__builtin_amdgcn_readfirstlane(r) - k0) * 16;
             return true;
         };
-        const double* Ak = a.F + (a.fake_share > 0 ? (int64_t)128 * (kend + I % a.fake_share) : row0) + (int64_t)128 * kbeg * a.ld;
-        const double* Bk = (LDL ? a.V : a.F) + (a.fake_share > 0 ? (int64_t)128 * (kend + J % a.fake_share) : col0) + (int64_t)128 * kbeg * a.ld;
+        const double* Ak = a.F + (a.fake_share > 0 ? (int64_t)128 * (kend + I % a.fake_share) : row0) + (int64_t)128 * k0 * a.ld;
+        const double* Bk = (LDL ? a.V : a.F) + (a.fake_share > 0 ? (int64_t)128 * (kend + J % a.fake_share) : col0) + (int64_t)128 * k0 * a.ld;
         auto wait_chunk_order = [&]() -> bool {
             if (flags & DAG_FIRST) return true;
             const int* word = a.tprog + (int64_t)I * a.ntile + J;
@@ -546,6 +582,11 @@
         if ((flags & DAG_FINAL) && !(flags & DAG_BANDACC)) {
             __builtin_amdgcn_s_setprio(3);
             if (!wait_chunk_order()) return;
+            if (J < eI) {
+                if (kend > kbeg && gate_at(kbeg) < 0) return;
+                if (LDL) dag_zero_tile(a.V, a.ld, row0, col0, tid);
+                goto publish;
+            }
             v4f64 X[8][2];
             {
                 const int lane = tid & 63, w = tid >> 6;
@@ -559,8 +600,8 @@
                         X[cb][1][r] = cp[16];
                     }
             }
-            if (kend > kbeg && !gate(0)) return;
-            (void)gemm_nt_mainloop3<2, 8, true>(X, Ak, a.ld, Bk, a.ld, (kend - kbeg) * 16, smem_raw, tid);
+            if (kend > kbeg && gate_at(kbeg) < 0) return;
+            if (kend > k0) (void)gemm_nt_mainloop3<2, 8, true>(X, Ak, a.ld, Bk, a.ld, (kend - k0) * 16, smem_raw, tid);
 #pragma unroll
             for (int i = 0; i < 8; ++i) { asm volatile("" : "+v"(X[i][0])); asm volatile("" : "+v"(X[i][1])); }
             if (tr) tr[1] = tr[3] = wall_clock64();
@@ -568,17 +609,17 @@
             if (tr) { tr[4] = wall_clock64(); s_stat[1] += tr[4] - tr[3]; }
             dag_finalize_tile<LDL>(&a, row0, col0, 2 * J, smem_raw, tid, X, tr);
             if (tr) s_stat[3] += wall_clock64() - tr[4];
-        } else if (!(MNK_DAG_DIAG_SUB && I == J && kend > kbeg)) {
+        } else if (!(MNK_DAG_DIAG_SUB && I == J && kend > k0)) {
             v4f64 acc[4][4];
 #pragma unroll
             for (int i = 0; i < 4; ++i)
 #pragma unroll
                 for (int j = 0; j < 4; ++j) acc[i][j] = v4f64{0.0, 0.0, 0.0, 0.0};
             if (flags & DAG_FINAL) __builtin_amdgcn_s_setprio(3);
-            if (!gemm_nt_mainloop<2, 2, 4, 0, 8>(acc, Ak, a.ld, Bk, a.ld, (kend - kbeg) * 16, smem_raw, tid, gate)) return;
+            if (!gemm_nt_mainloop<2, 2, 4, 0, 8>(acc, Ak, a.ld, Bk, a.ld, (kend - k0) * 16, smem_raw, tid, gate)) return;
             if (tr) tr[1] = wall_clock64();
             if (!wait_chunk_order()) return;
-            if (kend > kbeg)
+            if (kend > k0)
                 gemm_nt_epilogue<2, 2, 4, 2, false, true>(acc, row0, col0, (int64_t)1 << 40, (int64_t)1 << 40, a.F, a.ld, nullptr, nullptr, 0, tid);
             if (tr) tr[3] = wall_clock64();
         } else {
@@ -590,11 +631,12 @@
             __builtin_amdgcn_s_setprio(3);
             if (!wait_chunk_order()) return;
             gemm_nt_load_neg_lower<2, 2, 4>(acc, row0, col0, a.F, a.ld, tid);
-            if (!gemm_nt_mainloop<2, 2, 4, 0, 8>(acc, Ak, a.ld, Bk, a.ld, (kend - kbeg) * 16, smem_raw, tid, gate)) return;
+            if (!gemm_nt_mainloop<2, 2, 4, 0, 8>(acc, Ak, a.ld, Bk, a.ld, (kend - k0) * 16, smem_raw, tid, gate)) return;
             if (tr) tr[1] = wall_clock64();
             gemm_nt_store_neg_lower<2, 2, 4>(acc, row0, col0, a.F, a.ld, tid);
             if (tr) tr[3] = wall_clock64();
         }
+    publish:
         asm volatile("s_waitcnt vmcnt(0)" ::: "memory");
         __syncthreads();
         if (tid == 0) {
@@ -754,7 +796,7 @@
     static const int fake = getenv("MNK_DAG_FAKE_SHARE") ? atoi(getenv("MNK_DAG_FAKE_SHARE")) : 0;
     if (insts == nullptr) {
         DagArgs1 a{one.F, one.ld, one.V, one.dinv, one.dblk, one.inv16, reinterpret_cast<const int4*>(tasks), ntasks, one.front, one.af,
-                   one.tprog, ntile, qctr, one.info, spin_limit, trace, wgstat, one.vmax, fake, one.zfill, one.N};
+                   one.tprog, ntile, qctr, one.info, spin_limit, trace, wgstat, one.vmax, fake, one.zfill, one.N, one.env, one.envgate};
 #if MNK_DIAG_BULK_DBG
         a.bdbg = g_diag_bdbg;
 #endif
@@ -807,8 +849,10 @@
     int* af = front + nblk;
     int* tprog = af + (size_t)ntile * ntile;
     double* zfill = (ls->dag_fill && ls->dag_has_fill && ls->spare_pending && ls->fact_spare.p && !ls->spare_zeroed) ? ls->fact_spare.p : nullptr;
+    const bool env = ls->envelope && ls->env_dev != nullptr && ls->env_word.p != nullptr;
     return mnk::DagInst{ls->fact.p, ls->ld, ls->algo == MNK_LDL ? ls->vfull.p : nullptr, ls->dinv.p, ls->dblk.p, ls->inv16.p,
-                        front, af, tprog, ls->info_dev.p, mnk_ls_growth_word(ls), zfill, ls->N};
+                        front, af, tprog, ls->info_dev.p, mnk_ls_growth_word(ls), zfill, ls->N, env ? ls->env_dev : nullptr,
+                        env ? ls->env_word.p + 1 : nullptr};
 }
 
 int mnk_ls_dag_prepare(mnk_ls* ls) {
@@ -871,8 +915,11 @@
     MNK_REQUIRE(ls->dag_tasks.p && ls->dag_flags.p && (!ldl || ls->vfull.p), "task-DAG schedule: mnk_ls_dag_prepare was not called");
     const mnk::DagInst inst = dag_instance(ls);
     ls->dag_filled = inst.zfill != nullptr;
+    ls->env_used = inst.env != nullptr;
     hipLaunchKernelGGL(mnk::dag_reset_kernel, dim3((unsigned)std::min<size_t>((nflags + 1023) / 1024, 64)), dim3(256), 0, s,
-                       ls->dag_flags.p, (int64_t)nflags, ls->info_dev.p, inst, (mnk::DagInst*)nullptr);
+                       ls->dag_flags.p, (int64_t)nflags, ls->info_dev.p, inst, (mnk::DagInst*)nullptr, (const mnk::SmallSysRec*)nullptr,
+                       ls->env_word.p);
+    ls->env_armed = false;
     int* qctr = ls->dag_flags.p;
     int* front = inst.front;
     const long spin_limit = mnk_ls_dag_spin_limit(ls);
@@ -1018,8 +1065,11 @@
         for (mnk_ls* ls : g) {
             hin.push_back(dag_instance(ls));
             ls->dag_filled = hin.back().zfill != nullptr;
+            ls->env_used = hin.back().env != nullptr;
             hipLaunchKernelGGL(mnk::dag_reset_kernel, dim3((unsigned)std::min<size_t>((nflags + 1023) / 1024, 64)), dim3(256), 0, h,
-                               ls->dag_flags.p, (int64_t)nflags, ls->info_dev.p, hin.back(), insts_dev + (hin.size() - 1));
+                               ls->dag_flags.p, (int64_t)nflags, ls->info_dev.p, hin.back(), insts_dev + (hin.size() - 1),
+                               (const mnk::SmallSysRec*)nullptr, ls->env_word.p);
+            ls->env_armed = false;
         }
         MNK_HIP(hipMemsetAsync(B.qctr.p, 0, 4 * sizeof(int), h));
         hipStream_t sp[2] = {c0->sp_dag, c0->sp_dagB}, su = c0->su_dagB;
@@ -1147,6 +1197,9 @@
                 mnk_ls* ls = g[r0 + i];
                 hin.push_back(dag_instance(ls));
                 ls->dag_filled = hin.back().zfill != nullptr;
+                hin.back().env = nullptr;
+                hin.back().envgate = nullptr;
+                ls->env_used = false;
                 fronts.push_back(hin.back().front);
                 afs.push_back(hin.back().af);
                 st_inst[i] = hin.back();
diff --git a/madnlp.jl_amd/csrc/factor.hip b/madnlp.jl_amd/csrc/factor.hip
--- a/madnlp.jl_amd/csrc/factor.hip
+++ b/madnlp.jl_amd/csrc/factor.hip
@@ -1192,6 +1192,7 @@
         }
     }
     ls->algo_now = ls->panel_algo;
+    ls->env_used = false;
     const int64_t min_rows = mnk_batch_active() ? std::min<int64_t>(ls->dag_min_rows, 256) : ls->dag_min_rows;
     if (ls->algo_now == 5 && (ctx->dag_cus < ls->dag_band || !ls->lookahead || Np < min_rows || Np > ls->dag_max_rows)) ls->algo_now = 4;
     if (ls->algo_now == 5 && ctx->sp_dag == nullptr && mnk_ctx_ensure_dag(ctx) != 0) { (void)hipGetLastError(); ls->algo_now = 4; }
diff --git a/madnlp.jl_amd/csrc/ls.h b/madnlp.jl_amd/csrc/ls.h
--- a/madnlp.jl_amd/csrc/ls.h
+++ b/madnlp.jl_amd/csrc/ls.h
@@ -12,6 +12,8 @@
     int64_t n = 0, m = 0, nnzj = 0, nnzh = 0;
     int64_t nnz_jt = 0, nnz_hess = 0, nnz_aug = 0, len_jptr = 0;
     std::vector<int32_t> jt_colptr, jt_rowval, h_colptr, h_rowval, aug_colptr, aug_rowval;
+    std::vector<int32_t> tile_env;
+    mnk::DevBuf<int32_t> d_tile_env;
     std::vector<int64_t> jt_map, h_map;
     std::vector<int32_t> d_dst, d_src, hp_dst, hp_src, j_dst, j_c, j_k, j_l;
     mnk::DevBuf<int32_t> jt_seg_ptr, jt_seg_src, h_seg_ptr, h_seg_src;
@@ -24,6 +26,21 @@
     void* extra = nullptr;
     std::shared_ptr<int> alive = std::make_shared<int>(0);
 };
+
+inline std::vector<int32_t> mnk_tile_envelope(int64_t n, const int32_t* row, const int32_t* col, int64_t nnz) {
+    std::vector<int32_t> fnz(n);
+    for (int64_t i = 0; i < n; ++i) fnz[i] = (int32_t)i;
+    for (int64_t k = 0; k < nnz; ++k)
+        if (row[k] >= 0 && row[k] < n && col[k] < fnz[row[k]]) fnz[row[k]] = col[k];
+    const int64_t ntile = (n + 127) / 128;
+    std::vector<int32_t> env(ntile);
+    for (int64_t I = 0; I < ntile; ++I) {
+        int32_t f = (int32_t)(128 * I);
+        for (int64_t i = 128 * I; i < std::min<int64_t>(n, 128 * I + 128); ++i) f = std::min(f, fnz[i]);
+        env[I] = f / 128;
+    }
+    return env;
+}
 
 struct mnk_dc {
     mnk_ctx* ctx = nullptr;
@@ -94,6 +111,13 @@
     int dag_chunk = 64;
     int64_t dag_min_rows = 1280;
     int64_t dag_deep_rows = 5376;
+    int envelope = 1;
+    const int32_t* env_dev = nullptr;
+    std::vector<int32_t> env_host;
+    mnk::DevBuf<int32_t> env_own;
+    mnk::DevBuf<int> env_word;
+    bool env_used = false;
+    bool env_armed = false;
     int64_t dag_max_rows = 30720;
     int panel_algo = 5;
     int persistent_solve = 1;
diff --git a/madnlp.jl_amd/csrc/ls.hip b/madnlp.jl_amd/csrc/ls.hip
--- a/madnlp.jl_amd/csrc/ls.hip
+++ b/madnlp.jl_amd/csrc/ls.hip
@@ -44,12 +44,13 @@
 
 __global__ void scatter_csc_kernel(double* __restrict__ F, int64_t ld, const int32_t* __restrict__ row,
                                    const int32_t* __restrict__ col, const double* __restrict__ nz, int64_t nnz,
-                                   unsigned long long* __restrict__ amax, int32_t lim = INT32_MAX) {
+                                   unsigned long long* __restrict__ amax, int32_t lim = INT32_MAX, int* __restrict__ nonfinite = nullptr) {
     const int64_t k = blockIdx.x * (int64_t)blockDim.x + threadIdx.x;
     double v = 0.0;
     if (k < nnz && row[k] < lim && col[k] < lim) {
         v = nz[k];
         F[row[k] + (int64_t)col[k] * ld] = v;
+        if (nonfinite != nullptr && !(fabs(v) <= DBL_MAX)) *nonfinite = 1;
     }
     if (amax != nullptr) wave_absmax_to(amax + AMAX_SLOT0 + AMAX_STRIDE * (blockIdx.x & (AMAX_SLOTS - 1)), v);
 }
@@ -635,6 +636,7 @@
             return 0;
         }
     if (!strcmp(key, "pivot_tol")) { ls->pivot_tol = value; return 0; }
+    if (!strcmp(key, "envelope")) { ls->envelope = value != 0.0; return 0; }
     if (!strcmp(key, "split_a")) { ls->split_a = (int)value; return 0; }
     if (!strcmp(key, "tail_rows")) { ls->tail_rows = (int64_t)value; return 0; }
     if (!strcmp(key, "tail_nbo")) { ls->tail_nbo = (int64_t)value; return 0; }
@@ -828,13 +830,31 @@
 }
 extern "C" {
 
+static int* set_envelope(mnk_ls* ls, const int32_t* env_dev, const std::vector<int32_t>& env_host) {
+    ls->env_dev = nullptr;
+    if (!ls->envelope || env_dev == nullptr || ls->algo == MNK_QR) return nullptr;
+    if (!ls->env_word.p) {
+        if (ls->env_word.alloc(2) || hipMemsetAsync(ls->env_word.p, 0, 2 * sizeof(int), ls->ctx->stream) != hipSuccess) {
+            (void)hipGetLastError();
+            ls->env_word.release();
+            return nullptr;
+        }
+    }
+    if (ls->env_armed && hipMemsetAsync(ls->env_word.p, 0, sizeof(int), ls->ctx->stream) != hipSuccess) { (void)hipGetLastError(); return nullptr; }
+    ls->env_armed = true;
+    ls->env_dev = env_dev;
+    ls->env_host.assign(env_host.begin(), env_host.begin() + std::min<size_t>(env_host.size(), (size_t)(ls->Np / 128)));
+    return ls->env_word.p;
+}
+
 static int transfer_sc(mnk_ls* ls, mnk_sc* sc) {
     int rc = prepare_fill(ls);
     if (rc) return rc;
     const int64_t nnz = sc->nnz_aug;
+    int* nonfinite = set_envelope(ls, sc->d_tile_env.p, sc->tile_env);
     hipLaunchKernelGGL(scatter_csc_kernel, dim3((unsigned)((nnz + 255) / 256)), dim3(256), 0, ls->ctx->stream,
                        ls->fact.p, ls->ld, sc->aug_row.p, sc->aug_col.p, sc->aug_nz.p, nnz, amax_word(ls),
-                       ls->N < sc->n ? (int32_t)ls->N : INT32_MAX);
+                       ls->N < sc->n ? (int32_t)ls->N : INT32_MAX, nonfinite);
     MNK_HIP(hipGetLastError());
     return 0;
 }
@@ -857,6 +877,7 @@
     }
     mnk_ls* c = ls->probe_ls;
     c->pivot_tol = ls->pivot_tol;
+    c->envelope = ls->envelope;
     int rc = mnk_ls_factorize_sc_async(c, sc);
     if (!rc) rc = mnk_ls_fetch_info(c);
     if (rc) return rc;
@@ -906,6 +927,7 @@
 }
 
 static int transfer_dense(mnk_ls* ls, const double* Adev, int64_t lda) {
+    ls->env_dev = nullptr;
     dim3 grid((unsigned)ls->Np, (unsigned)((ls->Np + 1023) / 1024));
     hipLaunchKernelGGL(copy_lower_kernel, grid, dim3(256), 0, ls->ctx->stream, ls->fact.p, ls->ld, Adev, lda,
                        ls->N, ls->Np, amax_word(ls));
@@ -1011,15 +1033,18 @@
     int rc = drow.upload(row, ls->ctx->stream);
     rc |= dcol.upload(col, ls->ctx->stream);
     rc |= dnz.upload(nzv, ls->ctx->stream);
+    const std::vector<int32_t> env = ls->envelope ? mnk_tile_envelope(N, row.data(), col.data(), nnz) : std::vector<int32_t>();
+    if (ls->envelope) rc |= ls->env_own.upload(env, ls->ctx->stream);
     if (rc) return -2;
     rc = ensure_wbuf(ls);
     if (rc) return rc;
-    auto transfer = [ls, nnz, &drow, &dcol, &dnz]() -> int {
+    auto transfer = [ls, nnz, &drow, &dcol, &dnz, &env]() -> int {
         int r = prepare_fill(ls);
         if (r) return r;
+        int* nonfinite = set_envelope(ls, env.empty() ? nullptr : ls->env_own.p, env);
         if (nnz > 0)
             hipLaunchKernelGGL(scatter_csc_kernel, dim3((unsigned)((nnz + 255) / 256)), dim3(256), 0, ls->ctx->stream,
-                               ls->fact.p, ls->ld, drow.p, dcol.p, dnz.p, nnz, amax_word(ls));
+                               ls->fact.p, ls->ld, drow.p, dcol.p, dnz.p, nnz, amax_word(ls), INT32_MAX, nonfinite);
         MNK_HIP(hipGetLastError());
         return 0;
     };
@@ -1034,6 +1059,18 @@
     }
     ls->retransfer = nullptr;
     return rc;
+}
+
+int mnk_debug_tile_env_csc(int64_t n, const int32_t* colptr, const int32_t* rowval, int index_base, int32_t* out, int cap) {
+    if (n <= 0 || colptr == nullptr || rowval == nullptr || cap < 0) return -1;
+    const int64_t nnz = colptr[n] - index_base;
+    std::vector<int32_t> row(nnz), col(nnz);
+    for (int64_t c = 0; c < n; ++c)
+        for (int64_t k = colptr[c] - index_base; k < colptr[c + 1] - index_base; ++k) { row[k] = rowval[k] - index_base; col[k] = (int32_t)c; }
+    const std::vector<int32_t> env = mnk_tile_envelope(n, row.data(), col.data(), nnz);
+    if (out != nullptr)
+        for (int I = 0; I < std::min((int)env.size(), cap); ++I) out[I] = env[I];
+    return (int)env.size();
 }
 
 int mnk_ls_inertia(mnk_ls* ls, int64_t* num_pos, int64_t* num_zero, int64_t* num_neg) {
@@ -1241,6 +1278,23 @@
     if (!strcmp(key, "dag_ntasks")) { *value = ls->dag_ntasks; return 0; }
     if (!strcmp(key, "dag_ntasks1")) { *value = ls->dag_ntasks1; return 0; }
     if (!strcmp(key, "dag_js2")) { *value = ls->dag_js2; return 0; }
+    if (!strcmp(key, "env_ksteps") || !strcmp(key, "env_ksteps_skipped")) {
+        int64_t total = 0, skipped = 0;
+        int gate = 1;
+        if (ls->env_used && ls->env_word.p) MNK_HIP(mnk::d2h_copy(&gate, ls->env_word.p + 1, sizeof(int), ls->ctx->stream));
+        const std::vector<int>& h = ls->dag_host_tasks;
+        const int ne = (int)ls->env_host.size();
+        for (size_t t = 0; t + 3 < h.size(); t += 4) {
+            const int flags = h[t] & 255, I = h[t + 1] & 0xffff, J = h[t + 2], kb = h[t + 3] & 0xffff, ke = h[t + 3] >> 16;
+            if (flags & 8) continue;
+            total += ke - kb;
+            if (!ls->env_used || gate != 0 || I >= ne || J >= ne) continue;
+            const int e = std::max(ls->env_host[I], ls->env_host[J]);
+            skipped += std::min(ke, std::max(kb, e)) - kb;
+        }
+        *value = (double)(!strcmp(key, "env_ksteps") ? total : skipped);
+        return 0;
+    }
     set_error("mnk_ls_get_stat: unknown key '%s'", key);
     return -1;
 }
diff --git a/madnlp.jl_amd/csrc/sparse_kkt.hip b/madnlp.jl_amd/csrc/sparse_kkt.hip
--- a/madnlp.jl_amd/csrc/sparse_kkt.hip
+++ b/madnlp.jl_amd/csrc/sparse_kkt.hip
@@ -246,6 +246,7 @@
     for (int64_t c = 0; c < n; ++c) sc->aug_colptr[c + 1] += sc->aug_colptr[c];
     sc->nnz_aug = slot + 1;
     sc->len_jptr = L;
+    sc->tile_env = mnk_tile_envelope(n, a_row.data(), a_col.data(), sc->nnz_aug);
 
     if (!ctx) { *out = sc; return 0; }
     hipStream_t s = ctx->stream;
@@ -260,6 +261,7 @@
     rc |= sc->aug_jptr.upload(a_jptr, s); rc |= sc->aug_jc.upload(a_jc, s);
     rc |= sc->aug_jk.upload(a_jk, s); rc |= sc->aug_jl.upload(a_jl, s);
     rc |= sc->aug_row.upload(a_row, s); rc |= sc->aug_col.upload(a_col, s);
+    rc |= sc->d_tile_env.upload(sc->tile_env, s);
     rc |= sc->d_jt_colptr.upload(sc->jt_colptr, s); rc |= sc->d_jt_rowval.upload(sc->jt_rowval, s);
     rc |= sc->d_h_colptr.upload(sc->h_colptr, s); rc |= sc->d_h_rowval.upload(sc->h_rowval, s);
     rc |= sc->jac_coo.alloc(nnzj); rc |= sc->hess_coo.alloc(nnzh);
@@ -324,6 +326,14 @@
     if (nnz_aug) *nnz_aug = sc->nnz_aug;
     if (len_jptr) *len_jptr = sc->len_jptr;
     return 0;
+}
+
+int mnk_sc_debug_tile_env(mnk_sc* sc, int64_t order, int32_t* out, int cap) {
+    if (sc == nullptr || order <= 0 || order > sc->n || cap < 0) return -1;
+    const int n = (int)((order + 127) / 128);
+    if (out != nullptr)
+        for (int I = 0; I < std::min(n, cap); ++I) out[I] = sc->tile_env[I];
+    return n;
 }
 
 int mnk_sc_get_structure(mnk_sc* sc, int which, int32_t* colptr, int32_t* rowval) {
```

Result: faster. 106.2 it/s (median of 6 runs) (+6.6%).
